# manuelbb-upb/Morbit.jl

Hardware: AMD Instinct MI355X
Metric: RBF build+solve+eval cycles/sec (higher is better)
Workload: dtype f64

## Files before the change

include/mrbf.h:

```cpp
#ifndef MRBF_H
#define MRBF_H

#include <stdint.h>

#ifdef __cplusplus
extern "C" {
#endif

typedef struct mrbf_ctx mrbf_ctx;
typedef struct mrbf_model mrbf_model;

enum {
    MRBF_CUBIC = 0,
    MRBF_INV_MULTIQUADRIC = 1,
    MRBF_MULTIQUADRIC = 2,
    MRBF_THIN_PLATE_SPLINE = 3,
    MRBF_GAUSSIAN = 4
};

enum {
    MRBF_OK = 0,
    MRBF_ENOTPD = 1,
    MRBF_ESINGULAR = 2,
    MRBF_EHIP = 3,
// ... 20 lines not shown
    MRBF_OPT_TIMING = 6,
    MRBF_OPT_DIAG_IMPL = 7,
    MRBF_OPT_CHOL_WINDOW = 8,
    MRBF_OPT_SPIN_MS = 9,
    MRBF_OPT_LAST_DEVICE_MS = 11,
    MRBF_OPT_SLOW_LAUNCHES = 12,
    MRBF_OPT_ARENA_BYTES = 13,
    MRBF_OPT_LIVE_HANDLES = 14,
    MRBF_OPT_DEBUG_FAULT = 10
};

enum {
    MRBF_FB_CHOL_HOST_DRIVEN = 1,
    MRBF_FB_BACKSOLVE_BLOCKED = 2,
    MRBF_FB_LU = 4
};

typedef struct {
    int32_t path;
    int32_t factor_info;
    int32_t n, q;
    double rel_residual;
    double max_pitw;
    double mu;
    float ms_gram, ms_project, ms_factor, ms_solve, ms_check, ms_total;
    int32_t fallbacks;
    int32_t giveup_code;
    float ms_factor_device;
    int32_t slow_launches;
} mrbf_fit_info;

typedef struct {
    float ms_total;
    float ms_dist, ms_kernel, ms_contract;
} mrbf_eval_info;

int32_t mrbf_init(int32_t device_id, mrbf_ctx **ctx);
int32_t mrbf_shutdown(mrbf_ctx *ctx);
const char *mrbf_last_error(const mrbf_ctx *ctx);
const char *mrbf_version(void);
int32_t mrbf_set_option(mrbf_ctx *ctx, int32_t key, double value);
int32_t mrbf_get_option(const mrbf_ctx *ctx, int32_t key, double *value);
int32_t mrbf_set_stream(mrbf_ctx *ctx, void *hip_stream);
int32_t mrbf_sync(mrbf_ctx *ctx);

int32_t mrbf_gram(mrbf_ctx *ctx, int64_t n, int32_t d, const double *centres, int32_t kernel_id, double a, double b,
                  int32_t poly_deg, double *Phi_out, double *Pi_out, float *ms);

int32_t mrbf_cross_gram(mrbf_ctx *ctx, int64_t m, int64_t n, int32_t d, const double *X, const double *centres, int32_t kernel_id,
                        double a, double b, double *K_out);

int32_t mrbf_fit(mrbf_ctx *ctx, int64_t n, int32_t d, int32_t k, const double *centres, const double *values,
                 int32_t kernel_id, double a, double b, int32_t poly_deg, mrbf_model **model, double *weights_out,
                 double *poly_out, mrbf_fit_info *info);

int32_t mrbf_model_from_coeffs(mrbf_ctx *ctx, int64_t n, int32_t d, int32_t k, const double *centres,
                               const double *weights, const double *poly, int32_t kernel_id, double a, double b,
                               int32_t poly_deg, mrbf_model **model);

int32_t mrbf_eval(mrbf_ctx *ctx, const mrbf_model *model, int64_t m, const double *X, double *vals_out,
                  double *jac_out, mrbf_eval_info *info);

int32_t mrbf_backtrack(mrbf_ctx *ctx, const mrbf_model *model, const double *x, const double *dir, double step0,
                       double omega, int32_t strict, double const_rhs, double shrink, double min_stepsize,
                       int32_t max_loops, double *x_plus, double *mx_plus, double *step, int32_t *n_loops);

int32_t mrbf_affine_scores(mrbf_ctx *ctx, int64_t mc, int32_t d, int32_t dz, const double *shifted, const double *Z, int32_t p_is_inf,
                           double *vals_out, int64_t *argmax, double *maxval);
int32_t mrbf_affine_select(mrbf_ctx *ctx, int64_t mc, int32_t d, const double *shifted, int32_t j0, const double *Q0, int32_t max_picks,
                           double pivot_val, int32_t p_is_inf, int64_t *picked_out, int32_t *n_picked, double *Z_out);

typedef struct {
    int64_t mc;
    int32_t j0;
    int32_t max_picks;
    double pivot_val;
    const double *shifted;
    const double *Q0;
    int64_t *picked_out;
    double *Z_out;
    int32_t n_picked;
    int32_t reserved;
} mrbf_affine_job;
int32_t mrbf_affine_select_batch(mrbf_ctx *ctx, int64_t n_starts, int32_t d, int32_t p_is_inf, mrbf_affine_job *jobs,
                                 float *ms_total);

typedef struct mrbf_round4_state mrbf_round4_state;
int32_t mrbf_round4(mrbf_ctx *ctx, int64_t n0, int32_t d, const double *start_sites, int64_t mc, const double *cand_sites,
                    int32_t kernel_id, double a, double b, int32_t poly_deg, int32_t max_points, double theta_pivot_cholesky,
                    int32_t *accepted_out, int32_t *n_accepted, mrbf_round4_state **state);
int32_t mrbf_fit_from_round4(mrbf_ctx *ctx, const mrbf_round4_state *state, int32_t k, const double *values, mrbf_model **model,
                             double *weights_out, double *poly_out, mrbf_fit_info *info);
int32_t mrbf_round4_sites(const mrbf_round4_state *state, int64_t *n0, int64_t *n_candidates, int32_t *n_accepted);
int32_t mrbf_free_round4(mrbf_ctx *ctx, mrbf_round4_state *state);

typedef struct {
    int64_t n0, mc;
    const double *start_sites;
    const double *cand_sites;
    int32_t kernel_id, poly_deg;
    double a, b;
    int32_t max_points;
    double theta_pivot_cholesky;
    int32_t *accepted_out;
    int32_t n_accepted;
    int32_t rc;
} mrbf_round4_job;
int32_t mrbf_round4_batch(mrbf_ctx *ctx, int64_t n_starts, int32_t d, mrbf_round4_job *jobs, float *ms_total);

int32_t mrbf_model_dims(const mrbf_model *model, int64_t *n, int32_t *d, int32_t *k, int32_t *q);
int32_t mrbf_free_model(mrbf_ctx *ctx, mrbf_model *model);

typedef struct {
    int64_t n, m;
    int32_t d, k, kernel_id, poly_deg;
    double a, b;
    const double *centres;
    const double *values;
    const double *X;
    double *weights_out;
    double *poly_out;
    double *vals_out;
    double *jac_out;
} mrbf_problem;

typedef struct {
    int32_t status;
    int32_t device;
    mrbf_fit_info fit;
    float ms_eval;
    double checksum_w;
    double checksum_vals;
} mrbf_result;

int32_t mrbf_batch_run(int32_t n_dev, const int32_t *device_ids, int64_t n_problems, const mrbf_problem *problems,
                       mrbf_result *results);

typedef struct {
    int64_t n;
    int32_t d, k, kernel_id, poly_deg;
    double a, b;
    const double *centres, *values;
    double *weights_out, *poly_out;
    mrbf_model *model;
    int32_t status;
    int32_t reserved;
    mrbf_fit_info info;
} mrbf_fit_job;
int32_t mrbf_fit_batch(mrbf_ctx *ctx, int64_t n_starts, mrbf_fit_job *jobs, float *ms_total);

int32_t mrbf_debug_env(const char *name);
int32_t mrbf_debug_mfma_layout(mrbf_ctx *ctx, double *out16x16_a_times_b, const double *A16x4, const double *B4x16);
int32_t mrbf_debug_potrf(mrbf_ctx *ctx, int64_t n, double *A_colmajor_inout, int32_t impl, int32_t *info, float *ms);
int32_t mrbf_debug_diag(mrbf_ctx *ctx, const double *A128, int32_t reps, float *ms_per_call, double *shader_cycles,
                        double *realtime_us);
int32_t mrbf_debug_mfma_peak(mrbf_ctx *ctx, int32_t blocks_per_cu, int32_t threads, int32_t iters, float *ms, double *tflops);
int32_t mrbf_debug_mfma_asm(mrbf_ctx *ctx, int32_t variant, int32_t blocks_per_cu, int32_t iters, float *ms, double *tflops,
                            double *cycles_per_mfma);
int32_t mrbf_debug_dgemm(mrbf_ctx *ctx, int32_t m, int32_t n, int32_t k, float *ms, double *tflops);
int32_t mrbf_debug_mega_tables(int32_t nt, int32_t mt, int32_t slack, int32_t slack_chain, int32_t first, int32_t win, int32_t srows,
                               int32_t half_cols, int64_t *out6);
int32_t mrbf_debug_mega_tables2(int32_t nt, int32_t mt, int32_t slack, int32_t slack_chain, int32_t first, int32_t win, int32_t srows,
                                int32_t half_cols, const int32_t *opt5, int64_t *out6);
int32_t mrbf_debug_mega_plan(int32_t nt, int32_t mt, int32_t xreal, int64_t *out39);

enum { MRBF_PS_OK = 0, MRBF_PS_CRITICAL = 1, MRBF_PS_FAILURE = 2 };
typedef struct {
    int32_t max_ideal_evals;
    int32_t max_ps_evals;
    int32_t max_polish_evals;
    int32_t reserved;
    uint64_t seed;
    double t0;
    double xtol_rel;
} mrbf_ps_options;
typedef struct {
    int32_t status;
    int32_t generations;
    int32_t evals_ideal, evals_ps, evals_polish;
    float ms_total;
    double tau;
} mrbf_ps_info;
int32_t mrbf_ps_step(mrbf_ctx *ctx, const mrbf_model *model, const double *x_n, const double *lb_eff, const double *ub_eff,
                     const double *fx_n, const double *r_or_null, const mrbf_ps_options *opts, double *x_trial, double *mx_trial,
                     double *r_out, mrbf_ps_info *info);

enum { MRBF_ROLE_NONE = -1, MRBF_ROLE_EQ = -2, MRBF_ROLE_INEQ = -3 };
typedef struct {
    int32_t n_models, n_objectives;
    const mrbf_model *const *models;
    const int32_t *roles;
    int32_t n_lin_eq, n_lin_ineq;
    const double *A_eq, *b_eq, *A_ineq, *b_ineq;
    double eq_tol;
} mrbf_ps_problem;
int32_t mrbf_ps_step_problem(mrbf_ctx *ctx, const mrbf_ps_problem *problem, const double *x_n, const double *lb_eff,
                             const double *ub_eff, const double *fx_n, const double *r_or_null, const mrbf_ps_options *opts,
                             double *x_trial, double *mx_trial, double *r_out, mrbf_ps_info *info);
int32_t mrbf_debug_ps_rank(mrbf_ctx *ctx, int32_t lam, const double *f, const double *phi, uint64_t seed, int32_t gen, int32_t impl,
                           int32_t *order_out, int32_t *gave_up);

enum { MRBF_SD_OK = 0, MRBF_SD_NO_OBJECTIVE = 1, MRBF_SD_INFEASIBLE = 2, MRBF_SD_GAVE_UP = 3 };
int32_t mrbf_sd_direction(mrbf_ctx *ctx, int64_t n_lp, int32_t d, int32_t k, int32_t m_eq, int32_t m_ineq, const double *G,
                          const double *x, const double *lb, const double *ub, const double *A_eq, const double *b_eq,
                          const double *A_ineq, const double *b_ineq, int32_t normalize, double *d_out, double *omega_out,
                          double *dual_out, int32_t *status_out, int32_t *iters_out);
typedef struct {
    int32_t status;
    int32_t iterations;
    int32_t bound_flips;
    float ms_total;
    double omega;
} mrbf_sd_info;
int32_t mrbf_sd_criticality(mrbf_ctx *ctx, const mrbf_ps_problem *problem, const double *x, const double *x_n, const double *lb,
                            const double *ub, int32_t normalize, double *d_out, double *dual_out, mrbf_sd_info *info);

enum { MRBF_NS_OK = 0, MRBF_NS_INFEASIBLE = 1, MRBF_NS_GAVE_UP = 2 };
int32_t mrbf_normal_direction(mrbf_ctx *ctx, int64_t n_lp, int32_t d, int32_t m_eq, int32_t m_ineq, const double *x, const double *lb,
                              const double *ub, const double *A_eq, const double *b_eq, const double *A_ineq, const double *b_ineq,
                              double *n_out, double *alpha_out, double *dual_out, int32_t *status_out, int32_t *iters_out);
typedef struct {
    int32_t status;
    int32_t iterations;
    int32_t bound_flips;
    float ms_total;
    double alpha;
    double delta;
} mrbf_normal_info;
int32_t mrbf_normal_step(mrbf_ctx *ctx, const mrbf_ps_problem *problem, int32_t d, const double *x, const double *lb, const double *ub,
                         double delta, double kappa_delta, double delta_max, int32_t variable_radius, double *n_out, double *dual_out,
                         mrbf_normal_info *info);

typedef struct {
    int32_t strict;
    int32_t max_loops;
    double const_rhs;
    double shrink;
    double min_stepsize;
} mrbf_sd_step_options;
typedef struct {
    int32_t branch;
    int32_t loops;
    float ms_total;
    double sigma;
    double omega;
    double step_norm;
} mrbf_sd_step_info;
int32_t mrbf_sd_step(mrbf_ctx *ctx, const mrbf_ps_problem *problem, const double *x, const double *x_n, double delta, const double *lb,
                     const double *ub, double omega, const double *d, const mrbf_sd_step_options *opts, double *x_plus, double *mx_plus,
                     mrbf_sd_step_info *info);

typedef struct {
    int32_t sd_status;
    int32_t iterations, bound_flips;
    int32_t branch, loops;
    int32_t reserved;
    double omega;
    double omega_step;
    double sigma, step_norm;
} mrbf_sd_batch_record;
int32_t mrbf_sd_iterate_batch(mrbf_ctx *ctx, int64_t n_starts, const mrbf_ps_problem *shape, const mrbf_model *const *models,
                              const double *x, const double *x_n, const double *delta, const double *lb, const double *ub,
                              int32_t normalize, const mrbf_sd_step_options *opts, double *d_out, double *x_plus, double *mx_plus,
                              mrbf_sd_batch_record *records, float *ms_total);

typedef struct {
    int32_t status;
    int32_t iterations, bound_flips;
    int32_t reserved;
    double alpha;
    double delta;
} mrbf_normal_batch_record;
int32_t mrbf_normal_step_batch(mrbf_ctx *ctx, int64_t n_starts, const mrbf_ps_problem *shape, const mrbf_model *const *models, int32_t d,
                               const double *x, const double *lb, const double *ub, const double *delta, double kappa_delta,
                               double delta_max, int32_t variable_radius, double *n_out, double *x_n_out, double *dual_out,
                               mrbf_normal_batch_record *records, float *ms_total);

enum { MRBF_DISPATCH_REFERENCE = 0, MRBF_DISPATCH_DEVICE = 1 };
enum { MRBF_FIT_FULL = 0, MRBF_FIT_FROM_ROUND4 = 1 };
enum { MRBF_ENTRY_ROUND4 = 1, MRBF_ENTRY_FIT_FROM_ROUND4 = 2, MRBF_ENTRY_PS_STEP = 3, MRBF_ENTRY_BACKTRACK = 4, MRBF_ENTRY_AFFINE = 5,
       MRBF_ENTRY_SD = 6, MRBF_ENTRY_NORMAL = 7, MRBF_ENTRY_SD_STEP = 8, MRBF_ENTRY_SD_BATCH = 9, MRBF_ENTRY_AFFINE_BATCH = 10,
       MRBF_ENTRY_FIT_BATCH = 11, MRBF_ENTRY_NORMAL_BATCH = 12, MRBF_ENTRY_ROUND4_BATCH = 13 };
int32_t mrbf_dispatch_ps(int32_t d, int32_t k, int32_t n_models, int32_t n_nl_constraints, int32_t n_lin_constraints, int32_t n_foreign);
int32_t mrbf_dispatch_sd(int32_t d, int32_t k, int32_t n_models, int32_t n_nl_constraints, int32_t n_lin_constraints, int32_t n_foreign);
int32_t mrbf_dispatch_normal(int32_t d, int32_t n_models, int32_t n_nl_constraints, int32_t n_lin_constraints, int32_t n_foreign);
int32_t mrbf_dispatch_sd_step(int32_t d, int32_t k, int32_t n_models, int32_t n_nl_constraints, int32_t n_lin_constraints, int32_t n_foreign,
                              int32_t max_loops);
int32_t mrbf_dispatch_sd_batch(int64_t n_starts, int32_t d, int32_t k, int32_t n_models, int32_t n_nl_constraints,
                               int32_t n_lin_constraints, int32_t n_foreign, int32_t max_loops);
int32_t mrbf_dispatch_normal_batch(int64_t n_starts, int32_t d, int32_t n_models, int32_t n_nl_constraints, int32_t n_lin_constraints,
                                   int32_t n_foreign);
int32_t mrbf_dispatch_backtrack(int32_t n_objective_models, int32_t n_foreign, int32_t outputs_in_order);
int32_t mrbf_dispatch_affine(int64_t n_candidates, int32_t d);
int32_t mrbf_dispatch_affine_batch(int64_t n_starts, int32_t d, int32_t p_is_inf);
int32_t mrbf_dispatch_round4(int64_t n0, int32_t d, int32_t poly_deg, int64_t n_candidates);
int32_t mrbf_dispatch_fit_batch(int64_t n_starts);
int32_t mrbf_dispatch_round4_batch(int64_t n_starts, int32_t d);
int32_t mrbf_dispatch_fit(int64_t n_training, int64_t state_n0, int32_t state_q, int32_t state_n_accepted, int32_t same_sites);
int32_t mrbf_dispatch_after(int32_t entry, int32_t rc);

int32_t mrbf_stochastic_rank(int32_t lam, const double *f, const double *phi, const double *u, double pf, int32_t *idx_out);

#ifdef __cplusplus
}
#endif
#endif
// ... 1 lines not shown
```

morbit.jl_amd/_lib.py:

```python
import ctypes
import os

import numpy as np

_HERE = os.path.dirname(os.path.abspath(__file__))
LIB_PATH = os.environ.get("MRBF_LIB") or os.path.join(_HERE, "libmrbf.so")

c_dp = ctypes.POINTER(ctypes.c_double)
c_fp = ctypes.POINTER(ctypes.c_float)
c_ip = ctypes.POINTER(ctypes.c_int32)
c_vp = ctypes.c_void_p

MRBF_OK, MRBF_ENOTPD, MRBF_ESINGULAR, MRBF_EHIP, MRBF_EBLAS, MRBF_ENOMEM, MRBF_ENODEVICE, MRBF_ENCCL = range(8)
PATH_CHOL, PATH_PROJ_CHOL, PATH_LU, PATH_MINNORM, PATH_ROUND4 = 1, 2, 3, 4, 5
OPT_GRAM_MODE, OPT_RESIDUAL, OPT_FORCE_PATH, OPT_CHOL_IMPL, OPT_EVAL_IMPL, OPT_TIMING, OPT_DIAG_IMPL, OPT_CHOL_WINDOW = 1, 2, 3, 4, 5, 6, 7, 8
OPT_SPIN_MS, OPT_DEBUG_FAULT, OPT_LAST_DEVICE_MS, OPT_SLOW_LAUNCHES = 9, 10, 11, 12
OPT_ARENA_BYTES, OPT_LIVE_HANDLES = 13, 14
FB_CHOL_HOST_DRIVEN, FB_BACKSOLVE_BLOCKED, FB_LU = 1, 2, 4


class FitInfo(ctypes.Structure):
    _fields_ = [("path", ctypes.c_int32), ("factor_info", ctypes.c_int32), ("n", ctypes.c_int32), ("q", ctypes.c_int32),
                ("rel_residual", ctypes.c_double), ("max_pitw", ctypes.c_double), ("mu", ctypes.c_double),
                ("ms_gram", ctypes.c_float), ("ms_project", ctypes.c_float), ("ms_factor", ctypes.c_float),
# ... 24 lines not shown

    def asdict(self):
        return {f: getattr(self, f) for f, _ in self._fields_}


PS_OK, PS_CRITICAL, PS_FAILURE = 0, 1, 2
ROLE_NONE, ROLE_EQ, ROLE_INEQ = -1, -2, -3
DISPATCH_REFERENCE, DISPATCH_DEVICE = 0, 1
FIT_FULL, FIT_FROM_ROUND4 = 0, 1
ENTRY_ROUND4, ENTRY_FIT_FROM_ROUND4, ENTRY_PS_STEP, ENTRY_BACKTRACK, ENTRY_AFFINE, ENTRY_SD, ENTRY_NORMAL, ENTRY_SD_STEP = 1, 2, 3, 4, 5, 6, 7, 8
ENTRY_SD_BATCH = 9
ENTRY_AFFINE_BATCH = 10
ENTRY_FIT_BATCH = 11
ENTRY_NORMAL_BATCH = 12
ENTRY_ROUND4_BATCH = 13
SD_OK, SD_NO_OBJECTIVE, SD_INFEASIBLE, SD_GAVE_UP = 0, 1, 2, 3
NS_OK, NS_INFEASIBLE, NS_GAVE_UP = 0, 1, 2
SD_BRANCH_DELTA, SD_BRANCH_ONE, SD_BRANCH_INTERSECT = 0, 1, 2


class PsProblem(ctypes.Structure):
    _fields_ = [("n_models", ctypes.c_int32), ("n_objectives", ctypes.c_int32), ("models", ctypes.POINTER(ctypes.c_void_p)),
                ("roles", ctypes.POINTER(ctypes.c_int32)), ("n_lin_eq", ctypes.c_int32), ("n_lin_ineq", ctypes.c_int32),
                ("A_eq", ctypes.c_void_p), ("b_eq", ctypes.c_void_p), ("A_ineq", ctypes.c_void_p), ("b_ineq", ctypes.c_void_p),
                ("eq_tol", ctypes.c_double)]


class SdInfo(ctypes.Structure):
    _fields_ = [("status", ctypes.c_int32), ("iterations", ctypes.c_int32), ("bound_flips", ctypes.c_int32), ("ms_total", ctypes.c_float),
                ("omega", ctypes.c_double)]

    def asdict(self):
        return {f: getattr(self, f) for f, _ in self._fields_}


class NormalInfo(ctypes.Structure):
    _fields_ = [("status", ctypes.c_int32), ("iterations", ctypes.c_int32), ("bound_flips", ctypes.c_int32), ("ms_total", ctypes.c_float),
                ("alpha", ctypes.c_double), ("delta", ctypes.c_double)]

    def asdict(self):
        return {f: getattr(self, f) for f, _ in self._fields_}


class SdStepOptions(ctypes.Structure):
    _fields_ = [("strict", ctypes.c_int32), ("max_loops", ctypes.c_int32), ("const_rhs", ctypes.c_double), ("shrink", ctypes.c_double),
                ("min_stepsize", ctypes.c_double)]


class SdStepInfo(ctypes.Structure):
    _fields_ = [("branch", ctypes.c_int32), ("loops", ctypes.c_int32), ("ms_total", ctypes.c_float), ("sigma", ctypes.c_double),
                ("omega", ctypes.c_double), ("step_norm", ctypes.c_double)]

    def asdict(self):
        return {f: getattr(self, f) for f, _ in self._fields_}


class SdBatchRecord(ctypes.Structure):
    _fields_ = [("sd_status", ctypes.c_int32), ("iterations", ctypes.c_int32), ("bound_flips", ctypes.c_int32), ("branch", ctypes.c_int32),
                ("loops", ctypes.c_int32), ("reserved", ctypes.c_int32), ("omega", ctypes.c_double), ("omega_step", ctypes.c_double),
                ("sigma", ctypes.c_double), ("step_norm", ctypes.c_double)]

    def asdict(self):
        return {f: getattr(self, f) for f, _ in self._fields_}


class NormalBatchRecord(ctypes.Structure):
    _fields_ = [("status", ctypes.c_int32), ("iterations", ctypes.c_int32), ("bound_flips", ctypes.c_int32), ("reserved", ctypes.c_int32),
                ("alpha", ctypes.c_double), ("delta", ctypes.c_double)]

    def asdict(self):
        return {f: getattr(self, f) for f, _ in self._fields_}


class AffineJob(ctypes.Structure):
    _fields_ = [("mc", ctypes.c_int64), ("j0", ctypes.c_int32), ("max_picks", ctypes.c_int32), ("pivot_val", ctypes.c_double),
                ("shifted", ctypes.c_void_p), ("Q0", ctypes.c_void_p), ("picked_out", ctypes.c_void_p), ("Z_out", ctypes.c_void_p),
                ("n_picked", ctypes.c_int32), ("reserved", ctypes.c_int32)]


class Round4Job(ctypes.Structure):
    _fields_ = [("n0", ctypes.c_int64), ("mc", ctypes.c_int64), ("start_sites", ctypes.c_void_p), ("cand_sites", ctypes.c_void_p),
                ("kernel_id", ctypes.c_int32), ("poly_deg", ctypes.c_int32), ("a", ctypes.c_double), ("b", ctypes.c_double),
                ("max_points", ctypes.c_int32), ("theta_pivot_cholesky", ctypes.c_double), ("accepted_out", ctypes.c_void_p),
                ("n_accepted", ctypes.c_int32), ("rc", ctypes.c_int32)]


class FitJob(ctypes.Structure):
    _fields_ = [("n", ctypes.c_int64), ("d", ctypes.c_int32), ("k", ctypes.c_int32), ("kernel_id", ctypes.c_int32),
                ("poly_deg", ctypes.c_int32), ("a", ctypes.c_double), ("b", ctypes.c_double), ("centres", ctypes.c_void_p),
                ("values", ctypes.c_void_p), ("weights_out", ctypes.c_void_p), ("poly_out", ctypes.c_void_p), ("model", ctypes.c_void_p),
                ("status", ctypes.c_int32), ("reserved", ctypes.c_int32), ("info", FitInfo)]


class Problem(ctypes.Structure):
    _fields_ = [("n", ctypes.c_int64), ("m", ctypes.c_int64), ("d", ctypes.c_int32), ("k", ctypes.c_int32),
                ("kernel_id", ctypes.c_int32), ("poly_deg", ctypes.c_int32), ("a", ctypes.c_double), ("b", ctypes.c_double),
                ("centres", c_dp), ("values", c_dp), ("X", c_dp), ("weights_out", c_dp), ("poly_out", c_dp),
                ("vals_out", c_dp), ("jac_out", c_dp)]


class Result(ctypes.Structure):
    _fields_ = [("status", ctypes.c_int32), ("device", ctypes.c_int32), ("fit", FitInfo), ("ms_eval", ctypes.c_float),
                ("checksum_w", ctypes.c_double), ("checksum_vals", ctypes.c_double)]


SIGNATURES = {
    "mrbf_init": (ctypes.c_int32, [ctypes.c_int32, ctypes.POINTER(c_vp)]),
    "mrbf_shutdown": (ctypes.c_int32, [c_vp]),
    "mrbf_last_error": (ctypes.c_char_p, [c_vp]),
    "mrbf_version": (ctypes.c_char_p, []),
    "mrbf_set_option": (ctypes.c_int32, [c_vp, ctypes.c_int32, ctypes.c_double]),
    "mrbf_get_option": (ctypes.c_int32, [c_vp, ctypes.c_int32, c_dp]),
    "mrbf_set_stream": (ctypes.c_int32, [c_vp, c_vp]),
    "mrbf_sync": (ctypes.c_int32, [c_vp]),
    "mrbf_gram": (ctypes.c_int32, [c_vp, ctypes.c_int64, ctypes.c_int32, c_vp, ctypes.c_int32, ctypes.c_double,
                                   ctypes.c_double, ctypes.c_int32, c_vp, c_vp, c_fp]),
    "mrbf_cross_gram": (ctypes.c_int32, [c_vp, ctypes.c_int64, ctypes.c_int64, ctypes.c_int32, c_vp, c_vp, ctypes.c_int32, ctypes.c_double,
                                         ctypes.c_double, c_vp]),
    "mrbf_fit": (ctypes.c_int32, [c_vp, ctypes.c_int64, ctypes.c_int32, ctypes.c_int32, c_vp, c_vp, ctypes.c_int32,
                                  ctypes.c_double, ctypes.c_double, ctypes.c_int32, ctypes.POINTER(c_vp), c_vp, c_vp,
                                  ctypes.POINTER(FitInfo)]),
    "mrbf_model_from_coeffs": (ctypes.c_int32, [c_vp, ctypes.c_int64, ctypes.c_int32, ctypes.c_int32, c_vp, c_vp, c_vp,
                                                ctypes.c_int32, ctypes.c_double, ctypes.c_double, ctypes.c_int32,
                                                ctypes.POINTER(c_vp)]),
    "mrbf_eval": (ctypes.c_int32, [c_vp, c_vp, ctypes.c_int64, c_vp, c_vp, c_vp, ctypes.POINTER(EvalInfo)]),
    "mrbf_backtrack": (ctypes.c_int32, [c_vp, c_vp, c_vp, c_vp, ctypes.c_double, ctypes.c_double, ctypes.c_int32,
                                        ctypes.c_double, ctypes.c_double, ctypes.c_double, ctypes.c_int32, c_vp, c_vp,
                                        c_vp, c_ip]),
    "mrbf_affine_scores": (ctypes.c_int32, [c_vp, ctypes.c_int64, ctypes.c_int32, ctypes.c_int32, c_vp, c_vp, ctypes.c_int32, c_vp,
                                            ctypes.POINTER(ctypes.c_int64), c_dp]),
    "mrbf_affine_select": (ctypes.c_int32, [c_vp, ctypes.c_int64, ctypes.c_int32, c_vp, ctypes.c_int32, c_vp, ctypes.c_int32, ctypes.c_double,
                                            ctypes.c_int32, ctypes.POINTER(ctypes.c_int64), c_ip, c_vp]),
    "mrbf_affine_select_batch": (ctypes.c_int32, [c_vp, ctypes.c_int64, ctypes.c_int32, ctypes.c_int32, ctypes.POINTER(AffineJob), c_fp]),
    "mrbf_round4": (ctypes.c_int32, [c_vp, ctypes.c_int64, ctypes.c_int32, c_vp, ctypes.c_int64, c_vp, ctypes.c_int32, ctypes.c_double,
                                     ctypes.c_double, ctypes.c_int32, ctypes.c_int32, ctypes.c_double, c_vp, c_ip, ctypes.POINTER(c_vp)]),
    "mrbf_fit_from_round4": (ctypes.c_int32, [c_vp, c_vp, ctypes.c_int32, c_vp, ctypes.POINTER(c_vp), c_vp, c_vp, ctypes.POINTER(FitInfo)]),
    "mrbf_round4_sites": (ctypes.c_int32, [c_vp, ctypes.POINTER(ctypes.c_int64), ctypes.POINTER(ctypes.c_int64), c_ip]),
    "mrbf_free_round4": (ctypes.c_int32, [c_vp, c_vp]),
    "mrbf_round4_batch": (ctypes.c_int32, [c_vp, ctypes.c_int64, ctypes.c_int32, ctypes.POINTER(Round4Job), c_fp]),
    "mrbf_dispatch_round4_batch": (ctypes.c_int32, [ctypes.c_int64, ctypes.c_int32]),
    "mrbf_model_dims": (ctypes.c_int32, [c_vp, ctypes.POINTER(ctypes.c_int64), c_ip, c_ip, c_ip]),
    "mrbf_free_model": (ctypes.c_int32, [c_vp, c_vp]),
    "mrbf_batch_run": (ctypes.c_int32, [ctypes.c_int32, c_ip, ctypes.c_int64, ctypes.POINTER(Problem),
                                        ctypes.POINTER(Result)]),
    "mrbf_fit_batch": (ctypes.c_int32, [c_vp, ctypes.c_int64, ctypes.POINTER(FitJob), c_fp]),
    "mrbf_dispatch_fit_batch": (ctypes.c_int32, [ctypes.c_int64]),
    "mrbf_debug_mfma_layout": (ctypes.c_int32, [c_vp, c_vp, c_vp, c_vp]),
    "mrbf_debug_potrf": (ctypes.c_int32, [c_vp, ctypes.c_int64, c_vp, ctypes.c_int32, c_ip, c_fp]),
    "mrbf_debug_env": (ctypes.c_int32, [ctypes.c_char_p]),
    "mrbf_debug_diag": (ctypes.c_int32, [c_vp, c_vp, ctypes.c_int32, c_fp, c_dp, c_dp]),
    "mrbf_debug_ps_rank": (ctypes.c_int32, [c_vp, ctypes.c_int32, c_vp, c_vp, ctypes.c_uint64, ctypes.c_int32, ctypes.c_int32, c_ip, c_ip]),
    "mrbf_debug_mfma_peak": (ctypes.c_int32, [c_vp, ctypes.c_int32, ctypes.c_int32, ctypes.c_int32, c_fp, c_dp]),
    "mrbf_debug_mfma_asm": (ctypes.c_int32, [c_vp, ctypes.c_int32, ctypes.c_int32, ctypes.c_int32, c_fp, c_dp, c_dp]),
    "mrbf_debug_dgemm": (ctypes.c_int32, [c_vp, ctypes.c_int32, ctypes.c_int32, ctypes.c_int32, c_fp, c_dp]),
    "mrbf_debug_mega_tables": (ctypes.c_int32, [ctypes.c_int32] * 8 + [c_vp]),
    "mrbf_debug_mega_tables2": (ctypes.c_int32, [ctypes.c_int32] * 8 + [c_vp, c_vp]),
    "mrbf_debug_mega_plan": (ctypes.c_int32, [ctypes.c_int32] * 3 + [c_vp]),
    "mrbf_stochastic_rank": (ctypes.c_int32, [ctypes.c_int32, c_vp, c_vp, c_vp, ctypes.c_double, c_vp]),
    "mrbf_ps_step": (ctypes.c_int32, [c_vp, c_vp, c_vp, c_vp, c_vp, c_vp, c_vp, ctypes.POINTER(PsOptions), c_vp, c_vp, c_vp,
                                      ctypes.POINTER(PsInfo)]),
    "mrbf_ps_step_problem": (ctypes.c_int32, [c_vp, ctypes.POINTER(PsProblem), c_vp, c_vp, c_vp, c_vp, c_vp, ctypes.POINTER(PsOptions),
                                              c_vp, c_vp, c_vp, ctypes.POINTER(PsInfo)]),
    "mrbf_sd_direction": (ctypes.c_int32, [c_vp, ctypes.c_int64, ctypes.c_int32, ctypes.c_int32, ctypes.c_int32, ctypes.c_int32] + [c_vp] * 8
                          + [ctypes.c_int32, c_vp, c_vp, c_vp, c_vp, c_vp]),
    "mrbf_sd_criticality": (ctypes.c_int32, [c_vp, ctypes.POINTER(PsProblem), c_vp, c_vp, c_vp, c_vp, ctypes.c_int32, c_vp, c_vp,
                                             ctypes.POINTER(SdInfo)]),
    "mrbf_normal_direction": (ctypes.c_int32, [c_vp, ctypes.c_int64, ctypes.c_int32, ctypes.c_int32, ctypes.c_int32] + [c_vp] * 12),
    "mrbf_normal_step": (ctypes.c_int32, [c_vp, ctypes.POINTER(PsProblem), ctypes.c_int32, c_vp, c_vp, c_vp, ctypes.c_double, ctypes.c_double,
                                          ctypes.c_double, ctypes.c_int32, c_vp, c_vp, ctypes.POINTER(NormalInfo)]),
    "mrbf_sd_step": (ctypes.c_int32, [c_vp, ctypes.POINTER(PsProblem), c_vp, c_vp, ctypes.c_double, c_vp, c_vp, ctypes.c_double, c_vp,
                                      ctypes.POINTER(SdStepOptions), c_vp, c_vp, ctypes.POINTER(SdStepInfo)]),
    "mrbf_sd_iterate_batch": (ctypes.c_int32, [c_vp, ctypes.c_int64, ctypes.POINTER(PsProblem), ctypes.POINTER(ctypes.c_void_p), c_vp, c_vp, c_vp,
                                               c_vp, c_vp, ctypes.c_int32, ctypes.POINTER(SdStepOptions), c_vp, c_vp, c_vp,
                                               ctypes.POINTER(SdBatchRecord), c_fp]),
    "mrbf_dispatch_sd_batch": (ctypes.c_int32, [ctypes.c_int64] + [ctypes.c_int32] * 7),
    "mrbf_normal_step_batch": (ctypes.c_int32, [c_vp, ctypes.c_int64, ctypes.POINTER(PsProblem), ctypes.POINTER(ctypes.c_void_p), ctypes.c_int32,
                                                c_vp, c_vp, c_vp, c_vp, ctypes.c_double, ctypes.c_double, ctypes.c_int32, c_vp, c_vp, c_vp,
                                                ctypes.POINTER(NormalBatchRecord), c_fp]),
    "mrbf_dispatch_normal_batch": (ctypes.c_int32, [ctypes.c_int64] + [ctypes.c_int32] * 5),
    "mrbf_dispatch_ps": (ctypes.c_int32, [ctypes.c_int32] * 6),
    "mrbf_dispatch_sd_step": (ctypes.c_int32, [ctypes.c_int32] * 7),
    "mrbf_dispatch_sd": (ctypes.c_int32, [ctypes.c_int32] * 6),
    "mrbf_dispatch_normal": (ctypes.c_int32, [ctypes.c_int32] * 5),
    "mrbf_dispatch_backtrack": (ctypes.c_int32, [ctypes.c_int32] * 3),
    "mrbf_dispatch_affine": (ctypes.c_int32, [ctypes.c_int64, ctypes.c_int32]),
    "mrbf_dispatch_affine_batch": (ctypes.c_int32, [ctypes.c_int64, ctypes.c_int32, ctypes.c_int32]),
    "mrbf_dispatch_round4": (ctypes.c_int32, [ctypes.c_int64, ctypes.c_int32, ctypes.c_int32, ctypes.c_int64]),
    "mrbf_dispatch_fit": (ctypes.c_int32, [ctypes.c_int64, ctypes.c_int64, ctypes.c_int32, ctypes.c_int32, ctypes.c_int32]),
    "mrbf_dispatch_after": (ctypes.c_int32, [ctypes.c_int32, ctypes.c_int32]),
}

_LIB = None


class MrbfError(RuntimeError):
    def __init__(self, code, msg):
        super().__init__("libmrbf error %d: %s" % (code, msg))
        self.code = code


def load():
    global _LIB
    if _LIB is None:
        if not os.path.exists(LIB_PATH):
            raise ImportError("libmrbf.so is not built (%s); run `python -c 'import __graft_entry__ as g; g.build()'` "
                              "or `make -C morbit.jl_amd/csrc`. There is no CPU fallback." % LIB_PATH)
        lib = ctypes.CDLL(LIB_PATH)
        for name, (res, args) in SIGNATURES.items():
            fn = getattr(lib, name)
            fn.restype = res
            fn.argtypes = args
        _LIB = lib
    return _LIB


def as_ptr(a):
    if a is None:
        return None
    if isinstance(a, np.ndarray):
        return ctypes.c_void_p(a.ctypes.data)
    if hasattr(a, "data_ptr"):
        return ctypes.c_void_p(a.data_ptr())
    raise TypeError("expected numpy array or tensor, got %r" % type(a))


def host_f64(a, shape=None):
    a = np.ascontiguousarray(a, dtype=np.float64)
    if shape is not None:
        a = a.reshape(shape)
    return a


class Context:

    def __init__(self, device_id=-1):
        self.lib = load()
        h = c_vp()
        rc = self.lib.mrbf_init(device_id, ctypes.byref(h))
        if rc != 0:
            raise MrbfError(rc, (self.lib.mrbf_last_error(None) or b"").decode())
        self.h = h

    def check(self, rc):
        if rc != 0:
            raise MrbfError(rc, (self.lib.mrbf_last_error(self.h) or b"").decode())

    def set_option(self, key, value):
        self.check(self.lib.mrbf_set_option(self.h, key, float(value)))

    def get_option(self, key):
        v = ctypes.c_double()
        self.check(self.lib.mrbf_get_option(self.h, key, ctypes.byref(v)))
        return v.value

    def sync(self):
        self.check(self.lib.mrbf_sync(self.h))

    def close(self):
        if getattr(self, "h", None):
            self.lib.mrbf_shutdown(self.h)
            self.h = None

    def __del__(self):
        try:
            self.close()
        except Exception:
            pass


_DEFAULT_CTX = {}


def default_context(device_id=-1):
    import threading

    key = (threading.get_ident(), device_id)
    if key not in _DEFAULT_CTX:
        _DEFAULT_CTX[key] = Context(device_id)
    return _DEFAULT_CTX[key]
```

morbit.jl_amd/csrc/backsolve.hip:

```cpp
#include "common.hpp"

namespace mrbf {

namespace bsolve {

constexpr int NB = 128, NTHR = 512;
typedef double v2d __attribute__((ext_vector_type(2)));
typedef double v4d __attribute__((ext_vector_type(4)));
typedef __attribute__((address_space(1))) unsigned gu32;
typedef __attribute__((address_space(1))) double gf64;
typedef __attribute__((address_space(1))) v2d gv2d;

template <int KB>
struct Shared {
    double xs[2][KB][NB];
    int ok;
};

__global__ __launch_bounds__(256) void premul_kernel(const double *__restrict__ L, int64_t lda, const double *__restrict__ linv_all,
                                                     double *__restrict__ Mbuf, int nb, unsigned *__restrict__ flags, int nflags,
                                                     unsigned long long *__restrict__ xb, int nxb) {
    for (int e = blockIdx.x * 256 + threadIdx.x; e < nflags; e += gridDim.x * 256) flags[e] = 0u;
    for (int e = blockIdx.x * 256 + threadIdx.x; e < nxb; e += gridDim.x * 256) xb[e] = ~0ull;
    const int slab = blockIdx.x & 3, t = (blockIdx.x >> 2) & 1, j = blockIdx.x >> 3;
    const int i = j + 1 + t;
    if (i >= nb) return;
    const double *A = L + (int64_t)i * NB + (int64_t)j * NB * lda;
    const double *B = linv_all + (size_t)j * NB * NB;
    double *M = Mbuf + ((size_t)j * 2 + t) * NB * NB;
    const int lane = threadIdx.x & 63, wave = threadIdx.x >> 6, l15 = lane & 15, l4 = lane >> 4;
    const int i0 = 32 * wave, j0 = 32 * slab;
    v4d acc[2][2];
#pragma unroll
    for (int a = 0; a < 2; ++a)
#pragma unroll
        for (int b = 0; b < 2; ++b) acc[a][b] = (v4d){0.0, 0.0, 0.0, 0.0};
    const double *pa = A + (i0 + l15) + (int64_t)(j0 + l4) * lda;
    const double *pb = B + (j0 + l4) + (int64_t)(j0 + l15) * NB;
    constexpr int UK = 8;
    double fa0[2][UK], fa1[2][UK], fb0[2][UK], fb1[2][UK];
    auto burst = [&](int buf) {
#pragma unroll
        for (int u = 0; u < UK; ++u) {
            fa0[buf][u] = pa[(int64_t)4 * u * lda];
            fa1[buf][u] = pa[(int64_t)4 * u * lda + 16];
            fb0[buf][u] = pb[4 * u];
            fb1[buf][u] = pb[4 * u + 16 * NB];
        }
        pa += (int64_t)4 * UK * lda;
        pb += 4 * UK;
    };
    auto mma = [&](int buf) {
#pragma unroll
        for (int u = 0; u < UK; ++u) {
            acc[0][0] = __builtin_amdgcn_mfma_f64_16x16x4f64(fa0[buf][u], fb0[buf][u], acc[0][0], 0, 0, 0);
            acc[0][1] = __builtin_amdgcn_mfma_f64_16x16x4f64(fa0[buf][u], fb1[buf][u], acc[0][1], 0, 0, 0);
            acc[1][0] = __builtin_amdgcn_mfma_f64_16x16x4f64(fa1[buf][u], fb0[buf][u], acc[1][0], 0, 0, 0);
            acc[1][1] = __builtin_amdgcn_mfma_f64_16x16x4f64(fa1[buf][u], fb1[buf][u], acc[1][1], 0, 0, 0);
        }
    };
    const int nburst = (NB - j0) / (4 * UK);
    burst(0);
    for (int b = 0; b < nburst; b += 2) {
        if (b + 1 < nburst) burst(1);
        mma(0);
        if (b + 1 >= nburst) break;
        if (b + 2 < nburst) burst(0);
        mma(1);
    }
#pragma unroll
    for (int a = 0; a < 2; ++a)
#pragma unroll
        for (int b = 0; b < 2; ++b)
#pragma unroll
            for (int r = 0; r < 4; ++r) M[(i0 + 16 * a + l4 + 4 * r) + (size_t)(j0 + 16 * b + l15) * NB] = acc[a][b][r];
}

__device__ __forceinline__ void load_tile(const double *__restrict__ T, int64_t ldt, v2d (&r)[2][8]) {
    const int lane = threadIdx.x & 63, w = threadIdx.x >> 6;
    const double *p = T + (int64_t)(16 * w + 2 * (lane >> 3)) * ldt + 2 * (lane & 7);
#pragma unroll
    for (int cc = 0; cc < 2; ++cc)
#pragma unroll
        for (int u = 0; u < 8; ++u) r[cc][u] = *(const gv2d *)(p + cc * ldt + 16 * u);
}

template <int N>
__device__ __forceinline__ double shl_lanes(double v) {
    const long long b = __double_as_longlong(v);
    const int lo = __builtin_amdgcn_update_dpp((int)b, (int)b, 0x100 + N, 0xf, 0xf, false);
    const int hi = __builtin_amdgcn_update_dpp((int)(b >> 32), (int)(b >> 32), 0x100 + N, 0xf, 0xf, false);
    return __longlong_as_double(((long long)hi << 32) | (unsigned)lo);
}

template <int KB>
__device__ __forceinline__ void tile_dot(const double (*xs)[NB], const v2d (&r)[2][8], double (&out)[2][KB]) {
    const int q = threadIdx.x & 7;
    double acc[2][KB];
#pragma unroll
    for (int cc = 0; cc < 2; ++cc)
#pragma unroll
        for (int l = 0; l < KB; ++l) acc[cc][l] = 0.0;
#pragma unroll
    for (int u = 0; u < 8; ++u) {
#pragma unroll
        for (int l = 0; l < KB; ++l) {
            const v2d x = *(const v2d *)&xs[l][16 * u + 2 * q];
#pragma unroll
            for (int cc = 0; cc < 2; ++cc) acc[cc][l] = fma(r[cc][u][1], x[1], fma(r[cc][u][0], x[0], acc[cc][l]));
        }
    }
#pragma unroll
    for (int cc = 0; cc < 2; ++cc)
#pragma unroll
        for (int l = 0; l < KB; ++l) {
            double v = acc[cc][l];
            v += shl_lanes<4>(v);
            v += shl_lanes<2>(v);
            v += shl_lanes<1>(v);
            out[cc][l] = v;
        }
}

template <int KB>
__device__ __forceinline__ void await_block(Shared<KB> &sh, double (*xs)[NB], const double *glob, int i, double spec, int backoff,
                                            unsigned *abortw, unsigned epoch, unsigned long long spin_ticks, int *status, int code) {
    const int tid = threadIdx.x;
    if (tid >= KB * NB) return;
    const gf64 *src = (const gf64 *)&glob[((size_t)i * KB + tid / NB) * NB + (tid % NB)];
    double v = spec;
    if (__double_as_longlong(v) == -1ll) v = __hip_atomic_load(src, __ATOMIC_RELAXED, __HIP_MEMORY_SCOPE_AGENT);
    unsigned spins = 0;
    unsigned long long t0 = 0;
    while (__double_as_longlong(v) == -1ll) {
        if ((++spins & 63u) == 0u) {
            if (__hip_atomic_load((const gu32 *)abortw, __ATOMIC_RELAXED, __HIP_MEMORY_SCOPE_AGENT) != 0u) {
                sh.ok = 0;
                break;
            }
            const unsigned long long now = wall_clock64();
            if (t0 == 0) t0 = now;
            if (now - t0 > spin_ticks) {
                __hip_atomic_store((gu32 *)abortw, epoch, __ATOMIC_RELAXED, __HIP_MEMORY_SCOPE_AGENT);
                *(__attribute__((address_space(1))) int *)status = code + (i & 0xff);
                sh.ok = 0;
                break;
            }
        }
        for (int b = 0; b < backoff; ++b) __builtin_amdgcn_s_sleep(8);
        v = __hip_atomic_load(src, __ATOMIC_RELAXED, __HIP_MEMORY_SCOPE_AGENT);
    }
    xs[tid / NB][tid % NB] = v;
}

__device__ __forceinline__ void lds_barrier() { asm volatile("s_waitcnt lgkmcnt(0)\n\ts_barrier" ::: "memory"); }

__device__ __forceinline__ void publish(double *dst, v2d v) {
    if (__double_as_longlong(v[0]) == -1ll) v[0] = __longlong_as_double(0x7ff8000000000000ll);
    if (__double_as_longlong(v[1]) == -1ll) v[1] = __longlong_as_double(0x7ff8000000000000ll);
    asm volatile("global_store_dwordx4 %0, %1, off sc1" ::"v"(dst), "v"(v) : "memory");
}

template <int KB>
__global__ __launch_bounds__(NTHR, 1) void backsolve_persistent_kernel(const double *__restrict__ L, int64_t lda, const double *__restrict__ linv_all,
                                                                        const double *__restrict__ Mbuf, double *__restrict__ Y, int64_t ldy, int k0,
                                                                        int nb, unsigned *flags, unsigned epoch, unsigned long long spin_ticks,
                                                                        int *status, int fault, double *__restrict__ xb, double *__restrict__ zb,
                                                                        long long *stamps) {
    __shared__ __attribute__((aligned(16))) Shared<KB> sh;
    const int p = (int)blockIdx.x >> 1;
    const bool finisher = blockIdx.x & 1;
    const int j = nb - 1 - p, tid = threadIdx.x;
    const int lane = tid & 63, col = 16 * (tid >> 6) + 2 * (lane >> 3), q = lane & 7;
    unsigned *abortw = flags + (size_t)nb * 32;
    const int na = nb - 1 - j, npm = na < 2 ? na : 2, npl = na - npm;
    if (tid == 0) sh.ok = 1;
// ... 13 lines not shown
        auto look = [&](int s) {
            const int i = nb - 1 - (s < npl ? s : (npl > 0 ? npl - 1 : 0));
            const int e = tid < KB * NB ? tid : 0;
            return __hip_atomic_load((const gf64 *)&xb[((size_t)i * KB + e / NB) * NB + (e % NB)], __ATOMIC_RELAXED, __HIP_MEMORY_SCOPE_AGENT);
        };
        double spec = fillv, spec2 = fillv;
        auto step = [&](int s, const v2d(&r)[2][8]) -> bool {
            double(*xs)[NB] = sh.xs[s & 1];
            if (s < npl) {
                const int i = nb - 1 - s;
                const int backoff = (i - j - 3) < 24 ? (i - j - 3) : 24;
                await_block<KB>(sh, xs, xb, i, spec, backoff, abortw, epoch, spin_ticks, status, 0x700);
                if (stamps && tid == 0 && s == npl - 1) stamps[256 * 5 + j * 4 + 0] = (long long)wall_clock64();
            } else if (q == 0) {
#pragma unroll
                for (int l = 0; l < KB; ++l) *(v2d *)&xs[l][col] = (v2d){w[0][l], w[1][l]};
            }
            spec = spec2;
            spec2 = look(s + 2);
            if (s + 2 >= npl) spec2 = fillv;
            lds_barrier();
            if (!sh.ok) return false;
            double dsum[2][KB];
            tile_dot<KB>(xs, r, dsum);
#pragma unroll
            for (int cc = 0; cc < 2; ++cc)
#pragma unroll
                for (int l = 0; l < KB; ++l) w[cc][l] = s == npl ? dsum[cc][l] : w[cc][l] - dsum[cc][l];
            return true;
        };
        v2d t0[2][8], t1[2][8], t2[2][8];
        const int o = (3 - nst % 3) % 3, G = (nst + o) / 3;
        if (0 - o >= 0) fetch(0 - o, t0);
        if (1 - o >= 0) fetch(1 - o, t1);
        fetch(2 - o, t2);
        spec = look(0);
        if (npl == 0) spec = fillv;
        spec2 = look(1);
        if (npl <= 1) spec2 = fillv;
        int g = 0;
        if (G >= 2) {
            const int s = -o;
            if (s >= 0 && !step(s, t0)) return;
            fetch(s + 3, t0);
            if (s + 1 >= 0 && !step(s + 1, t1)) return;
            fetch(s + 4, t1);
            if (!step(s + 2, t2)) return;
            fetch(s + 5, t2);
            g = 1;
        }
        for (; g < G - 1; ++g) {
            const int s = 3 * g - o;
            if (!step(s, t0)) return;
            fetch(s + 3, t0);
            if (!step(s + 1, t1)) return;
            fetch(s + 4, t1);
            if (!step(s + 2, t2)) return;
            fetch(s + 5, t2);
        }
        {
            const int s = 3 * (G - 1) - o;
            if (s >= 0 && !step(s, t0)) return;
            if (s + 1 >= 0 && !step(s + 1, t1)) return;
            if (!step(s + 2, t2)) return;
        }
        if (stamps && tid == 0) stamps[256 * 5 + j * 4 + 1] = (long long)wall_clock64();
        if (q == 0) {
#pragma unroll
            for (int l = 0; l < KB; ++l) publish(&zb[((size_t)j * KB + l) * NB + col], (v2d){w[0][l], w[1][l]});
        }
        return;
    }
    v2d tm2[2][8], tm1[2][8];
    if (npm == 2) load_tile(Mbuf + ((size_t)j * 2 + 1) * NB * NB, NB, tm2);
    if (npm >= 1) load_tile(Mbuf + (size_t)j * 2 * NB * NB, NB, tm1);
    double acc[2][KB];
#pragma unroll
    for (int cc = 0; cc < 2; ++cc)
#pragma unroll
        for (int l = 0; l < KB; ++l) acc[cc][l] = 0.0;
    if (npm == 2) {
        await_block<KB>(sh, sh.xs[0], xb, j + 2, fillv, 1, abortw, epoch, spin_ticks, status, 0x700);
        lds_barrier();
        if (!sh.ok) return;
        if (stamps && tid == 0) stamps[256 * 5 + j * 4 + 3] = (long long)wall_clock64();
        tile_dot<KB>(sh.xs[0], tm2, acc);
    }
    v2d zj[KB];
    if (q == 0) {
        unsigned spins = 0;
        unsigned long long t0 = 0;
#pragma unroll
        for (int l = 0; l < KB; ++l) {
            const double *src = &zb[((size_t)j * KB + l) * NB + col];
            while (true) {
                v2d v;
                asm volatile("global_load_dwordx4 %0, %1, off sc1\n\ts_waitcnt vmcnt(0)" : "=v"(v) : "v"(src) : "memory");
                if (__double_as_longlong(v[0]) != -1ll && __double_as_longlong(v[1]) != -1ll) {
                    zj[l] = v;
                    break;
                }
                if ((++spins & 63u) == 0u) {
                    if (__hip_atomic_load((const gu32 *)abortw, __ATOMIC_RELAXED, __HIP_MEMORY_SCOPE_AGENT) != 0u) {
                        sh.ok = 0;
                        break;
                    }
                    const unsigned long long now = wall_clock64();
                    if (t0 == 0) t0 = now;
                    if (now - t0 > spin_ticks) {
                        __hip_atomic_store((gu32 *)abortw, epoch, __ATOMIC_RELAXED, __HIP_MEMORY_SCOPE_AGENT);
                        *(__attribute__((address_space(1))) int *)status = 0x600 + (j & 0xff);
                        sh.ok = 0;
                        break;
                    }
                }
                __builtin_amdgcn_s_sleep(2);
            }
            if (!sh.ok) break;
        }
    }
    if (stamps && tid == 0) stamps[256 * 5 + j * 4 + 2] = (long long)wall_clock64();
    double last[2][KB];
#pragma unroll
    for (int cc = 0; cc < 2; ++cc)
#pragma unroll
        for (int l = 0; l < KB; ++l) last[cc][l] = 0.0;
    if (npm >= 1) {
        if (stamps && tid == 0) stamps[256 * 4 + j] = (long long)wall_clock64();
        await_block<KB>(sh, sh.xs[1], xb, j + 1, fillv, 0, abortw, epoch, spin_ticks, status, 0x700);
        if (stamps && tid == 0) stamps[j * 4 + 0] = (long long)wall_clock64();
        lds_barrier();
        if (!sh.ok) return;
        if (stamps && tid == 0) stamps[j * 4 + 1] = (long long)wall_clock64();
        tile_dot<KB>(sh.xs[1], tm1, last);
    } else {
        lds_barrier();
        if (!sh.ok) return;
    }
    if ((fault & 1) && j == nb / 2) return;
    if (stamps && tid == 0) stamps[j * 4 + 2] = (long long)wall_clock64();
    if (q == 0) {
#pragma unroll
        for (int l = 0; l < KB; ++l) {
            const v2d v = (v2d){(zj[l][0] - acc[0][l]) - last[0][l], (zj[l][1] - acc[1][l]) - last[1][l]};
            publish(&xb[((size_t)j * KB + l) * NB + col], v);
            *(v2d *)&Y[(int64_t)(k0 + l) * ldy + (int64_t)j * NB + col] = v;
        }
    }
}

}

int backsolve_blocked(mrbf_ctx *ctx, int64_t npad, const double *L, int64_t lda, const double *linv_all, double *Y, int64_t ldy, int k);

int backsolve_persistent(mrbf_ctx *ctx, int64_t npad, const double *L, int64_t lda, const double *linv_all, double *Y, int64_t ldy, int k,
                         int *status) {
    using namespace bsolve;
    const int nb = (int)(npad / NB);
    static const int force_old = mrbf_env("MRBF_BACKSOLVE_LAUNCHES") ? atoi(mrbf_env("MRBF_BACKSOLVE_LAUNCHES")) : 0;
    const int ncu = ctx->ncu;
    if (force_old || nb < 3 || nb > ncu || (lda & 1) || (reinterpret_cast<uintptr_t>(L) & 15))
        return backsolve_blocked(ctx, npad, L, lda, linv_all, Y, ldy, k);
    unsigned *flags;
    MRBF_TRY(get_buf(ctx, S_BSOLVE_FLAGS, (size_t)(nb + 1) * 32, &flags));
    const unsigned long long spin_ticks = (unsigned long long)std::max(1, ctx->spin_ms) * 100000ull;
    const int fault = (ctx->debug_fault & 2) ? 1 : 0;
    double *xb, *Mbuf;
    MRBF_TRY(get_buf(ctx, S_BSOLVE_X, (size_t)2 * nb * 4 * NB, &xb));
    MRBF_TRY(get_buf(ctx, S_BSOLVE_M, (size_t)nb * 2 * NB * NB, &Mbuf));
    hipLaunchKernelGGL(premul_kernel, dim3((unsigned)(8 * (nb - 1))), dim3(256), 0, ctx->stream, L, lda, linv_all, Mbuf, nb, flags, (nb + 1) * 32,
                       reinterpret_cast<unsigned long long *>(xb), 2 * nb * 4 * NB);
    static const bool want_stamps = mrbf_env("MRBF_BSOLVE_STAMPS") && atoi(mrbf_env("MRBF_BSOLVE_STAMPS")) != 0;
    long long *stamps = nullptr;
    if (want_stamps) {
        static long long *dbg = nullptr;
        if (!dbg) MRBF_HIP(ctx, hipMalloc(&dbg, (size_t)256 * 9 * sizeof(long long)));
        stamps = dbg;
    }
    unsigned epoch = 0;
    for (int k0 = 0; k0 < k; k0 += 4) {
        const int kb = std::min(4, k - k0);
        ++epoch;
        if (k0 > 0) MRBF_HIP(ctx, hipMemsetAsync(xb, 0xff, (size_t)2 * nb * 4 * NB * sizeof(double), ctx->stream));
#define MRBF_BSP(KBV)                                                                                                          \
    hipLaunchKernelGGL((backsolve_persistent_kernel<KBV>), dim3((unsigned)(2 * nb)), dim3(NTHR), 0, ctx->stream, L, lda, linv_all, Mbuf, Y, ldy, k0, nb, \
                       flags, epoch, spin_ticks, status, fault, xb, xb + (size_t)nb * 4 * NB, stamps)
        if (kb == 1) MRBF_BSP(1); else if (kb == 2) MRBF_BSP(2); else if (kb == 3) MRBF_BSP(3); else MRBF_BSP(4);
#undef MRBF_BSP
    }
    MRBF_HIP(ctx, hipGetLastError());
    if (want_stamps) {
        std::vector<long long> h((size_t)256 * 9);
        MRBF_HIP(ctx, hipMemcpyAsync(h.data(), stamps, h.size() * sizeof(long long), hipMemcpyDeviceToHost, ctx->stream));
        MRBF_HIP(ctx, hipStreamSynchronize(ctx->stream));
        double seen = 0, bar = 0, dot = 0, hop = 0, late = 0;
        int cnt = 0;
        for (int j = 1; j + 2 < nb; ++j) {
            seen += (double)(h[j * 4 + 0] - h[(j + 1) * 4 + 2]);
            bar += (double)(h[j * 4 + 1] - h[j * 4 + 0]);
            dot += (double)(h[j * 4 + 2] - h[j * 4 + 1]);
            hop += (double)(h[j * 4 + 2] - h[(j + 1) * 4 + 2]);
            late += (double)(h[256 * 4 + j] - h[(j + 1) * 4 + 2]);
            ++cnt;
        }
        double a3 = 0, zt = 0, zs = 0, x2 = 0;
        int c2 = 0;
        for (int j = 2; j + 4 < nb; ++j) {
            const long long *S = &h[256 * 5 + j * 4];
            a3 += (double)(S[0] - h[(j + 3) * 4 + 2]);
            zt += (double)(S[1] - S[0]);
            zs += (double)(S[2] - S[1]);
            x2 += (double)(S[3] - h[(j + 2) * 4 + 2]);
            ++c2;
        }
        fprintf(stderr, "[backsolve stamps] streamer: x_{j+3} seen %.2f us after its publication, z_j published %.2f us later, finisher has z_j %.2f us "
                "later; finisher past x_{j+2} %.2f us after that block's publication\n", a3 / c2 / 100.0, zt / c2 / 100.0, zs / c2 / 100.0, x2 / c2 / 100.0);
        fprintf(stderr, "[backsolve stamps] nb %d: publish -> seen %.2f us, seen -> barrier %.2f us, barrier -> publish %.2f us, step %.2f us; "
                "the finisher starts polling %.2f us after the publication\n", nb, seen / cnt / 100.0, bar / cnt / 100.0, dot / cnt / 100.0,
                hop / cnt / 100.0, late / cnt / 100.0);
    }
    return 0;
}

}
```

morbit.jl_amd/csrc/chol.hip:

```cpp
#include <chrono>

#include "common.hpp"

namespace mrbf {

int debug_diag(mrbf_ctx *ctx, const double *A128_dev, int reps, float *ms_per_call, unsigned long long *stamps_host);
int launch_pad_identity(mrbf_ctx *ctx, double *A, int64_t n, int64_t npad, int64_t ld);

int potrf_lower(mrbf_ctx *ctx, int impl, int64_t n, double *A, int64_t lda, int *info_host) {
    int *dinfo;
    MRBF_TRY(get_buf(ctx, S_INFO, (size_t)4, &dinfo));
    const int64_t npad = round_up(n, 128);
    if (impl == 0) impl = (lda >= npad) ? ((npad >= ctx->mega.min && npad <= ctx->mega.max) ? 3 : 2) : 1;
    if (impl == 2 || impl == 3) {
        if (lda < npad) return fail(ctx, MRBF_EHIP, "built-in Cholesky needs lda >= round_up(n,128)");
        MRBF_TRY(launch_pad_identity(ctx, A, n, npad, lda));
        PotrfOpts opt;
        opt.impl = impl;
        opt.any_size = true;
        MRBF_TRY(potrf_blocked_tall(ctx, npad, npad, A, lda, dinfo, nullptr, opt));
    } else {
        MRBF_BLAS(ctx, rocsolver_dpotrf(ctx->blas, rocblas_fill_lower, (int)n, A, (int)lda, dinfo));
    }
    MRBF_HIP(ctx, hipMemcpyAsync(info_host, dinfo, sizeof(int), hipMemcpyDeviceToHost, ctx->stream));
    MRBF_HIP(ctx, hipStreamSynchronize(ctx->stream));
    MRBF_TRY(mega_collect_stat(ctx));
    return 0;
}

}

using namespace mrbf;

extern "C" int32_t mrbf_debug_potrf(mrbf_ctx *ctx, int64_t n, double *A, int32_t impl, int32_t *info, float *ms) {
    if (!ctx) return -1;
    if (n <= 0) return -2;
    if (!A) return -3;
    (void)hipSetDevice(ctx->device);
    const int64_t npad = round_up(n, 128);
    double *dA;
    MRBF_TRY(get_buf(ctx, S_PHI, (size_t)npad * npad, &dA));
    const hipMemcpyKind in = is_device_ptr(A) ? hipMemcpyDeviceToDevice : hipMemcpyHostToDevice;
    const hipMemcpyKind out = is_device_ptr(A) ? hipMemcpyDeviceToDevice : hipMemcpyDeviceToHost;
    MRBF_HIP(ctx, hipMemcpy2DAsync(dA, (size_t)npad * sizeof(double), A, (size_t)n * sizeof(double), (size_t)n * sizeof(double),
                                   (size_t)n, in, ctx->stream));
    int hinfo = 0;
    static const double host_trace_ms = mrbf_env("MRBF_MEGA_HOSTTRACE") ? atof(mrbf_env("MRBF_MEGA_HOSTTRACE")) : 0.0;
    auto now_ms = []() { return std::chrono::duration<double, std::milli>(std::chrono::steady_clock::now().time_since_epoch()).count(); };
    const double h0 = now_ms();
    MRBF_HIP(ctx, hipEventRecord(ctx->ev[0], ctx->stream));
    const double h1 = now_ms();
    MRBF_TRY(potrf_lower(ctx, impl, n, dA, npad, &hinfo));
    const double h2 = now_ms();
    MRBF_HIP(ctx, hipEventRecord(ctx->ev[1], ctx->stream));
    MRBF_HIP(ctx, hipEventSynchronize(ctx->ev[1]));
    const double h3 = now_ms();
    if (host_trace_ms > 0.0 && h3 - h0 > host_trace_ms)
        fprintf(stderr, "mrbf_debug_potrf host trace (n %lld): record ev0 %.3f ms | potrf_lower incl. sync %.3f | record ev1 + sync %.3f\n", (long long)n,
                h1 - h0, h2 - h1, h3 - h2);
    if (ms) MRBF_HIP(ctx, hipEventElapsedTime(ms, ctx->ev[0], ctx->ev[1]));
    if (info) *info = hinfo;
    MRBF_HIP(ctx, hipMemcpy2DAsync(A, (size_t)n * sizeof(double), dA, (size_t)npad * sizeof(double), (size_t)n * sizeof(double),
                                   (size_t)n, out, ctx->stream));
    MRBF_HIP(ctx, hipStreamSynchronize(ctx->stream));
    return MRBF_OK;
}

extern "C" int32_t mrbf_debug_diag(mrbf_ctx *ctx, const double *A128, int32_t reps, float *ms_per_call, double *shader_cycles,
                                   double *realtime_us) {
    if (!ctx) return -1;
    if (!A128) return -2;
    (void)hipSetDevice(ctx->device);
    const double *dA;
    MRBF_TRY(stage_in(ctx, S_STAGE_A, A128, 128 * 128, &dA));
    unsigned long long st[6] = {0, 0, 0, 0, 0, 0};
    float ms = 0;
    MRBF_TRY(debug_diag(ctx, dA, reps, &ms, st));
    if (ms_per_call) *ms_per_call = ms;
    if (shader_cycles) *shader_cycles = (double)st[0];
    if (realtime_us) *realtime_us = (double)st[1] / 100.0;
    if (mrbf_env("MRBF_DIAG_VERBOSE"))
        fprintf(stderr, "diag segments (cycles over 128 columns, wave 0): barrier %llu read %llu critical %llu rest %llu\n", st[2], st[3],
                st[4], st[5]);
    return MRBF_OK;
}
```

morbit.jl_amd/csrc/chol_blocked.hip:

```cpp
#include "common.hpp"
#include "mega_gemm.hpp"

namespace mrbf {

typedef double v4d __attribute__((ext_vector_type(4)));
typedef double v2d __attribute__((ext_vector_type(2)));

constexpr int CNB = 128;

enum { UPD_LOWER_SUB = 0, UPD_OVERWRITE = 1, UPD_FULL_SUB = 2, UPD_COLUMN_SUB = 3 };
int launch_diag_v4(mrbf_ctx *ctx, hipStream_t st, double *Ajj, int64_t lda, double *Linv, int *dinfo, int col0);

template <int TM, int MODE>
__global__ __launch_bounds__(256, 2) void chol_update_kernel(const double *__restrict__ A, int64_t lda,
                                                             const double *__restrict__ B, int64_t ldb,
                                                             double *__restrict__ C, int64_t ldc, int K,
                                                             const int *__restrict__ info, int mt_sq = 0, int ntiles_total = 0,
                                                             const double *__restrict__ cvec = nullptr, double cs = 0.0, int64_t cn = 0) {
    constexpr int NJ = (TM == 128) ? 4 : 2;
    __shared__ __attribute__((aligned(16))) double smem[mega::NSTG * mega::STG];
    if (info && *info != 0) return;
    if (MODE == UPD_OVERWRITE || MODE == UPD_COLUMN_SUB) __builtin_amdgcn_s_setprio(2);
    const int tid = threadIdx.x, lane = tid & 63, wave = tid >> 6;
    const int l15 = lane & 15, l4 = lane >> 4;
    const int tile_end = (MODE == UPD_LOWER_SUB && ntiles_total > 0) ? ntiles_total : (int)blockIdx.x + 1;
    for (int bid = blockIdx.x; bid < tile_end; bid += gridDim.x) {
    int ti, tj;
    if (MODE == UPD_LOWER_SUB) {
        const int ntri = mt_sq * (mt_sq + 1) / 2;
        if (bid < ntri || mt_sq == 0) {
            int t = (int)((sqrt(8.0 * (double)bid + 1.0) - 1.0) * 0.5);
            while ((t + 1) * (t + 2) / 2 <= bid) ++t;
            while (t * (t + 1) / 2 > bid) --t;
            ti = t;
            tj = bid - t * (t + 1) / 2;
        } else {
            ti = mt_sq + (bid - ntri) / mt_sq;
            tj = (bid - ntri) % mt_sq;
        }
    } else {
        ti = blockIdx.x;
        tj = blockIdx.y;
    }
    const int64_t I0 = (int64_t)ti * TM, J0 = (int64_t)tj * 128;
    const int ioff = (TM == 128) ? (wave >> 1) * 64 : 0;
    const int joff = (TM == 128) ? (wave & 1) * 64 : wave * 32;

    v4d acc[NJ][4];
#pragma unroll
    for (int j = 0; j < NJ; ++j)
#pragma unroll
        for (int i = 0; i < 4; ++i) acc[j][i] = (v4d){0.0, 0.0, 0.0, 0.0};

    asm volatile("s_waitcnt vmcnt(0)" ::: "memory");
    constexpr bool NEG_START = (MODE == UPD_LOWER_SUB);
    if (NEG_START) {
#pragma unroll
        for (int j = 0; j < NJ; ++j)
#pragma unroll
            for (int r = 0; r < 4; ++r) {
                const int64_t gj = J0 + joff + j * 16 + l4 + 4 * r;
#pragma unroll
                for (int i = 0; i < 4; ++i) acc[j][i][r] = -C[(I0 + ioff + i * 16 + l15) + gj * ldc];
            }
    }
    mega::gemm_acc<TM>(A + I0, lda, B + J0, ldb, K, acc, smem);
    double cvi[4] = {0.0, 0.0, 0.0, 0.0}, cei[4] = {0.0, 0.0, 0.0, 0.0};
    if (MODE == UPD_LOWER_SUB && cvec) {
#pragma unroll
        for (int i = 0; i < 4; ++i) {
            const int64_t gi = I0 + ioff + i * 16 + l15;
            cvi[i] = cs * cvec[gi];
            cei[i] = gi < cn ? cs : 0.0;
        }
    }
#pragma unroll
    for (int j = 0; j < NJ; ++j) {
        double cv[4][4];
        double cvj[4] = {0.0, 0.0, 0.0, 0.0}, cej[4] = {0.0, 0.0, 0.0, 0.0};
        if (MODE == UPD_LOWER_SUB && cvec) {
#pragma unroll
            for (int r = 0; r < 4; ++r) {
                const int64_t gj = J0 + joff + j * 16 + l4 + 4 * r;
                cvj[r] = cvec[gj];
                cej[r] = gj < cn ? 1.0 : 0.0;
            }
        }
        if (MODE != UPD_OVERWRITE && !NEG_START) {
#pragma unroll
            for (int r = 0; r < 4; ++r) {
                const int64_t gj = J0 + joff + j * 16 + l4 + 4 * r;
#pragma unroll
                for (int i = 0; i < 4; ++i) cv[r][i] = C[(I0 + ioff + i * 16 + l15) + gj * ldc];
            }
        }
#pragma unroll
        for (int r = 0; r < 4; ++r) {
            const int64_t gj = J0 + joff + j * 16 + l4 + 4 * r;
#pragma unroll
            for (int i = 0; i < 4; ++i) {
                const int64_t gi = I0 + ioff + i * 16 + l15;
                double *dst = C + gi + gj * ldc;
                if (MODE == UPD_OVERWRITE) {
                    *dst = acc[j][i][r];
                } else if (MODE == UPD_FULL_SUB) {
                    *dst = cv[r][i] - acc[j][i][r];
                } else if (MODE == UPD_COLUMN_SUB) {
                    if (gi >= gj) *dst = cv[r][i] - acc[j][i][r];
                } else {
                    double x = -acc[j][i][r];
                    if (cvec) x -= fma(cei[i], cvj[r], cvi[i] * cej[r]);
                    if (ti != tj || gi >= gj) *dst = x;
                }
            }
        }
    }
    if (bid + (int)gridDim.x < tile_end) __syncthreads();
    }
}

struct __attribute__((aligned(16))) DiagShared {
    double col[2][2 * CNB];
    double rinv[2];
    int sbad;
    unsigned long long seg[4];
    int stamp;
};

__device__ __forceinline__ double fast_rsqrt(double x) {
    double y = __builtin_amdgcn_rsq(x);
    const double h = 0.5 * x;
#pragma unroll
    for (int it = 0; it < 3; ++it) y = y * fma(-h, y * y, 1.5);
    return y;
}

template <int KV, bool STAMP>
__device__ __forceinline__ void diag_phase(double (&a)[8][8], DiagShared &sh, int ti, int tj, int half, int &buf, int &bad) {
    constexpr int KN = (KV < 7) ? KV + 1 : 7;
    double piv = 0.0;
    if (half == 0) piv = __shfl(a[KV][KV], tj, 16);
#pragma unroll 1
    for (int kk = 0; kk < 16; ++kk) {
        const int k = KV * 16 + kk;
        const bool st = STAMP && threadIdx.x < 64;
        unsigned long long s0 = 0, s1 = 0, s2 = 0, s3 = 0;
        if (st) s0 = __builtin_amdgcn_s_memtime();
        __syncthreads();
        if (st) s1 = __builtin_amdgcn_s_memtime();
        double lj[8];
#pragma unroll
        for (int v = KV; v < 8; ++v) lj[v] = sh.col[buf][tj + 16 * v];
        if (half == 0) {
            double li[8];
#pragma unroll
            for (int u = KV; u < 8; ++u) li[u] = sh.col[buf][ti + 16 * u];
            if (st) {
                asm volatile("s_waitcnt lgkmcnt(0)" ::: "memory");
                s2 = __builtin_amdgcn_s_memtime();
            }
            if (kk < 15) {
                if (tj > kk) piv = fma(-lj[KV], lj[KV], piv);
                if (tj == kk + 1) {
                    const int kn = k + 1;
                    double rinv = 0.0;
                    if (piv > 0.0) {
                        rinv = fast_rsqrt(piv);
                    } else if (bad == 0) {
                        bad = kn + 1;
                    }
                    if (ti == 0) sh.rinv[buf ^ 1] = rinv;
                    double w[8];
#pragma unroll
                    for (int u = 0; u < 8; ++u) {
                        const int i = ti + 16 * u;
                        double val = 0.0;
                        if (u >= KV && i >= kn) {
                            val = fma(-li[u], lj[KV], a[u][KV]) * rinv;
                            a[u][KV] = val;
                        }
                        w[u] = val;
                    }
#pragma unroll
                    for (int u = 0; u < 8; ++u) sh.col[buf ^ 1][ti + 16 * u] = w[u];
                }
            } else if (KV < 7) {
                if (tj == 0) {
                    const int kn = k + 1;
                    const double pv = __shfl(fma(-li[KN], lj[KN], a[KN][KN]), 0, 16);
                    double rinv = 0.0;
                    if (pv > 0.0) {
                        rinv = fast_rsqrt(pv);
                    } else if (bad == 0) {
                        bad = kn + 1;
                    }
                    if (ti == 0) sh.rinv[buf ^ 1] = rinv;
                    double w[8];
#pragma unroll
                    for (int u = 0; u < 8; ++u) {
                        double val = 0.0;
                        if (u >= KN) {
                            val = fma(-li[u], lj[KN], a[u][KN]) * rinv;
                            a[u][KN] = val;
                        }
                        w[u] = val;
                    }
#pragma unroll
                    for (int u = 0; u < 8; ++u) sh.col[buf ^ 1][ti + 16 * u] = w[u];
                }
            }
            if (st) {
                asm volatile("s_waitcnt lgkmcnt(0)" ::: "memory");
                s3 = __builtin_amdgcn_s_memtime();
            }
            const bool own_next = (kk < 15) ? (tj == kk + 1) : (KV < 7 && tj == 0);
            const bool lowtri = ti >= tj;
#pragma unroll
            for (int v = KV; v < 8; ++v) {
                double ljv = lj[v];
                if (v == KV) ljv = (tj > kk && !(own_next && kk < 15)) ? ljv : 0.0;
                if (v == KN && KV < 7) ljv = (own_next && kk == 15) ? 0.0 : ljv;
                a[v][v] = fma(lowtri ? -li[v] : 0.0, ljv, a[v][v]);
#pragma unroll
                for (int u = v + 1; u < 8; ++u) a[u][v] = fma(-li[u], ljv, a[u][v]);
            }
            if (st && threadIdx.x == 0) {
                asm volatile("" ::"v"(a[7][7]));
                const unsigned long long s4 = __builtin_amdgcn_s_memtime();
                sh.seg[0] += s1 - s0;
                sh.seg[1] += s2 - s1;
                sh.seg[2] += s3 - s2;
                sh.seg[3] += s4 - s3;
            }
        } else {
            const double rinv = sh.rinv[buf];
            const double ljk = (tj > kk) ? lj[KV] : 0.0;
#pragma unroll
            for (int u = 0; u <= KV; ++u) {
                const double erk = sh.col[buf][CNB + ti + 16 * u] * rinv;
                if (tj == kk) a[u][KV] = erk;
                a[u][KV] = fma(-erk, ljk, a[u][KV]);
#pragma unroll
                for (int v = KV + 1; v < 8; ++v) a[u][v] = fma(-erk, lj[v], a[u][v]);
            }
            if (kk < 15) {
                if (tj == kk + 1) {
#pragma unroll
                    for (int u = 0; u < 8; ++u) sh.col[buf ^ 1][CNB + ti + 16 * u] = (u <= KV) ? a[u][KV] : 0.0;
                }
            } else if (KV < 7) {
                if (tj == 0) {
#pragma unroll
                    for (int u = 0; u < 8; ++u) sh.col[buf ^ 1][CNB + ti + 16 * u] = (u <= KN) ? a[u][KN] : 0.0;
                }
            }
        }
        buf ^= 1;
    }
}

template <bool STAMP>
__global__ __launch_bounds__(512) void chol_diag_kernel(double *__restrict__ A, int64_t lda, double *__restrict__ Linv,
                                                        int *__restrict__ info, int col0,
                                                        unsigned long long *__restrict__ stamps) {
    __shared__ DiagShared sh;
    if (*info != 0) return;
    unsigned long long t0 = 0, r0 = 0;
    if (STAMP) {
        if (threadIdx.x == 0) sh.seg[0] = sh.seg[1] = sh.seg[2] = sh.seg[3] = 0;
        __syncthreads();
        t0 = __builtin_amdgcn_s_memtime();
        r0 = __builtin_amdgcn_s_memrealtime();
    }
    const int tid = threadIdx.x, ti = tid & 15, tj = (tid >> 4) & 15, half = tid >> 8;
    double a[8][8];
#pragma unroll
    for (int v = 0; v < 8; ++v)
#pragma unroll
        for (int u = 0; u < 8; ++u) {
            const int i = ti + 16 * u, j = tj + 16 * v;
            if (half == 0)
                a[u][v] = (i >= j) ? A[i + (int64_t)j * lda] : 0.0;
            else
                a[u][v] = (i == j) ? 1.0 : 0.0;
        }
    int buf = 0, bad = 0;
    if (tj == 0) {
        if (half == 0) {
            const double pv = __shfl(a[0][0], 0, 16);
            double rinv = 0.0;
            if (pv > 0.0) {
                rinv = fast_rsqrt(pv);
            } else {
                bad = 1;
            }
            if (ti == 0) sh.rinv[0] = rinv;
#pragma unroll
            for (int u = 0; u < 8; ++u) {
                a[u][0] *= rinv;
                sh.col[0][ti + 16 * u] = a[u][0];
            }
        } else {
#pragma unroll
            for (int u = 0; u < 8; ++u) sh.col[0][CNB + ti + 16 * u] = (u == 0) ? a[0][0] : 0.0;
        }
    }
    diag_phase<0, STAMP>(a, sh, ti, tj, half, buf, bad);
    diag_phase<1, STAMP>(a, sh, ti, tj, half, buf, bad);
    diag_phase<2, STAMP>(a, sh, ti, tj, half, buf, bad);
    diag_phase<3, STAMP>(a, sh, ti, tj, half, buf, bad);
    diag_phase<4, STAMP>(a, sh, ti, tj, half, buf, bad);
    diag_phase<5, STAMP>(a, sh, ti, tj, half, buf, bad);
    diag_phase<6, STAMP>(a, sh, ti, tj, half, buf, bad);
    diag_phase<7, STAMP>(a, sh, ti, tj, half, buf, bad);
    if (tid == 0) sh.sbad = 0x7fffffff;
    __syncthreads();
    if (bad) atomicMin(&sh.sbad, bad);
    __syncthreads();
    if (sh.sbad != 0x7fffffff) {
        if (tid == 0) *info = col0 + sh.sbad;
        return;
    }
#pragma unroll
    for (int v = 0; v < 8; ++v)
#pragma unroll
        for (int u = 0; u < 8; ++u) {
            const int i = ti + 16 * u, j = tj + 16 * v;
            if (half == 0) {
                if (i >= j) A[i + (int64_t)j * lda] = a[u][v];
            } else {
                Linv[j + i * CNB] = (j >= i) ? a[u][v] : 0.0;
            }
        }
    if (STAMP && threadIdx.x == 0) {
        stamps[0] = __builtin_amdgcn_s_memtime() - t0;
        stamps[1] = __builtin_amdgcn_s_memrealtime() - r0;
        for (int q = 0; q < 4; ++q) stamps[2 + q] = sh.seg[q];
    }
}

__global__ void pad_identity_kernel(double *__restrict__ A, int64_t n, int64_t npad, int64_t ld) {
    const int64_t idx = (int64_t)blockIdx.x * blockDim.x + threadIdx.x;
    const int64_t pw = npad - n;
    if (idx >= npad * pw) return;
    const int64_t j = n + idx / npad, i = idx % npad;
    A[i + j * ld] = (i == j) ? 1.0 : 0.0;
    if (i < n) A[j + i * ld] = 0.0;
}

int launch_pad_identity(mrbf_ctx *ctx, double *A, int64_t n, int64_t npad, int64_t ld) {
    if (npad == n) return 0;
    const int64_t cnt = npad * (npad - n);
    hipLaunchKernelGGL(pad_identity_kernel, dim3((unsigned)((cnt + 255) / 256)), dim3(256), 0, ctx->stream, A, n, npad, ld);
    MRBF_HIP(ctx, hipGetLastError());
    return 0;
}

int debug_diag(mrbf_ctx *ctx, const double *A128_dev, int reps, float *ms_per_call, unsigned long long *stamps_host) {
    const bool with_stamps = reps > 0;
    if (reps < 0) reps = -reps;
    double *W, *Linv;
    int *dinfo;
    unsigned long long *st;
    MRBF_TRY(get_buf(ctx, S_PHI, (size_t)CNB * CNB * reps, &W));
    MRBF_TRY(get_buf(ctx, S_CHOL_WS, (size_t)CNB * CNB, &Linv));
    MRBF_TRY(get_buf(ctx, S_INFO, (size_t)4, &dinfo));
    MRBF_TRY(get_buf(ctx, S_MISC, (size_t)8, (double **)&st));
    for (int r = 0; r < reps; ++r)
        MRBF_HIP(ctx, hipMemcpyAsync(W + (size_t)r * CNB * CNB, A128_dev, sizeof(double) * CNB * CNB, hipMemcpyDeviceToDevice, ctx->stream));
    MRBF_HIP(ctx, hipMemsetAsync(dinfo, 0, sizeof(int), ctx->stream));
    MRBF_HIP(ctx, hipEventRecord(ctx->ev[0], ctx->stream));
    for (int r = 0; r < reps; ++r)
        if (ctx->diag_impl != 1)
            launch_diag_v4(ctx, ctx->stream, W + (size_t)r * CNB * CNB, (int64_t)CNB, Linv, dinfo, 0);
        else if (with_stamps)
            hipLaunchKernelGGL(chol_diag_kernel<true>, dim3(1), dim3(512), 0, ctx->stream, W + (size_t)r * CNB * CNB, (int64_t)CNB, Linv,
                               dinfo, 0, st);
        else
            hipLaunchKernelGGL(chol_diag_kernel<false>, dim3(1), dim3(512), 0, ctx->stream, W + (size_t)r * CNB * CNB, (int64_t)CNB, Linv,
                               dinfo, 0, (unsigned long long *)nullptr);
    MRBF_HIP(ctx, hipEventRecord(ctx->ev[1], ctx->stream));
    MRBF_HIP(ctx, hipEventSynchronize(ctx->ev[1]));
    float t;
    MRBF_HIP(ctx, hipEventElapsedTime(&t, ctx->ev[0], ctx->ev[1]));
    *ms_per_call = t / reps;
    if (const char *e = mrbf_env("MRBF_DIAG_DBG")) {
        if (atoi(e) & 4) {
            double seg[6];
            MRBF_HIP(ctx, hipMemcpy(seg, Linv, sizeof(seg), hipMemcpyDeviceToHost));
            fprintf(stderr, "diag segments (wave 0, cycles over 8 panels): pre-leaf %.0f leaf %.0f post-leaf %.0f wait-X %.0f deferred %.0f wait-Y %.0f\n",
                    seg[0], seg[1], seg[2], seg[3], seg[4], seg[5]);
        }
    }
    MRBF_HIP(ctx, hipMemcpy(stamps_host, st, 6 * sizeof(unsigned long long), hipMemcpyDeviceToHost));
    return 0;
}

int launch_update_lower(mrbf_ctx *ctx, const double *A, int64_t lda, const double *B, int64_t ldb, double *C, int64_t ldc, int64_t nt,
                        int K, const double *cvec, double cs, int64_t cn) {
    if (nt <= 0 || K <= 0) return 0;
    hipLaunchKernelGGL((chol_update_kernel<128, UPD_LOWER_SUB>), dim3((unsigned)(nt * (nt + 1) / 2)), dim3(256), 0, ctx->stream, A,
                       lda, B, ldb, C, ldc, K, (const int *)nullptr, (int)nt, 0, cvec, cs, cn);
    MRBF_HIP(ctx, hipGetLastError());
    return 0;
}

int potrf_blocked_tall(mrbf_ctx *ctx, int64_t ncols, int64_t mrows, double *A, int64_t lda, int *dinfo, double *linv_all, PotrfOpts opt) {
    if (ncols % CNB != 0 || mrows % CNB != 0 || mrows < ncols || (lda & 1) || (reinterpret_cast<uintptr_t>(A) & 15))
        return fail(ctx, MRBF_EHIP, "potrf_blocked needs 128-padded, 16-byte aligned storage (ncols=%lld mrows=%lld lda=%lld)",
                    (long long)ncols, (long long)mrows, (long long)lda);
    const int impl = opt.impl != 0 ? opt.impl : ctx->chol_impl;
    if ((impl == 3 || (impl == 0 && ncols <= ctx->mega.max)) && (opt.any_size || ncols >= ctx->mega.min))
        return potrf_mega_tall(ctx, ncols, mrows, A, lda, dinfo, linv_all, opt);
    double *Lone = nullptr;
    if (!linv_all) MRBF_TRY(get_buf(ctx, S_CHOL_WS, (size_t)CNB * CNB, &Lone));
    hipStream_t S = ctx->stream, M = ctx->bulk_stream, P = ctx->panel_stream;
    hipEvent_t evStart = ctx->evx[0], evT = ctx->evx[1], evU2 = ctx->evx[2], evEnd = ctx->evx[3];
    const bool single = ncols <= 4 * CNB;
    if (single) M = P = S;
    MRBF_HIP(ctx, hipMemsetAsync(dinfo, 0, sizeof(int), S));
    if (!single) {
        MRBF_HIP(ctx, hipEventRecord(evStart, S));
        MRBF_HIP(ctx, hipStreamWaitEvent(P, evStart, 0));
        MRBF_HIP(ctx, hipStreamWaitEvent(M, evStart, 0));
    }
    const int nb = (int)(ncols / CNB);
    bool have_u2 = false;
    int w0 = 0, W = 1;
    for (int j = 0; j < nb; ++j) {
        const int64_t c = (int64_t)j * CNB;
        if (j == w0) {
            const int64_t rem = ncols - c;
            W = (rem > 4800) ? 4 : (rem > 2400 ? 2 : 1);
            if (ctx->chol_window > 0) W = ctx->chol_window;
        }
        const bool last_in_window = (j == w0 + W - 1) || (j == nb - 1);
        const int kpan = (int)((j - w0 + 1) * CNB);
        const int64_t cw = (int64_t)w0 * CNB;
        double *Ajj = A + c + c * lda;
        double *Linv = linv_all ? linv_all + (size_t)j * CNB * CNB : Lone;
        if (ctx->diag_impl == 1)
            hipLaunchKernelGGL(chol_diag_kernel<false>, dim3(1), dim3(512), 0, P, Ajj, lda, Linv, dinfo, (int)c,
                               (unsigned long long *)nullptr);
        else
            launch_diag_v4(ctx, P, Ajj, lda, Linv, dinfo, (int)c);
        const int64_t m = mrows - c - CNB;
        if (m <= 0) break;
        double *A21 = A + (c + CNB) + c * lda;
        hipLaunchKernelGGL((chol_update_kernel<64, UPD_OVERWRITE>), dim3((unsigned)(m / 64), 1), dim3(256), 0, P, A21, lda, Linv,
                           (int64_t)CNB, A21, lda, CNB, dinfo);
        if (c + CNB >= ncols) break;
        if (!single) MRBF_HIP(ctx, hipEventRecord(evT, P));
        if (have_u2 && !single) {
            MRBF_HIP(ctx, hipStreamWaitEvent(P, evU2, 0));
            have_u2 = false;
        }
        const double *Pw = A + (c + CNB) + cw * lda;
        double *A22 = A + (c + CNB) + (c + CNB) * lda;
        hipLaunchKernelGGL((chol_update_kernel<64, UPD_COLUMN_SUB>), dim3((unsigned)(m / 64), 1), dim3(256), 0, P, Pw, lda, Pw, lda,
                           A22, lda, kpan, dinfo);
        if (last_in_window) {
            const int64_t mt2 = (ncols - c - 2 * CNB) / CNB;
            if (mt2 > 0) {
                if (!single) MRBF_HIP(ctx, hipStreamWaitEvent(M, evT, 0));
                const int64_t mx = (mrows - ncols) / CNB;
                const int64_t rem_next = ncols - c - CNB;
                int Wn = (rem_next > 4800) ? 4 : (rem_next > 2400 ? 2 : 1);
                if (ctx->chol_window > 0) Wn = ctx->chol_window;
                const int64_t na = std::min<int64_t>(Wn, mt2);
                const double *P2 = A + (c + 2 * CNB) + cw * lda;
                double *C2 = A + (c + 2 * CNB) + (c + 2 * CNB) * lda;
                hipLaunchKernelGGL((chol_update_kernel<128, UPD_LOWER_SUB>),
                                   dim3((unsigned)(na * (na + 1) / 2 + (mt2 - na + mx) * na)), dim3(256), 0, M, P2, lda, P2, lda, C2, lda,
                                   kpan, dinfo, (int)na);
                if (!single) MRBF_HIP(ctx, hipEventRecord(evU2, M));
                have_u2 = true;
                const int64_t mb2 = mt2 - na;
                if (mb2 > 0) {
                    const double *P3 = P2 + na * CNB;
                    double *C3 = C2 + na * CNB + na * CNB * lda;
                    const int64_t nt3 = mb2 * (mb2 + 1) / 2 + mx * mb2;
                    const int64_t g3 = (ctx->bulk_grid > 0 && nt3 > ctx->bulk_grid) ? ctx->bulk_grid : nt3;
                    hipLaunchKernelGGL((chol_update_kernel<128, UPD_LOWER_SUB>), dim3((unsigned)g3), dim3(256), 0, M, P3, lda, P3, lda,
                                       C3, lda, kpan, dinfo, (int)mb2, (int)nt3);
                }
            }
            w0 = j + 1;
        }
    }
    MRBF_HIP(ctx, hipGetLastError());
    if (!single) {
        MRBF_HIP(ctx, hipEventRecord(evEnd, P));
        MRBF_HIP(ctx, hipStreamWaitEvent(S, evEnd, 0));
        MRBF_HIP(ctx, hipEventRecord(evStart, M));
        MRBF_HIP(ctx, hipStreamWaitEvent(S, evStart, 0));
    }
    return 0;
}

constexpr int BS_LD = 65;
template <int KB>
__device__ __forceinline__ void tile_tdot(const double *__restrict__ Tl, int64_t ldt, const double *xs ,
                                          double *res , double *stage ,
                                          double *part ) {
    const int tid = threadIdx.x, c = tid & 127, g = tid >> 7;
    double acc[KB];
#pragma unroll
    for (int l = 0; l < KB; ++l) acc[l] = 0.0;
    for (int h = 0; h < 2; ++h) {
        double v[32];
#pragma unroll
        for (int p = 0; p < 32; ++p) v[p] = Tl[(int64_t)(p * 4 + (tid >> 6)) * ldt + 64 * h + (tid & 63)];
        __syncthreads();
#pragma unroll
        for (int p = 0; p < 32; ++p) stage[(p * 4 + (tid >> 6)) * BS_LD + (tid & 63)] = v[p];
        __syncthreads();
#pragma unroll 8
        for (int r = 0; r < 32; ++r) {
            const double t = stage[c * BS_LD + 32 * g + r];
#pragma unroll
            for (int l = 0; l < KB; ++l) acc[l] = fma(t, xs[l * CNB + 64 * h + 32 * g + r], acc[l]);
        }
    }
#pragma unroll
    for (int l = 0; l < KB; ++l) part[l * 256 + tid] = acc[l];
    __syncthreads();
    if (g == 0) {
#pragma unroll
        for (int l = 0; l < KB; ++l) res[l * CNB + c] = part[l * 256 + c] + part[l * 256 + 128 + c];
    }
}

template <int KB>
__global__ __launch_bounds__(256) void chol_backsolve_kernel(const double *__restrict__ L, int64_t lda, const double *__restrict__ linv_all,
                                                             double *__restrict__ Y, int64_t ldy, int k0, int i ,
                                                             int prologue) {
    __shared__ double xs[KB * CNB];
    __shared__ double res[KB * CNB];
    __shared__ double part[KB * 256];
    __shared__ double stage[CNB * BS_LD];
    const int tid = threadIdx.x;
    const int j = blockIdx.x;
    if (!prologue) {
        for (int t = tid; t < KB * CNB; t += 256) xs[t] = Y[(int64_t)(k0 + t / CNB) * ldy + (int64_t)i * CNB + (t % CNB)];
        __syncthreads();
        tile_tdot<KB>(L + (int64_t)i * CNB + (int64_t)j * CNB * lda, lda, xs, res, stage, part);
        __syncthreads();
        for (int t = tid; t < KB * CNB; t += 256) {
            double *yp = Y + (int64_t)(k0 + t / CNB) * ldy + (int64_t)j * CNB + (t % CNB);
            const double v = *yp - res[t];
            *yp = v;
            xs[t] = v;
        }
        if (j != i - 1) return;
        __syncthreads();
// ... 34 lines not shown
```

morbit.jl_amd/csrc/chol_mega.hip:

```cpp
#include <chrono>

#include "chol_diag_core.hpp"
#include "common.hpp"
#include "mega_gemm.hpp"

namespace mrbf {

typedef double v4d __attribute__((ext_vector_type(4)));
typedef double v2d __attribute__((ext_vector_type(2)));

namespace mega {

constexpr int WIN_DEFAULT = 4;

enum { JOB_U = 0, JOB_T = 1, JOB_P = 2, JOB_S = 3, JOB_UH = 4 };
struct Job {
    short kind, i, c, w;
};
enum { CTL_QP = 0, CTL_ABORT = 32, CTL_TIMEOUT = 64, CTL_PCOLS = 96, CTL_QC = 128, CTL_TS = 144 , CTL_WORDS = 160 };
constexpr int QSTRIDE = 32;
__host__ __device__ inline int wstart(int w, int first, int win) { return w <= 0 ? 0 : first + win * (w - 1); }
__host__ __device__ inline int nbulk_updates(int i, int c, int slack, int slack_chain, int first, int win, int srows = 2) {
    const int t = c - ((i - c <= srows) ? slack_chain : slack);
    return t < first ? 0 : (t - first) / win + 1;
// ... 1099 lines not shown
        if (ctx->mega_tables.size() >= 8) {
            MRBF_HIP(ctx, hipStreamSynchronize(ctx->stream));
            size_t lru = 0;
            for (size_t t = 1; t < ctx->mega_tables.size(); ++t)
                if (ctx->mega_tables[t].stamp < ctx->mega_tables[lru].stamp) lru = t;
            (void)hipFree(ctx->mega_tables[lru].block);
            ctx->mega_tables.erase(ctx->mega_tables.begin() + lru);
        }
        MegaTables t{};
        t.nt = NT;
        t.mt = MT;
        t.params = tp;
        t.npanel = (int)pj.size();
        t.nbulk = (int)bj.size();
        t.nchainjobs = (int)cj.size();
        t.nwin = ((int)wqs.size() - 1) / 2;
        const size_t job_bytes = (pj.size() + bj.size() + cj.size() + 1) * sizeof(Job), wq_bytes = wqs.size() * sizeof(int);
        const size_t wq_off = (job_bytes + 255) & ~size_t(255);
        MRBF_HIP(ctx, hipMalloc(&t.block, wq_off + wq_bytes));
        std::vector<char> img(wq_off + wq_bytes, 0);
        Job *hj = (Job *)img.data();
        std::copy(pj.begin(), pj.end(), hj);
        std::copy(bj.begin(), bj.end(), hj + pj.size());
        std::copy(cj.begin(), cj.end(), hj + pj.size() + bj.size());
        std::memcpy(img.data() + wq_off, wqs.data(), wq_bytes);
        MRBF_HIP(ctx, hipMemcpy(t.block, img.data(), img.size(), hipMemcpyHostToDevice));
        t.jobs = t.block;
        t.wq = (char *)t.block + wq_off;
        ctx->mega_tables.push_back(t);
        tab = &ctx->mega_tables.back();
    }
    tab->stamp = ++ctx->mega_table_clock;
    Job *dj = (Job *)tab->jobs;
    a.pjobs = dj;
    a.npanel = tab->npanel;
    a.bjobs = dj + tab->npanel;
    a.nbulk = tab->nbulk;
    a.cjobs = dj + tab->npanel + tab->nbulk;
    a.nchainjobs = tab->nchainjobs;
    a.nwin = tab->nwin;
    a.wq_start = (int *)tab->wq;
    const size_t nfl = ((size_t)CTL_WORDS + (size_t)QSTRIDE * (2 * a.nwin + 1) + (size_t)QSTRIDE * 512 + (size_t)QSTRIDE * (1 + 2 * plan.srows_max) * NT + 2 * (size_t)MT * NT + 3) / 4 * 4;
    unsigned *fl;
    MRBF_TRY(get_buf(ctx, S_MEGA_FLAGS, nfl, &fl));
    hnow();
    MRBF_HIP(ctx, hipMemsetAsync(fl, 0, nfl * sizeof(unsigned), ctx->stream));
    hnow();
    if (!opt.info_clean) MRBF_HIP(ctx, hipMemsetAsync(dinfo, 0, sizeof(int), ctx->stream));
    hnow();
    a.ctl = fl;
    a.wq_head = fl + CTL_WORDS;
    a.quiet = a.wq_head + (size_t)QSTRIDE * (2 * a.nwin + 1);
    a.dprog = a.quiet + (size_t)QSTRIDE * 512;
    a.sprog = a.dprog + (size_t)QSTRIDE * NT;
    a.tdone = a.sprog + (size_t)QSTRIDE * 2 * plan.srows_max * NT;
    a.ucnt = a.tdone + (size_t)MT * NT;
    a.info = dinfo;
    a.nchain = plan.nchain;
    a.ndedicated = plan.ndedicated;
    a.look = plan.look;
    a.use_quiet = plan.use_quiet;
    a.slack = tp.slack;
    a.slack_chain = tp.slack_chain;
    a.first = tp.first;
    a.win = tp.win;
    a.wbias = plan.wbias;
    a.srows = tp.srows;
    a.edge = tp.edge;
    a.cboost = plan.cboost;
    a.head_job1 = plan.head_job1;
    a.reserve_job0 = plan.reserve_job0;
    a.nreserve = plan.nreserve;
    a.panel_dma = plan.panel_dma;
    a.pstream = plan.pstream;
    a.xchain = plan.xchain;
    a.quiet_tail = plan.quiet_tail;
    a.spin_ticks = (unsigned long long)std::max(1, ctx->spin_ms) * 100000ull;
    a.fault = (ctx->debug_fault & 1) && MT > 1;
    const int grid = plan.grid;
    const char *trace_path = mrbf_env("MRBF_MEGA_TRACE");
    if (trace_path) {
        a.trace_dbg = mrbf_env("MRBF_MEGA_TRACE_WAVE") ? 12 + 16 * (atoi(mrbf_env("MRBF_MEGA_TRACE_WAVE")) & 3) : 4;
        MRBF_TRY(get_buf(ctx, S_MEGA_TRACE, (size_t)NT * 80 + 4 * 1024, &a.trace));
        MRBF_HIP(ctx, hipMemsetAsync(a.trace, 0, ((size_t)NT * 80 + 4 * 1024) * sizeof(unsigned long long), ctx->stream));
    }
    const char *jlog_path = mrbf_env("MRBF_MEGA_JLOG");
    if (jlog_path) {
        a.jlog_cap = a.npanel + a.nbulk + a.nchainjobs + 16;
        MRBF_TRY(get_buf(ctx, S_MEGA_JLOG, (size_t)8 * a.jlog_cap + 16, &a.jlog));
        MRBF_HIP(ctx, hipMemsetAsync(a.jlog, 0, ((size_t)8 * a.jlog_cap + 16) * sizeof(unsigned long long), ctx->stream));
    }
    hipLaunchKernelGGL(potrf_mega_kernel, dim3((unsigned)grid), dim3(256), 0, ctx->stream, a);
    hnow();
    if (jlog_path) {
        std::vector<unsigned long long> h((size_t)8 * a.jlog_cap + 16);
        MRBF_HIP(ctx, hipStreamSynchronize(ctx->stream));
        MRBF_HIP(ctx, hipMemcpy(h.data(), a.jlog, h.size() * sizeof(unsigned long long), hipMemcpyDeviceToHost));
        if (FILE *f = fopen(jlog_path, "w")) {
            const unsigned long long n = std::min<unsigned long long>(h[0], (unsigned long long)a.jlog_cap);
            unsigned long long t0 = ~0ull;
            for (unsigned long long j = 0; j < n; ++j) t0 = std::min(t0, h[8 + 8 * j + 1]);
            for (unsigned long long j = 0; j < n; ++j) {
                const unsigned long long *r = &h[8 + 8 * j];
                fprintf(f, "%llu %llu %llu %llu %llu", r[0] & 0xff, (r[0] >> 8) & 0xffff, (r[0] >> 24) & 0xffff, (r[0] >> 40) & 0xfff, r[0] >> 52);
                for (int k = 1; k < 8; ++k) fprintf(f, " %.2f", r[k] ? (double)(r[k] - t0) * 0.01 : -1.0);
                fprintf(f, "\n");
            }
            fclose(f);
        }
    }
    MRBF_HIP(ctx, hipGetLastError());
    if (trace_path) {
        std::vector<unsigned long long> h((size_t)NT * 2 * 8);
        MRBF_HIP(ctx, hipStreamSynchronize(ctx->stream));
        MRBF_HIP(ctx, hipMemcpy(h.data(), a.trace, h.size() * sizeof(unsigned long long), hipMemcpyDeviceToHost));
        if (FILE *f = fopen(trace_path, "w")) {
            const unsigned long long t0 = h[0];
            for (int c = 0; c < NT; ++c) {
                fprintf(f, "%d", c);
                for (int k = 0; k < 8; ++k) fprintf(f, " %.2f", h[(size_t)c * 16 + k] ? (double)(h[(size_t)c * 16 + k] - t0) * 0.01 : -1.0);
                for (int k = 8; k < 15; ++k) fprintf(f, " %.0f", (double)h[(size_t)c * 16 + k]);
                fprintf(f, " %.2f", h[(size_t)c * 16 + 15] ? (double)(h[(size_t)c * 16 + 15] - t0) * 0.01 : -1.0);
                fprintf(f, "\n");
            }
            std::vector<unsigned long long> u(4 * 1024);
            (void)hipMemcpy(u.data(), a.trace + (size_t)NT * 16, u.size() * sizeof(unsigned long long), hipMemcpyDeviceToHost);
            double tb = 0, tp = 0;
            unsigned long long nb = 0, np = 0;
            for (int g = 0; g < grid && g < 1024; ++g) {
                tb += (double)u[4 * g] * 0.01;
                tp += (double)u[4 * g + 1] * 0.01;
                nb += u[4 * g + 2];
                np += u[4 * g + 3];
            }
            {
                std::vector<unsigned long long> ss((size_t)NT * 64);
                (void)hipMemcpy(ss.data(), a.trace + (size_t)NT * 16 + 4 * 1024, ss.size() * sizeof(unsigned long long), hipMemcpyDeviceToHost);
                for (int c2 = 0; c2 < NT; ++c2) {
                    fprintf(f, "#S %d", c2);
                    for (int k2 = 0; k2 < 64; ++k2) {
                        if ((k2 & 7) > 5) continue;
                        fprintf(f, " %.2f", ss[(size_t)c2 * 64 + k2] ? (double)(ss[(size_t)c2 * 64 + k2] - t0) * 0.01 : -1.0);
                    }
                    fprintf(f, "\n");
                }
            }
            fprintf(f, "# util: bulk %.1f us over %llu jobs (%.1f us/job), panel %.1f us over %llu jobs (%.1f us/job), grid %d\n", tb, nb,
                    nb ? tb / nb : 0.0, tp, np, np ? tp / np : 0.0, grid);
            fclose(f);
        }
    }
    unsigned long long *dstat;
    MRBF_TRY(get_buf(ctx, S_MEGA_STAT, (size_t)2, &dstat));
    hipLaunchKernelGGL(mega_status_kernel, dim3(1), dim3(1), 0, ctx->stream, (const unsigned *)fl, dinfo, dstat);
    ctx->mega_stat_dev = dstat;
    ctx->mega_stat_shape = (long)NT * 100000 + MT;
    ctx->mega_stat_pending = 1;
    hnow();
    if (host_trace_ms > 0.0 && nh == 6 && hstamp[5] - hstamp[0] > host_trace_ms)
        fprintf(stderr, "potrf_mega_tall host trace (NT %d): buffers/tables %.3f ms | memset flags %.3f | memset info %.3f | kernel launch %.3f | status launch %.3f\n", NT,
                hstamp[1] - hstamp[0], hstamp[2] - hstamp[1], hstamp[3] - hstamp[2], hstamp[4] - hstamp[3], hstamp[5] - hstamp[4]);
    if (mrbf_env("MRBF_MEGA_DEBUG")) {
        unsigned h[CTL_WORDS];
        MRBF_HIP(ctx, hipStreamSynchronize(ctx->stream));
        MRBF_HIP(ctx, hipMemcpy(h, fl, sizeof(h), hipMemcpyDeviceToHost));
        if (h[CTL_TIMEOUT]) {
            const long off = (long)h[CTL_TIMEOUT + 1];
            const long t0 = a.tdone - a.ctl, u0 = a.ucnt - a.ctl, d0 = a.dprog - a.ctl, s0 = a.sprog - a.ctl;
            fprintf(stderr, "mega timeout code 0x%x word %ld want %u: ", h[CTL_TIMEOUT], off, h[CTL_TIMEOUT + 2]);
            if (off >= u0) fprintf(stderr, "ucnt[%ld][%ld]", (off - u0) / NT, (off - u0) % NT);
            else if (off >= t0) fprintf(stderr, "tdone[%ld][%ld]", (off - t0) / NT, (off - t0) % NT);
            else if (off >= s0) fprintf(stderr, "sprog[%ld][%ld]", (off - s0) / QSTRIDE / NT, (off - s0) / QSTRIDE % NT);
            else if (off >= d0) fprintf(stderr, "dprog[%ld]", (off - d0) / QSTRIDE);
            fprintf(stderr, "  (NT %d MT %d pcols %u qpanel %u/%d qchain %u/%d)\n", NT, MT, h[CTL_PCOLS], h[CTL_QP], a.npanel, h[CTL_QC], a.nchainjobs);
        }
    }
    MRBF_HIP(ctx, hipGetLastError());
    return 0;
}

}

static int32_t check_mega_tables(int nt, int mt, const mrbf::mega::TableParams &p, int64_t *out) {
    using namespace mrbf;
    using namespace mrbf::mega;
    std::vector<Job> pj, bj, cj;
    std::vector<int> wqs;
    build_job_tables(nt, mt, p, pj, bj, cj, wqs);
    const int slack = p.slack, slack_chain = p.slack_chain, first = p.first, win = p.win, srows = p.srows;
    const bool chainq = p.chainq != 0;
    const Edge &edge = p.edge;
    int64_t bad = 0;
    auto sr = [&](int c) { return srows_at(c, srows, edge); };
    std::vector<int> fin((size_t)mt * nt, 0);
    for (const Job &j : cj) {
        if (j.i < j.c || j.i >= mt || j.c >= nt) {
            ++bad;
            continue;
        }
        fin[(size_t)j.i * nt + j.c] += (j.kind == JOB_S && j.w != 0) ? 1 : 2;
        if (j.kind == JOB_P ? j.i != j.c : (j.kind != JOB_S || j.i <= j.c || j.i > j.c + sr(j.c) || j.w < 0 || j.w > 2 ||
                                            (j.w != 0) != shalf_at(j.c, srows, edge)))
            ++bad;
    }
    for (const Job &j : pj) {
        const bool xh = xhalf_at(j.i, nt, edge);
        if (j.kind != JOB_T || j.c >= nt || j.i <= j.c + sr(j.c) || j.i >= mt || j.w < 0 || j.w > 3 || (j.w == 3) != xh ||
            (!xh && (j.w == 2) != tfull_at(j.i, j.c, srows, edge))) {
            ++bad;
            continue;
        }
        fin[(size_t)j.i * nt + j.c] += j.w >= 2 ? 2 : 1;
    }
    for (int c = 0; c < nt; ++c)
        for (int i = 0; i < mt; ++i) bad += fin[(size_t)i * nt + c] != (i >= c ? 2 : 0);
    const int nwin = ((int)wqs.size() - 1) / 2;
    std::vector<int> upd((size_t)mt * nt, 0);
    for (int w = 0; w < nwin; ++w) {
        std::fill(upd.begin(), upd.end(), 0);
        for (int cls = 0; cls < 2; ++cls) {
            int last_c = -1;
            for (int q = wqs[cls * nwin + w]; q < wqs[cls * nwin + w + 1]; ++q) {
                const Job &j = bj[q];
                if (j.i < j.c || j.i >= mt || j.c >= nt || (j.w & 255) != w || (j.kind != JOB_U && j.kind != JOB_UH)) {
                    ++bad;
                    continue;
                }
                if (j.c < last_c) ++bad;
                last_c = j.c;
                if (j.c < wstart(w + 1, first, win)) ++bad;
                if (((j.i - j.c <= sr(j.c)) && chainq) != (cls == 1)) ++bad;
                const int hcode = j.w >> 8;
                if (j.kind == JOB_U ? hcode != 0 : (hcode > 2 || (hcode == 2) != xhalf_at(j.i, nt, edge))) ++bad;
                if (j.kind == JOB_U && xhalf_at(j.i, nt, edge)) ++bad;
                upd[(size_t)j.i * nt + j.c] += (j.kind == JOB_U || hcode == 2) ? 2 : 1;
            }
        }
        for (int c = 0; c < nt; ++c)
            for (int i = c; i < mt; ++i) bad += upd[(size_t)i * nt + c] != (w < nbulk_updates(i, c, slack, slack_chain, first, win, sr(c)) ? 2 : 0);
    }
    for (size_t w = 0; w + 1 < wqs.size(); ++w) bad += wqs[w] > wqs[w + 1];
    int64_t sum = 0;
    int64_t pos = 1;
    for (const std::vector<Job> *v : {&pj, &bj, &cj})
        for (const Job &j : *v) sum += (pos++) * (int64_t)(1 + j.kind + 7 * j.i + 131 * j.c + 1009 * j.w);
    out[0] = (int64_t)pj.size();
    out[1] = (int64_t)bj.size();
    out[2] = (int64_t)cj.size();
    out[3] = nwin;
    out[4] = sum;
    out[5] = bad;
    return 0;
}

extern "C" int32_t mrbf_debug_mega_tables(int32_t nt, int32_t mt, int32_t slack, int32_t slack_chain, int32_t first, int32_t win, int32_t srows,
                                          int32_t half_cols, int64_t *out) {
    if (nt < 1 || mt < nt || mt > 32000) return -1;
    if (slack < 1 || slack_chain < slack || win < 1 || first < 1 || first > win || srows < 0 || half_cols < 0) return -3;
    if (!out) return -9;
    const mrbf::mega::Edge no_edge{0, nt, srows, 1, 0};
    return check_mega_tables(nt, mt, mrbf::mega::TableParams{slack, slack_chain, first, win, srows, half_cols, 0, 0, 0, no_edge}, out);
}

extern "C" int32_t mrbf_debug_mega_tables2(int32_t nt, int32_t mt, int32_t slack, int32_t slack_chain, int32_t first, int32_t win, int32_t srows,
                                           int32_t half_cols, const int32_t *opt5, int64_t *out) {
    if (nt < 1 || mt < nt || mt > 32000) return -1;
    if (slack < 1 || slack_chain < slack || win < 1 || first < 1 || first > win || srows < 0 || half_cols < 0) return -3;
    if (!opt5) return -9;
    if (!out) return -10;
    if (opt5[0] < 0 || opt5[1] < 0 || opt5[2] < 0 || opt5[3] < 0) return -9;
    mrbf::mega::Edge edge{};
    edge.srows_edge = std::max(srows, 5);
    edge.pstream_edge = 2;
    edge.head = srows < edge.srows_edge ? std::min(opt5[0], nt) : 0;
    edge.tail_c0 = srows < edge.srows_edge ? std::max(edge.head, nt - opt5[1]) : nt;
    edge.shalf = (opt5[4] & 2) ? 1 : 0;
    edge.sh_head = (opt5[4] >> 2) & 0xff;
    edge.sh_tail_c0 = ((opt5[4] >> 10) & 0xff) ? std::max(edge.sh_head, nt - ((opt5[4] >> 10) & 0xff)) : (edge.sh_head ? nt : 0);
    edge.xhalf = (opt5[4] >> 26) & 1;
    edge.tfull1 = (opt5[4] >> 18) & 0xff;
    return check_mega_tables(nt, mt, mrbf::mega::TableParams{slack, slack_chain, first, win, srows, half_cols, opt5[2], opt5[3] > 0 ? opt5[3] : 1000, opt5[4] & 1, edge}, out);
}

extern "C" int32_t mrbf_debug_mega_plan(int32_t nt, int32_t mt, int32_t xreal, int64_t *out) {
    if (nt < 1 || mt < nt || mt > 32000) return -1;
    if (xreal < 0) return -3;
    if (!out) return -4;
    const mrbf::mega::Plan p = mrbf::mega::plan_for(nt, mt, mrbf::mega::Knobs{}, xreal);
    const mrbf::mega::TableParams &t = p.tp;
    const mrbf::mega::Edge &e = t.edge;
    const int v[33] = {t.slack, t.slack_chain, t.first, t.win, t.srows, t.half_cols, t.tail_half, t.tail_half_w, t.chainq,
                       e.head, e.tail_c0, e.srows_edge, e.pstream_edge, e.shalf, e.sh_head, e.sh_tail_c0, e.tfull1, e.xhalf,
                       p.nchain, p.ndedicated, p.nreserve, p.head_job1, p.reserve_job0, p.xchain, p.quiet_tail, p.pstream, p.look, p.use_quiet,
                       p.wbias, p.cboost, p.panel_dma, p.grid, p.srows_max};
    for (int i = 0; i < 33; ++i) out[i] = v[i];
    return check_mega_tables(nt, mt, t, out + 33);
}
```

morbit.jl_amd/csrc/common.hpp:

```cpp
#pragma once
#include <hip/hip_runtime.h>
#include <rocblas/rocblas.h>
#include <rocsolver/rocsolver.h>

#include <cmath>
#include <cstdlib>
#include <cstdint>
#include <cstdio>
#include <cstring>
#include <map>
#include <string>
#include <vector>

#include "../../include/mrbf.h"
#include "model_pool.hpp"

namespace mrbf {

struct KP {
    int kid;
    double a, b;
    double a2;
    double sgn;
    int fast;
    int ik;
    double phi0;
};
KP make_kp(int kid, double a, double b);
int cpd_order(int kid, double a, double b);
inline int poly_dim(int d, int deg) { return deg < 0 ? 0 : (deg == 0 ? 1 : d + 1); }

enum Slot {
    S_XC = 0, S_SQ, S_MEAN, S_PHI, S_PI, S_Q1, S_W1, S_G, S_R, S_TAU, S_RHS, S_T1, S_T2, S_IPIV, S_INFO,
    S_STAGE_A, S_STAGE_B, S_STAGE_C, S_STAGE_D, S_EVAL_E, S_EVAL_A, S_EVAL_J, S_EVAL_SA, S_EVAL_XC, S_EVAL_XSQ,
    S_OUT_A, S_OUT_B, S_CHOL_WS, S_MISC, S_MEGA_JOBS, S_MEGA_FLAGS, S_MEGA_WQ, S_MEGA_IT, S_BSOLVE_FLAGS, S_MEGA_TRACE, S_MEGA_JLOG,
    S_T1W, S_PS_STATE, S_PS_STAT, S_PS_POLISH, S_BSOLVE_X, S_V0, S_QR_INV, S_DIAG_SCR, S_SMALL_WS, S_SMALL_DESC, S_SMALL_FLAGS, S_MEGA_STAT, S_BSOLVE_M, S_SMALL_CL, S_GW_PART, S_GW_RS, S_GW_GP, S_GW_M, S_CHECK_SCAL, S_TAIL_PART, S_PS_RANK, S_SD_IN, S_SD_OUT, S_SD_WS, S_NS_IN, S_NS_OUT, S_NS_WS, S_SD_STEP, S_SD_BATCH, S_AFF_BATCH, S_NS_BATCH, S_R4_BATCH, S_NSLOTS
};
}

namespace mrbf {
namespace mega {
struct Edge {
    int head, tail_c0, srows_edge, pstream_edge;
    int shalf, sh_head, sh_tail_c0;
    int tfull1;
    int xhalf;
};
struct TableParams {
    int slack, slack_chain, first, win, srows, half_cols, tail_half, tail_half_w, chainq;
    Edge edge;
};
constexpr bool operator==(const TableParams &a, const TableParams &b) {
    return a.slack == b.slack && a.slack_chain == b.slack_chain && a.first == b.first && a.win == b.win && a.srows == b.srows &&
           a.half_cols == b.half_cols && a.tail_half == b.tail_half && a.tail_half_w == b.tail_half_w && a.chainq == b.chainq &&
           a.edge.head == b.edge.head && a.edge.tail_c0 == b.edge.tail_c0 && a.edge.srows_edge == b.edge.srows_edge &&
           a.edge.pstream_edge == b.edge.pstream_edge && a.edge.shalf == b.edge.shalf && a.edge.sh_head == b.edge.sh_head &&
           a.edge.sh_tail_c0 == b.edge.sh_tail_c0 && a.edge.tfull1 == b.edge.tfull1 && a.edge.xhalf == b.edge.xhalf;
}
struct Knobs {
    int grid = 512, dedicated = 64, look = 2, quiet = 1, slack = 3, half_cols = 0, first_window = 1, wbias = 4, xhalf = 1, chainq = 0, cboost = 12, panel_dma = 1;
    int min = 256, max = 32768;
    int chain = 0, slack_chain = 0, win = 0, pstream = 0, srows = 0;
    int shalf = -1, shalf_head = -1, head = -1, tail = -1, reserve = -1, tail_half = -1, tail_half_w = -1, xchain = -1, quiet_tail = -1;
    int tfull = -1;
};
}
struct MegaTables {
    int nt, mt;
    mega::TableParams params;
    void *block, *jobs, *wq;
    int npanel, nbulk, nchainjobs, nwin;
    unsigned long long stamp;
};
struct PotrfOpts {
    int impl = 0;
    bool any_size = false;
    int xreal = 0;
    bool info_clean = false;
};
struct EvalHints {
    bool population = false;
    bool check_call = false;
    const double *pre_xq = nullptr;
};
}

struct mrbf_ctx {
    int device = 0;
    int ncu = 256;
    hipStream_t own_stream = nullptr;
    hipStream_t stream = nullptr;
    rocblas_handle blas = nullptr;
    mrbf::Buf slots[mrbf::S_NSLOTS];
    hipEvent_t ev[8] = {};
    hipStream_t panel_stream = nullptr;
    hipEvent_t evx[4] = {};
    hipStream_t bulk_stream = nullptr;
    int bulk_masked = 0;
    int bulk_grid = 384;
    mrbf::mega::Knobs mega;
    std::string err;
    std::vector<mrbf::Buf> model_pool;
    int gram_mode = 0, residual = 1, force_path = 0, chol_impl = 0, eval_impl = 0, timing = 1, diag_impl = 0, chol_window = 0;
    int spin_ms = 1000, debug_fault = 0;
    unsigned long long *mega_stat_dev = nullptr;
    long mega_stat_shape = 0;
    int mega_stat_pending = 0;
    char *pin_base = nullptr;
    size_t pin_off = 0;
    bool pin_armed = false;
    struct PinOut {
        void *user;
        const void *pin;
        size_t bytes;
    };
    std::vector<PinOut> pin_out;
    unsigned long long *hpin = nullptr;
    float last_device_ms = 0.f;
    int slow_launches = 0;
    int small_nc = 4;
    int small_cluster_ok = 0;
    int small_timeouts = 0;
    int live_models = 0, live_round4 = 0;
    unsigned ps_rank_epoch = 0;
    int ps_multi_off = 0;
    std::map<long, float> mega_best_ms;
    std::vector<mrbf::MegaTables> mega_tables;
    unsigned long long mega_table_clock = 0;
};

struct mrbf_model {
    int64_t n = 0, npad = 0;
    int d = 0, dpad = 0, k = 0, q = 0, deg = -1;
    mrbf::KP kp{};
    double *C = nullptr;
    double *Xc = nullptr;
    double *sq = nullptr;
    double *mean = nullptr;
    double *W = nullptr;
    double *Wc = nullptr;
    double *lam = nullptr;
    void *block = nullptr;
    size_t block_bytes = 0;
    mrbf::ModelSlab *slab = nullptr;
};

namespace mrbf {

int fail(mrbf_ctx *ctx, int code, const char *fmt, ...);
#define MRBF_HIP(ctx, call)                                                                                  \
    do {                                                                                                      \
        hipError_t e__ = (call);                                                                              \
        if (e__ != hipSuccess)                                                                                \
            return mrbf::fail(ctx, e__ == hipErrorOutOfMemory ? MRBF_ENOMEM : MRBF_EHIP, "%s: %s (%s:%d)", #call, \
                              hipGetErrorString(e__), __FILE__, __LINE__);                                    \
    } while (0)
#define MRBF_BLAS(ctx, call)                                                                                 \
    do {                                                                                                      \
        rocblas_status s__ = (call);                                                                          \
        if (s__ != rocblas_status_success)                                                                    \
            return mrbf::fail(ctx, MRBF_EBLAS, "%s: rocblas status %d (%s:%d)", #call, (int)s__, __FILE__, __LINE__); \
    } while (0)
#define MRBF_TRY(call)             \
    do {                           \
        int rc__ = (call);         \
        if (rc__ != 0) return rc__; \
    } while (0)

int get_buf(mrbf_ctx *ctx, Slot s, size_t bytes, void **out);
template <class T>
inline int get_buf(mrbf_ctx *ctx, Slot s, size_t count, T **out) {
    return get_buf(ctx, s, count * sizeof(T), (void **)out);
}
bool is_device_ptr(const void *p);
int stage_in(mrbf_ctx *ctx, Slot s, const double *user, size_t count, const double **dev);
int stage_out(mrbf_ctx *ctx, Slot s, double *user, size_t count, double **dev);
int finish_out(mrbf_ctx *ctx, double *user, const double *dev, size_t count);
void pin_reset(mrbf_ctx *ctx);
void pin_flush(mrbf_ctx *ctx);
void pin_discard(mrbf_ctx *ctx);
char *pin_take(mrbf_ctx *ctx, size_t bytes);
struct PinGuard {
    mrbf_ctx *ctx;
    bool flushed = false;
    explicit PinGuard(mrbf_ctx *c) : ctx(c) { pin_reset(c); }
    void flush() {
        pin_flush(ctx);
        flushed = true;
    }
    ~PinGuard() {
        if (!flushed) pin_discard(ctx);
    }
    PinGuard(const PinGuard &) = delete;
    PinGuard &operator=(const PinGuard &) = delete;
};
enum HpinSlot : int {
    HPIN_FIT_FLAGS = 0,
    HPIN_FIT_SCAL = 4,
    HPIN_SMALL_FLAGS = 8,
    HPIN_SMALL_SCAL = 12,
    HPIN_SMALL_CHK = 16,
    HPIN_RESIDUAL = 20,
    HPIN_R4_COUNT = 24,
    HPIN_MEGA_STAT = 63,
};

inline int64_t round_up(int64_t x, int64_t m) { return (x + m - 1) / m * m; }

inline const char *mrbf_env(const char *name) {
    const char *gate = std::getenv("MRBF_EXPERIMENTS");
    if (!gate || std::atoi(gate) == 0) return nullptr;
    return std::getenv(name);
}

int launch_center_pad(mrbf_ctx *ctx, const double *X, int64_t n, int d, const double *mean_or_null, double *mean_out,
                      double *Xc, int64_t npad, int dpad, double *sq);
int launch_poly_matrix(mrbf_ctx *ctx, const double *C, int64_t n, int d, int q, double *Pi, int64_t ldpi);
int launch_transpose(mrbf_ctx *ctx, const double *in, int64_t rows, int64_t cols, double *out);
int launch_gram(mrbf_ctx *ctx, int mode, const double *C, const double *Xc, const double *sq, int64_t n, int64_t npad,
                int d, int dpad, const KP &kp, double *Phi, int64_t ld);
int launch_cross_gram(mrbf_ctx *ctx, const double *X, int64_t m, const double *C, int64_t n, int d, const KP &kp, double *K);
bool gram_w_applies(const mrbf_ctx *ctx, const mrbf_model *M);
int launch_gram_w(mrbf_ctx *ctx, const mrbf_model *M, double *Phi, int64_t ld, double **Wpart_out, double **rspart_out, int *nseg_out);
int launch_projection_small(mrbf_ctx *ctx, const mrbf_model *M, const double *Wpart, const double *rspart, int nseg, const double *linv,
                            const double *Q1, double *W1, double *G, double *scal, int *flags, int K2, int skip, double *PA, double *PB,
                            double *v0);
int eval_model(mrbf_ctx *ctx, const mrbf_model *M, int64_t m, const double *Xdev, double *vals_dev, double *jac_dev,
               mrbf_eval_info *info, EvalHints hints = {});
int potrf_blocked_tall(mrbf_ctx *ctx, int64_t ncols, int64_t mrows, double *A, int64_t lda, int *dinfo, double *linv_all, PotrfOpts opt = {});
int potrf_mega_tall(mrbf_ctx *ctx, int64_t ncols, int64_t mrows, double *A, int64_t lda, int *dinfo, double *linv_all, PotrfOpts opt = {});
mega::Knobs mega_knobs_from_env();
int potrf_lower(mrbf_ctx *ctx, int impl, int64_t n, double *A, int64_t lda, int *info_host);
int fit_model(mrbf_ctx *ctx, mrbf_model *M, const double *Ydev, mrbf_fit_info *info);
int build_model_shell(mrbf_ctx *ctx, int64_t n, int d, int k, const double *Cdev, int kid, double a, double b, int deg,
                      mrbf_model **out);
void destroy_model(mrbf_ctx *ctx, mrbf_model *M);
void model_set_dims(mrbf_model *M, int64_t n, int d, int k, int kid, double a, double b, int deg);
size_t model_block_layout(const mrbf_model *M, size_t off[7]);
void model_carve(mrbf_model *M, char *base, const size_t off[7]);
int model_block_acquire(mrbf_ctx *ctx, size_t total, void **p, size_t *bytes);
void model_block_release(mrbf_ctx *ctx, void *p, size_t bytes, bool slab = false);
int fit_check(mrbf_ctx *ctx, mrbf_model *M, const double *Y, mrbf_fit_info *info);
int mega_collect_stat(mrbf_ctx *ctx);
int mega_stat_enqueue(mrbf_ctx *ctx);
int mega_stat_finish(mrbf_ctx *ctx);

}
```

morbit.jl_amd/csrc/small.hip:

```cpp
#include "chol_diag_core.hpp"
#include "radial.hpp"
#include "small.hpp"

#include <utility>

namespace mrbf {
namespace smallfit {

typedef double v4d __attribute__((ext_vector_type(4)));

__device__ __forceinline__ double phi_rt(double s, const KP &p) {
    switch (p.kid) {
        case MRBF_CUBIC: return p.fast ? rbf_phi_t<MRBF_CUBIC, true>(s, p) : rbf_phi_t<MRBF_CUBIC, false>(s, p);
        case MRBF_INV_MULTIQUADRIC: return p.fast ? rbf_phi_t<MRBF_INV_MULTIQUADRIC, true>(s, p) : rbf_phi_t<MRBF_INV_MULTIQUADRIC, false>(s, p);
        case MRBF_MULTIQUADRIC: return p.fast ? rbf_phi_t<MRBF_MULTIQUADRIC, true>(s, p) : rbf_phi_t<MRBF_MULTIQUADRIC, false>(s, p);
        case MRBF_THIN_PLATE_SPLINE: return rbf_phi_t<MRBF_THIN_PLATE_SPLINE, false>(s, p);
        default: return rbf_phi_t<MRBF_GAUSSIAN, false>(s, p);
    }
}

typedef __attribute__((address_space(1))) double gdbl;
__device__ __forceinline__ void gst(double *p, double v) { *(gdbl *)p = v; }
__device__ __forceinline__ double gld(const double *p) { return *(const gdbl *)p; }

// ... 550 lines not shown
        }
        if (q > 1) {
            const int d16 = (d + 15) & ~15;
            for (int e = tid + 256 * member; e < 128 * 128; e += 256 * nc) Gx[e] = (e % 128 == e / 128 && e % 128 >= d) ? 1.0 : 0.0;
            MRBF_CLB();
            wg_gemm<false, true, true>(d16, d16, n16, P.Xc, dpad, P.Xc, dpad, NoPre(), [&](int a, int b, double v, double) {
                if (a < d && b < d) gst(&Gx[a + b * 128], v);
            }, member, nc);
            MRBF_CLB();
            if (member == 0) {
                const int bad = diag_block_auto(Gx, 128, d, LinvX, sh);
                __syncthreads();
                if (tid == 0 && bad) P.flags[1] = bad;
            }
            MRBF_CLB();
            double *Qx = Q1 + np;
            wg_gemm<true, true, false>(n16, d16, d16, P.Xc, dpad, LinvX, 128, NoPre(), [&](int i, int a, double v, double) {
                if (i < n && a < d) gst(&Qx[i + (int64_t)a * np], v);
            }, member, nc);
        }
        MRBF_CLB();
        MRBF_STAMP();
        wg_gemm<false, false, false>(n16, q16, n16, Phi, np, Q1, np, NoPre(), [&](int i, int t, double v, double) { gst(&Wm[i + (int64_t)t * np], v); },
                                     member, nc);
        for (int e = tid + 256 * member; e < (np - n16) * q16; e += 256 * nc) Wm[n16 + e % (np - n16) + (int64_t)(e / (np - n16)) * np] = 0.0;
        MRBF_CLB();
        wg_gemm<true, false, false>(q16, q16, n16, Q1, np, Wm, np, NoPre(), [&](int a, int b, double v, double) { gst(&G[a + b * q16], v); }, member, nc);
        MRBF_CLB();
        double tr = 0.0;
        for (int t = tid; t < q; t += 256) tr += gld(&G[t + t * q16]);
        tr = wg_sum(tr, red);
        const double mu_raw = ((double)n * P.kp.phi0 - tr) / (double)max(n - q, 1);
        const bool mu_ok = mu_raw > 0.0 && mu_raw < 1e300;
        const double mu = mu_ok ? mu_raw : 1.0;
        if (tid == 0 && member == 0) {
            P.scal[0] = tr;
            P.scal[1] = mu;
            if (!mu_ok) P.flags[2] = 1;
        }
        wg_gemm<false, false, false>(n16, q16, q16, Q1, np, G, q16, [&](int i, int t) { return gld(&Wm[i + (int64_t)t * np]); },
                                     [&](int i, int t, double v, double o) { gst(&Wm[i + (int64_t)t * np], o - 0.5 * v); }, member, nc);
        MRBF_CLB();
        {
            const double hmu = -0.5 * mu;
            batched_pass(np * q16, [&](int e) { return fma(hmu, gld(&Q1[e]), gld(&Wm[e])); }, [&](int e, double v) { gst(&V[e], v); }, member, nc);
        }
        MRBF_CLB();
        MRBF_STAMP();
        wg_gemm<false, true, true>(n16, n16, q16, Q1, np, V, np, [&](int i, int j) { return gld(&Phi[i + (int64_t)j * np]); },
                                   [&](int i, int j, double v, double o) { gst(&Phi[i + (int64_t)j * np], o - v); }, member, nc);
        __syncthreads();
        wg_gemm<false, true, true>(n16, n16, q16, V, np, Q1, np, [&](int i, int j) { return gld(&Phi[i + (int64_t)j * np]); },
                                   [&](int i, int j, double v, double o) { gst(&Phi[i + (int64_t)j * np], o - v); }, member, nc);
        MRBF_STAMP();
        wg_gemm<true, false, false>(q16, 16, n16, Q1, np, Yc, np, NoPre(), [&](int a, int l, double v, double) { gst(&T1[a + l * ldz], v); }, member, nc);
        batched_pass(np * 16, [&](int e) { return gld(&Yc[e]); }, [&](int e, double v) { gst(&Bm[e], v); }, member, nc);
        MRBF_CLB();
        wg_gemm<false, false, false>(n16, 16, q16, Q1, np, T1, ldz, [&](int i, int l) { return gld(&Bm[i + l * np]); },
                                     [&](int i, int l, double v, double o) { gst(&Bm[i + l * np], o - v); }, member, nc);
    } else {
        batched_pass(np * 16, [&](int e) { return gld(&Yc[e]); }, [&](int e, double v) { gst(&Bm[e], v); }, member, nc);
        if (tid == 0 && member == 0) {
            P.scal[0] = 0.0;
            P.scal[1] = 0.0;
        }
    }
    MRBF_CLB();

    MRBF_STAMP();
    {
        const int bad = wg_potrf(Phi, np, np, n16, Linv, Pt, sh, cl, P.diag6);
        if (bad) {
            if (tid == 0 && (member == 0 || bad < 0)) P.flags[bad > 0 ? 0 : 3] = bad > 0 ? bad : 1;
            return;
        }
        if (member != 0) return;
    }
    __syncthreads();
    MRBF_STAMP();
    const int nb = np / 128;
    for (int c = 0; c < nb; ++c) {
        if (c > 0) {
            wg_gemm<false, false, false>(128, 16, 128 * c, Phi + 128 * c, np, Fy, np, [&](int i, int l) { return gld(&Bm[128 * c + i + l * np]); },
                                         [&](int i, int l, double v, double o) { gst(&Bm[128 * c + i + l * np], o - v); });
            __syncthreads();
        }
        wg_gemm<false, false, false>(128, 16, 128, Linv + (int64_t)c * 128 * 128, 128, Bm + 128 * c, np, NoPre(),
                                     [&](int i, int l, double v, double) { gst(&Fy[128 * c + i + l * np], v); });
        __syncthreads();
    }
    for (int c = nb - 1; c >= 0; --c) {
        const int rest = np - 128 * (c + 1);
        if (rest > 0) {
            wg_gemm<true, false, false>(128, 16, rest, Phi + 128 * (c + 1) + (int64_t)128 * c * np, np, Xs + 128 * (c + 1), np,
                                        [&](int i, int l) { return gld(&Fy[128 * c + i + l * np]); },
                                        [&](int i, int l, double v, double o) { gst(&Fy[128 * c + i + l * np], o - v); });
            __syncthreads();
        }
        wg_gemm<true, false, false>(128, 16, 128, Linv + (int64_t)c * 128 * 128, 128, Fy + 128 * c, np, NoPre(),
                                    [&](int i, int l, double v, double) { gst(&Xs[128 * c + i + l * np], v); });
        __syncthreads();
    }
    MRBF_STAMP();
    if (q > 0) {
        wg_gemm<true, false, false>(q16, 16, n16, Q1, np, Xs, np, NoPre(), [&](int a, int l, double v, double) { gst(&T2[a + l * ldz], v); });
        __syncthreads();
        wg_gemm<false, false, false>(n16, 16, q16, Q1, np, T2, ldz, [&](int i, int l) { return gld(&Xs[i + l * np]); },
                                     [&](int i, int l, double v, double o) { gst(&Xs[i + l * np], o - v); });
        __syncthreads();
        wg_gemm<true, false, false>(q16, 16, n16, Wm, np, Xs, np, [&](int a, int l) { return gld(&T1[a + l * ldz]); },
                                    [&](int a, int l, double v, double o) { gst(&Z[a + l * ldz], o - v); });
        for (int e = tid; e < 16 * 16; e += 256) Z[q16 + e % 16 + (e / 16) * ldz] = 0.0;
        __syncthreads();
        if (q > 1) {
            const int d16 = (d + 15) & ~15;
            wg_gemm<true, false, false>(d16, 16, d16, LinvX, 128, Z + 1, ldz, NoPre(), [&](int a, int l, double v, double) { gst(&T2[1 + a + l * ldz], v); });
            __syncthreads();
        }
        for (int l = wave; l < k; l += 4) {
            double acc = 0.0;
            for (int t = 1 + lane; t < q; t += 64) acc = fma(s_mean[t - 1], T2[t + l * ldz], acc);
            for (int off = 32; off > 0; off >>= 1) acc += __shfl_xor(acc, off);
            if (lane == 0) P.lam[l] = Z[l * ldz] * rsn - acc;
        }
        for (int e = tid; e < (q - 1) * k; e += 256) {
            const int t = 1 + e / k, l = e % k;
            P.lam[(int64_t)t * k + l] = T2[t + l * ldz];
        }
    }
    MRBF_STAMP();
    for (int e = tid; e < np * k; e += 256) {
        const int i = e % np, l = e / np;
        const double v = i < n ? Xs[i + l * np] : 0.0;
        P.Wc[e] = v;
        if (i < n) P.W[(int64_t)i * k + l] = v;
    }
}

struct TailQ {
    const double *Xc, *Y;
    int n, npad, d, dpad, q, k;
    int np, rows;
    double *part;
    double *Gx, *LinvX;
    double *T1;
    double *Q1, *B;
    double *rows_out;
    int64_t ld;
    int xt;
    int *flags;
    double rsn;
};
constexpr int TQ_PS = 4096 + 1024 + 16;

__global__ __launch_bounds__(256) void tailq_gram_kernel(TailQ t) {
    __shared__ double red[4];
    __shared__ double part4[4][64];
    const int tid = threadIdx.x, p = blockIdx.x;
    const int n16 = (t.n + 15) & ~15, d16 = (t.d + 15) & ~15;
    const int r0 = p * t.rows, r1 = min(r0 + t.rows, n16), K = max(r1 - r0, 0);
    double *out = t.part + (size_t)p * TQ_PS;
    const double *X0 = t.Xc + (int64_t)r0 * t.dpad;
    if (K > 0) {
        wg_gemm<false, true, true>(d16, d16, K, X0, t.dpad, X0, t.dpad, NoPre(), [&](int a, int b, double v, double) { gst(&out[a + 64 * b], v); });
    } else {
        for (int e = tid; e < 4096; e += 256) gst(&out[e], 0.0);
    }
    const int c = tid & 63, g = tid >> 6;
    const int rend = min(r1, t.n);
    for (int l = 0; l < t.k; ++l) {
        double s = 0.0, sy = 0.0;
        for (int i0 = r0 + g; i0 < rend; i0 += 32) {
            double xv[8], yv[8];
#pragma unroll
            for (int u = 0; u < 8; ++u) {
                const int i = i0 + 4 * u < rend ? i0 + 4 * u : i0;
                xv[u] = gld(&X0[(int64_t)(i - r0) * t.dpad + c]);
                yv[u] = gld(&t.Y[(int64_t)i * t.k + l]);
            }
#pragma unroll
            for (int u = 0; u < 8; ++u)
                if (i0 + 4 * u < rend) {
                    s = fma(xv[u], yv[u], s);
                    sy += yv[u];
                }
        }
        __syncthreads();
        part4[g][c] = s;
        if (c == 0) red[g] = sy;
        __syncthreads();
        if (g == 0) gst(&out[4096 + c + 64 * l], (part4[0][c] + part4[1][c]) + (part4[2][c] + part4[3][c]));
        if (tid == 0) gst(&out[4096 + 1024 + l], (red[0] + red[1]) + (red[2] + red[3]));
    }
}

__global__ __launch_bounds__(256) void tailq_factor_kernel(TailQ t) {
    __shared__ double colbuf[2 * 128];
    __shared__ double Li[64 * 65];
    __shared__ double xty[64 * 16 + 16];
    const int tid = threadIdx.x, d = t.d, i = tid & 63, w = tid >> 6;
    __builtin_amdgcn_s_setprio(3);
    double g[16], e[16];
#pragma unroll
    for (int u = 0; u < 16; ++u) g[u] = 0.0;
    for (int p0 = 0; p0 < t.np; p0 += 4) {
        double x[4][16];
#pragma unroll
        for (int p = 0; p < 4; ++p)
#pragma unroll
            for (int u = 0; u < 16; ++u) {
                const int j = 4 * u + w;
                x[p][u] = (p0 + p < t.np && i < d && j <= i) ? gld(&t.part[(size_t)(p0 + p) * TQ_PS + i + 64 * j]) : 0.0;
            }
#pragma unroll
        for (int p = 0; p < 4; ++p)
#pragma unroll
            for (int u = 0; u < 16; ++u) g[u] += x[p][u];
    }
#pragma unroll
    for (int u = 0; u < 16; ++u) {
        const int j = 4 * u + w;
        if (!(i < d && j <= i)) g[u] = i == j ? 1.0 : 0.0;
        e[u] = i == j ? 1.0 : 0.0;
    }
    for (int idx = tid; idx < 64 * t.k + t.k; idx += 256) {
        const int src = idx < 64 * t.k ? 4096 + idx : 4096 + 1024 + (idx - 64 * t.k);
        double v = 0.0;
        for (int p0 = 0; p0 < t.np; p0 += 16) {
            double x[16];
#pragma unroll
            for (int p = 0; p < 16; ++p) x[p] = p0 + p < t.np ? gld(&t.part[(size_t)(p0 + p) * TQ_PS + src]) : 0.0;
#pragma unroll
            for (int p = 0; p < 16; ++p) v += x[p];
        }
        xty[idx < 64 * t.k ? idx : 64 * 16 + (idx - 64 * t.k)] = v;
    }
    const int bad = chol64_regs(g, e, d, colbuf);
    if (tid == 0) t.flags[1] = bad;
#pragma unroll
    for (int u = 0; u < 16; ++u) {
        const int j = 4 * u + w;
        Li[j * 65 + i] = (j < d && i <= j) ? e[u] : 0.0;
    }
    __syncthreads();
    for (int idx = tid; idx < 128 * 128; idx += 256) {
        const int a = idx & 127, b = idx >> 7;
        gst(&t.LinvX[idx], (a < d && b < d) ? Li[a * 65 + b] : (a == b ? 1.0 : 0.0));
    }
    for (int idx = tid; idx < t.q * t.k; idx += 256) {
        const int a = idx % t.q, l = idx / t.q;
        double v;
        if (a == 0) {
            v = xty[64 * 16 + l] * t.rsn;
        } else {
            v = 0.0;
            for (int b = 0; b < a; ++b) v = fma(Li[(a - 1) * 65 + b], xty[b + 64 * l], v);
        }
        gst(&t.T1[a + (int64_t)l * t.q], v);
    }
}

__global__ __launch_bounds__(256) void tailq_q1_kernel(TailQ t) {
    __shared__ double Qs[64 * 65];
    __shared__ double part4[4][64];
    const int tid = threadIdx.x, d = t.d, d16 = (t.d + 15) & ~15;
    const int R0 = 64 * blockIdx.x;
    for (int e = tid; e < 64 * 65; e += 256) Qs[e] = 0.0;
    __syncthreads();
    wg_gemm<true, true, false>(64, d16, d16, t.Xc + (int64_t)R0 * t.dpad, t.dpad, t.LinvX, 128, NoPre(), [&](int i, int a, double v, double) {
        if (a < d) {
            const double w = R0 + i < t.n ? v : 0.0;
            Qs[a * 65 + i] = w;
            gst(&t.Q1[(R0 + i) + (int64_t)(1 + a) * t.npad], w);
        }
    });
    if (tid < 64) gst(&t.Q1[R0 + tid], R0 + tid < t.n ? t.rsn : 0.0);
    __syncthreads();
    const int i = tid & 63, g = tid >> 6;
    for (int l = 0; l < t.k; ++l) {
        double s = 0.0;
        for (int a = g; a < d; a += 4) s = fma(Qs[a * 65 + i], gld(&t.T1[1 + a + (int64_t)l * t.q]), s);
        __syncthreads();
        part4[g][i] = s;
        __syncthreads();
        if (g == 0) {
            double b = 0.0;
            if (R0 + i < t.n)
                b = gld(&t.Y[(int64_t)(R0 + i) * t.k + l]) - fma(t.rsn, gld(&t.T1[(int64_t)l * t.q]), (part4[0][i] + part4[1][i]) + (part4[2][i] + part4[3][i]));
            gst(&t.B[(R0 + i) + (int64_t)l * t.npad], b);
            if (t.rows_out) gst(&t.rows_out[(t.npad + l) + (int64_t)(R0 + i) * t.ld], b);
        }
    }
    if (t.rows_out)
        for (int e = tid; e < 64 * t.xt; e += 256) {
            const int l = e % t.xt, r = e / t.xt;
            if (l >= t.k) gst(&t.rows_out[(t.npad + l) + (int64_t)(R0 + r) * t.ld], 0.0);
        }
}

}

bool small_fit_applies(const mrbf_ctx *ctx, int64_t n, int d, int k, int q, int path) {
    static const int off = mrbf_env("MRBF_SMALL_FIT") ? atoi(mrbf_env("MRBF_SMALL_FIT")) == 0 : 0;
    if (off || ctx->chol_impl == 1 || ctx->gram_mode == 1) return false;
    return n >= 1 && n <= 512 && d >= 1 && d <= 128 && k >= 1 && k <= 16 && n > q && (path == MRBF_PATH_CHOL || path == MRBF_PATH_PROJ_CHOL);
}

int small_fit_cluster(const mrbf_ctx *ctx, int count) {
    static const int env = mrbf_env("MRBF_SMALL_NC") ? atoi(mrbf_env("MRBF_SMALL_NC")) : 0;
    if (env == 1 || ctx->small_nc == 1 || !ctx->small_cluster_ok) return 1;
    const int groups = (std::max(count, 1) + 7) / 8;
    int nc = 1;
    while (2 * nc <= smallfit::MAX_CLUSTER && 8 * groups * 2 * nc <= ctx->ncu) nc *= 2;
    if (env > 1) nc = std::min(env, smallfit::MAX_CLUSTER);
    int p2 = 1;
    while (2 * p2 <= nc) p2 *= 2;
    return p2;
}

int launch_small_fit(mrbf_ctx *ctx, const smallfit::Prob *host_probs, int count, const smallfit::Prob *dev_probs, int nc) {
    if (count <= 0) return 0;
    const unsigned grid = nc == 1 ? (unsigned)count : 8u * (unsigned)nc * (unsigned)((count + 7) / 8);
    hipLaunchKernelGGL(smallfit::small_fit_kernel, dim3(grid), dim3(256), 0, ctx->stream, host_probs[0],
                       (count == 1 && !dev_probs) ? (const smallfit::Prob *)nullptr : dev_probs, count, nc);
    MRBF_HIP(ctx, hipGetLastError());
    return 0;
}

int launch_small_means(mrbf_ctx *ctx, const smallfit::Prob *dev_probs, int count) {
    if (count <= 0) return 0;
    hipLaunchKernelGGL(smallfit::small_mean_kernel, dim3((unsigned)count), dim3(256), 0, ctx->stream, dev_probs, count);
    MRBF_HIP(ctx, hipGetLastError());
    return 0;
}

bool tail_basis_applies(const mrbf_model *M) {
    static const int on = mrbf_env("MRBF_TAILQ") ? atoi(mrbf_env("MRBF_TAILQ")) : 1;
    return on && M->dpad == 64 && M->d >= 1 && M->d <= 64 && M->q == M->d + 1 && M->k >= 1 && M->k <= 16 && M->npad % 64 == 0;
}
int launch_tail_basis(mrbf_ctx *ctx, const mrbf_model *M, const double *Y, double *scratch, double *LinvX, double *T1, double *Q1, double *B,
                      double *rows_out, int64_t ld, int xt, int *flags) {
    smallfit::TailQ t;
    t.Xc = M->Xc;
    t.Y = Y;
    t.n = (int)M->n;
    t.npad = (int)M->npad;
    t.d = M->d;
    t.dpad = M->dpad;
    t.q = M->q;
    t.k = M->k;
    const int n16 = (t.n + 15) & ~15;
    t.np = std::min(32, std::max(4, t.n / 128));
    t.rows = ((n16 + t.np - 1) / t.np + 15) & ~15;
    t.Gx = scratch;
    t.part = scratch + 128 * 128;
    t.LinvX = LinvX;
    t.T1 = T1;
    t.Q1 = Q1;
    t.B = B;
    t.rows_out = rows_out;
    t.ld = ld;
    t.xt = xt;
    t.flags = flags;
    t.rsn = 1.0 / std::sqrt((double)M->n);
    hipLaunchKernelGGL(smallfit::tailq_gram_kernel, dim3((unsigned)t.np), dim3(256), 0, ctx->stream, t);
    hipLaunchKernelGGL(smallfit::tailq_factor_kernel, dim3(1), dim3(256), 0, ctx->stream, t);
    hipLaunchKernelGGL(smallfit::tailq_q1_kernel, dim3((unsigned)(M->npad / 64)), dim3(256), 0, ctx->stream, t);
    MRBF_HIP(ctx, hipGetLastError());
    return 0;
}
size_t tail_basis_scratch_doubles() { return (size_t)128 * 128 + (size_t)32 * smallfit::TQ_PS; }

}
```

morbit.jl_amd/csrc/solve.hip:

```cpp
#include "common.hpp"
#include "small.hpp"

namespace mrbf {

__global__ void fit_publish_kernel(const int *__restrict__ dinfo, const double *__restrict__ scal, const unsigned long long *__restrict__ dstat,
                                   int *__restrict__ hflags, double *__restrict__ hscal, unsigned long long *__restrict__ hstat) {
    const int t = threadIdx.x;
    if (t < 4) hflags[t] = dinfo[t];
    if (t >= 4 && t < 6 && scal) hscal[t - 4] = scal[t - 4];
    if (t == 6 && dstat && hstat) hstat[0] = dstat[0];
}

__global__ void fill_saddle_kernel(const double *__restrict__ Pi, int64_t n, int q, double *__restrict__ S, int64_t N) {
    const int64_t idx = (int64_t)blockIdx.x * blockDim.x + threadIdx.x;
    const int64_t tot = n * q;
    if (idx < tot) {
        const int64_t i = idx % n;
        const int t = (int)(idx / n);
        const double v = Pi[idx];
        S[i + (n + t) * N] = v;
        S[(n + t) + i * N] = v;
    } else if (idx < tot + (int64_t)q * q) {
        const int64_t r = idx - tot;
        S[(n + r % q) + (n + r / q) * N] = 0.0;
    }
}

__global__ void rhs_from_values_kernel(const double *__restrict__ Y, int64_t n, int k, double *__restrict__ B, int64_t N) {
    const int64_t idx = (int64_t)blockIdx.x * blockDim.x + threadIdx.x;
    if (idx >= N * k) return;
    const int64_t i = idx % N;
    const int l = (int)(idx / N);
    B[idx] = (i < n) ? Y[i * k + l] : 0.0;
}

__global__ void scatter_solution_kernel(const double *__restrict__ B, int64_t ldB, int64_t n, int64_t npad, int k, int q,
                                        int64_t lam_row0, double *__restrict__ W, double *__restrict__ Wc,
                                        double *__restrict__ lam, const double *__restrict__ lamsrc, int64_t ldlam) {
    const int64_t idx = (int64_t)blockIdx.x * blockDim.x + threadIdx.x;
    if (idx < npad * k) {
        const int64_t i = idx % npad;
        const int l = (int)(idx / npad);
        const double v = (i < n) ? B[i + l * ldB] : 0.0;
        Wc[idx] = v;
        if (i < n) W[i * k + l] = v;
    } else if (idx < npad * k + (int64_t)q * k) {
        const int64_t r = idx - npad * k;
        const int t = (int)(r % q), l = (int)(r / q);
        lam[(int64_t)t * k + l] = lamsrc[lam_row0 + t + l * ldlam];
    }
}

__global__ void copy_upper_kernel(const double *__restrict__ A, int64_t lda, int q, double *__restrict__ R) {
    const int idx = blockIdx.x * blockDim.x + threadIdx.x;
    if (idx >= q * q) return;
    const int i = idx % q, j = idx / q;
    R[idx] = (i <= j) ? A[i + (int64_t)j * lda] : 0.0;
}

__global__ void trace_kernel(const double *__restrict__ G, int q, double *__restrict__ out) {
    __shared__ double red[256];
    double s = 0.0;
    for (int i = threadIdx.x; i < q; i += 256) s += G[i + (int64_t)i * q];
    red[threadIdx.x] = s;
    __syncthreads();
    for (int w = 128; w > 0; w >>= 1) {
        if ((int)threadIdx.x < w) red[threadIdx.x] += red[threadIdx.x + w];
        __syncthreads();
    }
    if (threadIdx.x == 0) out[0] = red[0];
}

__global__ void max_abs_kernel(const double *__restrict__ v, int64_t cnt, double *__restrict__ out) {
    __shared__ double red[256];
    double s = 0.0;
    for (int64_t i = threadIdx.x; i < cnt; i += 256) s = fmax(s, fabs(v[i]));
    red[threadIdx.x] = s;
    __syncthreads();
    for (int w = 128; w > 0; w >>= 1) {
        if ((int)threadIdx.x < w) red[threadIdx.x] = fmax(red[threadIdx.x], red[threadIdx.x + w]);
        __syncthreads();
    }
    if (threadIdx.x == 0) out[0] = red[0];
}

__global__ void residual_kernel(const double *__restrict__ a, const double *__restrict__ b, int64_t cnt,
                                double *__restrict__ out) {
    __shared__ double r0[256], r1[256];
    double s0 = 0.0, s1 = 0.0;
    for (int64_t i = threadIdx.x; i < cnt; i += 256) {
        const double df = a[i] - b[i];
        s0 = fma(df, df, s0);
        s1 = fma(b[i], b[i], s1);
    }
    r0[threadIdx.x] = s0;
    r1[threadIdx.x] = s1;
    __syncthreads();
    for (int w = 128; w > 0; w >>= 1) {
        if ((int)threadIdx.x < w) {
            r0[threadIdx.x] += r0[threadIdx.x + w];
            r1[threadIdx.x] += r1[threadIdx.x + w];
        }
        __syncthreads();
    }
    if (threadIdx.x == 0) {
        out[0] = r0[0];
        out[1] = r1[0];
    }
}

static inline unsigned nblk(int64_t cnt) { return (unsigned)((cnt + 255) / 256); }

void model_block_release(mrbf_ctx *ctx, void *p, size_t bytes, bool slab) {
    if (!ctx) {
        (void)hipFree(p);
        return;
    }
    model_pool_release(ctx->model_pool, p, bytes, slab, [](void *q) { (void)hipFree(q); });
}

void destroy_model(mrbf_ctx *ctx, mrbf_model *M) {
    if (!M) return;
    if (ctx && (M->block || M->slab)) --ctx->live_models;
    if (M->block) model_block_release(ctx, M->block, M->block_bytes);
    if (M->slab && slab_drop(M->slab)) {
        model_block_release(ctx, M->slab->p, M->slab->bytes, true);
        delete M->slab;
    }
    delete M;
}

void model_set_dims(mrbf_model *M, int64_t n, int d, int k, int kid, double a, double b, int deg) {
    M->n = n;
    M->d = d;
    M->k = k;
    M->deg = deg;
    M->q = poly_dim(d, deg);
    M->npad = round_up(n, 128);
    M->dpad = (d <= 64) ? 64 : (d <= 128 ? 128 : (d <= 256 ? 256 : (int)round_up(d, 16)));
    M->kp = make_kp(kid, a, b);
}

size_t model_block_layout(const mrbf_model *M, size_t off[7]) {
    const size_t cnt[7] = {(size_t)M->n * M->d, (size_t)M->npad * M->dpad, (size_t)M->npad, (size_t)M->dpad, (size_t)M->n * M->k,
                           (size_t)M->npad * M->k, (size_t)std::max(M->q, 1) * M->k};
    size_t at = 0;
    for (int i = 0; i < 7; ++i) {
        off[i] = at;
        at += (std::max<size_t>(cnt[i], 2) * sizeof(double) + 255) & ~size_t(255);
    }
    return at;
}

void model_carve(mrbf_model *M, char *base, const size_t off[7]) {
    M->C = (double *)(base + off[0]);
    M->Xc = (double *)(base + off[1]);
    M->sq = (double *)(base + off[2]);
    M->mean = (double *)(base + off[3]);
    M->W = (double *)(base + off[4]);
    M->Wc = (double *)(base + off[5]);
    M->lam = (double *)(base + off[6]);
}

int model_block_acquire(mrbf_ctx *ctx, size_t total, void **p, size_t *bytes) {
    hipError_t e = hipSuccess;
    auto alloc = [&](size_t b) -> void * {
        void *q = nullptr;
        e = hipMalloc(&q, b);
        return e == hipSuccess ? q : nullptr;
    };
    if (!model_pool_acquire(ctx->model_pool, total, p, bytes, alloc, [](void *q) { (void)hipFree(q); }))
        return fail(ctx, MRBF_ENOMEM, "model allocation failed: %s", hipGetErrorString(e));
    return 0;
}

int build_model_shell(mrbf_ctx *ctx, int64_t n, int d, int k, const double *Cdev, int kid, double a, double b, int deg,
                      mrbf_model **out) {
    mrbf_model *M = new mrbf_model();
    model_set_dims(M, n, d, k, kid, a, b, deg);
    size_t off[7];
    const size_t total = model_block_layout(M, off);
    const int rc_block = model_block_acquire(ctx, total, &M->block, &M->block_bytes);
    if (rc_block != 0) {
        delete M;
        return rc_block;
    }
    ++ctx->live_models;
    model_carve(M, (char *)M->block, off);
    auto init = [&]() -> int {
        if (Cdev != M->C)
            MRBF_HIP(ctx, hipMemcpyAsync(M->C, Cdev, (size_t)n * d * sizeof(double), hipMemcpyDeviceToDevice, ctx->stream));
        MRBF_TRY(launch_center_pad(ctx, M->C, n, d, nullptr, M->mean, M->Xc, M->npad, M->dpad, M->sq));
        return 0;
    };
    const int rc = init();
    if (rc != 0) {
        destroy_model(ctx, M);
        return rc;
    }
    *out = M;
    return 0;
}

static int read_info(mrbf_ctx *ctx, const int *dinfo, int *hinfo) {
    MRBF_HIP(ctx, hipMemcpyAsync(hinfo, dinfo, sizeof(int), hipMemcpyDeviceToHost, ctx->stream));
    MRBF_HIP(ctx, hipStreamSynchronize(ctx->stream));
    return 0;
}

static int fit_lu(mrbf_ctx *ctx, mrbf_model *M, const double *Y, mrbf_fit_info *info) {
    const int64_t n = M->n, N = n + M->q;
    const int k = M->k, q = M->q;
    double *S, *B, *Pi = nullptr;
    int *ipiv, *dinfo;
    MRBF_TRY(get_buf(ctx, S_PHI, (size_t)N * N, &S));
    MRBF_TRY(get_buf(ctx, S_RHS, (size_t)N * k, &B));
    MRBF_TRY(get_buf(ctx, S_IPIV, (size_t)N, &ipiv));
    MRBF_TRY(get_buf(ctx, S_INFO, (size_t)4, &dinfo));
    hipLaunchKernelGGL(rhs_from_values_kernel, dim3(nblk(N * k)), dim3(256), 0, ctx->stream, Y, n, k, B, N);
    MRBF_HIP(ctx, hipEventRecord(ctx->ev[0], ctx->stream));
    MRBF_TRY(launch_gram(ctx, ctx->gram_mode, M->C, M->Xc, M->sq, n, M->npad, M->d, M->dpad, M->kp, S, N));
    MRBF_HIP(ctx, hipEventRecord(ctx->ev[1], ctx->stream));
    if (q > 0) {
        MRBF_TRY(get_buf(ctx, S_PI, (size_t)n * q, &Pi));
        MRBF_TRY(launch_poly_matrix(ctx, M->C, n, M->d, q, Pi, n));
        hipLaunchKernelGGL(fill_saddle_kernel, dim3(nblk(n * q + (int64_t)q * q)), dim3(256), 0, ctx->stream, Pi, n, q, S, N);
    }
    MRBF_HIP(ctx, hipGetLastError());
    MRBF_HIP(ctx, hipEventRecord(ctx->ev[5], ctx->stream));
    MRBF_BLAS(ctx, rocsolver_dgetrf(ctx->blas, (int)N, (int)N, S, (int)N, ipiv, dinfo));
    MRBF_HIP(ctx, hipEventRecord(ctx->ev[2], ctx->stream));
    int hinfo = 0;
    MRBF_TRY(read_info(ctx, dinfo, &hinfo));
    info->factor_info = hinfo;
    info->path = MRBF_PATH_LU;
    if (hinfo != 0) return fail(ctx, MRBF_ESINGULAR, "saddle matrix is singular (getrf info = %d, N = %lld)", hinfo, (long long)N);
    MRBF_BLAS(ctx, rocsolver_dgetrs(ctx->blas, rocblas_operation_none, (int)N, k, S, (int)N, ipiv, B, (int)N));
    hipLaunchKernelGGL(scatter_solution_kernel, dim3(nblk(M->npad * k + (int64_t)q * k)), dim3(256), 0, ctx->stream, B, N, n,
                       M->npad, k, q, n, M->W, M->Wc, M->lam, B, N);
    MRBF_HIP(ctx, hipGetLastError());
    MRBF_HIP(ctx, hipEventRecord(ctx->ev[3], ctx->stream));
    MRBF_HIP(ctx, hipEventSynchronize(ctx->ev[3]));
    MRBF_HIP(ctx, hipEventElapsedTime(&info->ms_gram, ctx->ev[0], ctx->ev[1]));
    MRBF_HIP(ctx, hipEventElapsedTime(&info->ms_project, ctx->ev[1], ctx->ev[5]));
    MRBF_HIP(ctx, hipEventElapsedTime(&info->ms_factor, ctx->ev[5], ctx->ev[2]));
    MRBF_HIP(ctx, hipEventElapsedTime(&info->ms_solve, ctx->ev[2], ctx->ev[3]));
    return 0;
}

__global__ void scale_rows_pinv_kernel(double *__restrict__ T, int N, int k, const double *__restrict__ sv) {
    const int idx = blockIdx.x * blockDim.x + threadIdx.x;
    if (idx >= N * k) return;
    const int i = idx % N;
    const double s = sv[i], cut = (double)N * 2.220446049250313e-16 * sv[0];
    T[idx] = (s > cut) ? T[idx] / s : 0.0;
}

static int fit_minnorm(mrbf_ctx *ctx, mrbf_model *M, const double *Y, mrbf_fit_info *info) {
    const int64_t n = M->n, N = n + M->q;
    const int k = M->k, q = M->q;
    const double one = 1.0, zero = 0.0;
    double *S, *B, *Pi, *U, *VT, *sv, *E, *T;
    int *dinfo;
    MRBF_TRY(get_buf(ctx, S_PHI, (size_t)N * N, &S));
    MRBF_TRY(get_buf(ctx, S_RHS, (size_t)N * k, &B));
    MRBF_TRY(get_buf(ctx, S_PI, (size_t)n * q, &Pi));
    MRBF_TRY(get_buf(ctx, S_Q1, (size_t)N * N, &U));
    MRBF_TRY(get_buf(ctx, S_W1, (size_t)N * N, &VT));
    MRBF_TRY(get_buf(ctx, S_TAU, (size_t)2 * N, &sv));
    MRBF_TRY(get_buf(ctx, S_T1, (size_t)N * k, &T));
    MRBF_TRY(get_buf(ctx, S_INFO, (size_t)4, &dinfo));
    E = sv + N;
    hipLaunchKernelGGL(rhs_from_values_kernel, dim3(nblk(N * k)), dim3(256), 0, ctx->stream, Y, n, k, B, N);
    MRBF_HIP(ctx, hipEventRecord(ctx->ev[0], ctx->stream));
    MRBF_TRY(launch_gram(ctx, ctx->gram_mode, M->C, M->Xc, M->sq, n, M->npad, M->d, M->dpad, M->kp, S, N));
    MRBF_HIP(ctx, hipEventRecord(ctx->ev[1], ctx->stream));
    MRBF_TRY(launch_poly_matrix(ctx, M->C, n, M->d, q, Pi, n));
    hipLaunchKernelGGL(fill_saddle_kernel, dim3(nblk(n * q + (int64_t)q * q)), dim3(256), 0, ctx->stream, Pi, n, q, S, N);
    MRBF_HIP(ctx, hipGetLastError());
    MRBF_BLAS(ctx, rocsolver_dgesvd(ctx->blas, rocblas_svect_all, rocblas_svect_all, (int)N, (int)N, S, (int)N, sv, U, (int)N, VT,
                                    (int)N, E, rocblas_outofplace, dinfo));
    MRBF_HIP(ctx, hipEventRecord(ctx->ev[2], ctx->stream));
    int hinfo = 0;
    MRBF_TRY(read_info(ctx, dinfo, &hinfo));
    info->factor_info = hinfo;
    info->path = MRBF_PATH_MINNORM;
    if (hinfo != 0) return fail(ctx, MRBF_ESINGULAR, "SVD of the saddle matrix did not converge (info = %d)", hinfo);
    MRBF_BLAS(ctx, rocblas_dgemm(ctx->blas, rocblas_operation_transpose, rocblas_operation_none, (int)N, k, (int)N, &one, U, (int)N,
                                 B, (int)N, &zero, T, (int)N));
    hipLaunchKernelGGL(scale_rows_pinv_kernel, dim3(nblk(N * k)), dim3(256), 0, ctx->stream, T, (int)N, k, sv);
    MRBF_BLAS(ctx, rocblas_dgemm(ctx->blas, rocblas_operation_transpose, rocblas_operation_none, (int)N, k, (int)N, &one, VT, (int)N,
                                 T, (int)N, &zero, B, (int)N));
    hipLaunchKernelGGL(scatter_solution_kernel, dim3(nblk(M->npad * k + (int64_t)q * k)), dim3(256), 0, ctx->stream, B, N, n,
                       M->npad, k, q, n, M->W, M->Wc, M->lam, B, N);
    MRBF_HIP(ctx, hipGetLastError());
    MRBF_HIP(ctx, hipEventRecord(ctx->ev[3], ctx->stream));
    MRBF_HIP(ctx, hipEventSynchronize(ctx->ev[3]));
    MRBF_HIP(ctx, hipEventElapsedTime(&info->ms_gram, ctx->ev[0], ctx->ev[1]));
    MRBF_HIP(ctx, hipEventElapsedTime(&info->ms_factor, ctx->ev[1], ctx->ev[2]));
    MRBF_HIP(ctx, hipEventElapsedTime(&info->ms_solve, ctx->ev[2], ctx->ev[3]));
    return 0;
}

int backsolve_blocked(mrbf_ctx *ctx, int64_t npad, const double *L, int64_t lda, const double *linv_all, double *Y, int64_t ldy, int k);
int backsolve_persistent(mrbf_ctx *ctx, int64_t npad, const double *L, int64_t lda, const double *linv_all, double *Y, int64_t ldy, int k,
                         int *status);
int launch_update_lower(mrbf_ctx *ctx, const double *A, int64_t lda, const double *B, int64_t ldb, double *C, int64_t ldc, int64_t nt, int K,
                        const double *cvec, double cs, int64_t cn);
int launch_pad_identity(mrbf_ctx *ctx, double *A, int64_t n, int64_t npad, int64_t ld);
int tsmm_tn(mrbf_ctx *ctx, int64_t n, int p, int r, double alpha, const double *A, int64_t lda, const double *B, int64_t ldb, double beta,
            double *C, int64_t ldc);
int symm_panel(mrbf_ctx *ctx, int64_t n, int64_t npad, int q, const double *Phi, int64_t ld, const double *Q, int64_t ldq, double *W,
               int64_t ldwo, bool const_first, double cval);

__global__ void set_rhs_rows_kernel(double *__restrict__ A, int64_t ld, int64_t npad, int xt, const double *__restrict__ B, int k) {
    const int64_t idx = (int64_t)blockIdx.x * blockDim.x + threadIdx.x;
    if (idx >= npad * xt) return;
    const int l = (int)(idx % xt);
    const int64_t i = idx / xt;
    A[(npad + l) + i * ld] = (l < k) ? B[i + (int64_t)l * npad] : 0.0;
}
__global__ void get_rhs_rows_kernel(const double *__restrict__ A, int64_t ld, int64_t npad, double *__restrict__ B, int k) {
    const int64_t idx = (int64_t)blockIdx.x * blockDim.x + threadIdx.x;
    if (idx >= npad * k) return;
    const int l = (int)(idx % k);
    const int64_t i = idx / k;
    B[i + (int64_t)l * npad] = A[(npad + l) + i * ld];
}
__global__ void xc_to_tall_kernel(const double *__restrict__ Xc, int64_t n, int d, int dpad, double *__restrict__ Tall, int64_t lt,
                                  int64_t dq) {
    const int64_t idx = (int64_t)blockIdx.x * blockDim.x + threadIdx.x;
    if (idx >= n * d) return;
    const int64_t i = idx / d;
    const int t = (int)(idx % d);
    Tall[(dq + i) + (int64_t)t * lt] = Xc[i * dpad + t];
}
__global__ void build_q1_kernel(const double *__restrict__ Tall, int64_t lt, int64_t dq, int64_t n, int64_t npad, int q,
                                double *__restrict__ Q1) {
    const int64_t idx = (int64_t)blockIdx.x * blockDim.x + threadIdx.x;
    if (idx >= npad * q) return;
    const int64_t i = idx % npad;
    const int t = (int)(idx / npad);
    double v = 0.0;
    if (i < n) v = (t == 0) ? 1.0 / sqrt((double)n) : Tall[(dq + i) + (int64_t)(t - 1) * lt];
    Q1[idx] = v;
}
__global__ void shift_from_trace_kernel(double *__restrict__ scal, double nphi0, double nmq, int *__restrict__ flags) {
    const double mu = (nphi0 - scal[0]) / nmq;
    const bool ok = mu > 0.0 && mu < 1e300;
    scal[1] = ok ? mu : 1.0;
    flags[2] = ok ? 0 : 1;
}

__global__ void build_panels_kernel(const double *__restrict__ Q1, const double *__restrict__ W, const double *__restrict__ scal,
                                    int64_t n, int64_t npad, int q, int K2, int skip, double *__restrict__ PA, double *__restrict__ PB,
                                    double *__restrict__ v0) {
    const int64_t idx = (int64_t)blockIdx.x * blockDim.x + threadIdx.x;
    if (idx >= npad * K2) return;
    const double mu = scal[1];
    const int64_t i = idx % npad;
    const int t = (int)(idx / npad);
    const int qq = q - skip;
    double a = 0.0, b = 0.0;
    if (i < n && t < 2 * qq) {
        const int tt = t % qq + skip;
        const double qv = Q1[i + (int64_t)tt * npad];
        const double vv = fma(-0.5 * mu, qv, W[i + (int64_t)tt * npad]);
        a = (t < qq) ? qv : vv;
        b = (t < qq) ? vv : qv;
    }
    PA[idx] = a;
    PB[idx] = b;
    if (skip && t == 0) v0[i] = (i < n) ? fma(-0.5 * mu, Q1[i], W[i]) : 0.0;
}
__global__ __launch_bounds__(64) void finish_lambda_kernel(double *__restrict__ T1, int q, int k, double sqrtn, const double *__restrict__ mean) {
    __shared__ double part[64];
    const int l = blockIdx.x, tid = threadIdx.x;
    if (l >= k) return;
    double acc = 0.0;
    for (int t = 1 + tid; t < q; t += 64) acc = fma(mean[t - 1], T1[t + (int64_t)l * q], acc);
    part[tid] = acc;
    __syncthreads();
    if (tid == 0) {
        double dsum = 0.0;
        for (int u = 0; u < 64; ++u) dsum += part[u];
        T1[(int64_t)l * q] = T1[(int64_t)l * q] / sqrtn - dsum;
    }
}

__global__ __launch_bounds__(256) void sub_qt_kernel(double *__restrict__ B, int64_t ldb, const double *__restrict__ Q, int64_t ldq,
                                                     const double *__restrict__ T, int64_t n, int q, int k) {
    __shared__ double part[4][64];
    const int r = threadIdx.x & 63, g = threadIdx.x >> 6;
    const int64_t row = (int64_t)blockIdx.x * 64 + r;
    for (int l = 0; l < k; ++l) {
        double s0 = 0.0, s1 = 0.0;
        if (row < n) {
            int t = g;
            for (; t + 4 < q; t += 8) {
                s0 = fma(Q[row + (int64_t)t * ldq], T[t + (int64_t)l * q], s0);
                s1 = fma(Q[row + (int64_t)(t + 4) * ldq], T[t + 4 + (int64_t)l * q], s1);
            }
            if (t < q) s0 = fma(Q[row + (int64_t)t * ldq], T[t + (int64_t)l * q], s0);
        }
        __syncthreads();
        part[g][r] = s0 + s1;
        __syncthreads();
        if (g == 0 && row < n) B[row + (int64_t)l * ldb] -= (part[0][r] + part[1][r]) + (part[2][r] + part[3][r]);
    }
}

__global__ __launch_bounds__(256) void apply_linv_t_kernel(const double *__restrict__ inv, int d, double *__restrict__ X, int64_t ldx, int k) {
    __shared__ double bs[128];
    const int j = threadIdx.x & 127, half = threadIdx.x >> 7;
    __shared__ double part[2][128];
    for (int l = 0; l < k; ++l) {
        __syncthreads();
        if (threadIdx.x < 128) bs[threadIdx.x] = threadIdx.x < d ? X[threadIdx.x + (int64_t)l * ldx] : 0.0;
        __syncthreads();
        double v = 0.0;
        if (j < d) {
            const double *col = inv + (int64_t)j * 128;
            for (int i = j + half; i < d; i += 2) v = fma(col[i], bs[i], v);
        }
        part[half][j] = v;
        __syncthreads();
        if (half == 0 && j < d) X[j + (int64_t)l * ldx] = part[0][j] + part[1][j];
    }
}

__global__ __launch_bounds__(256) void trsm_lt_small_kernel(const double *__restrict__ L, int64_t ldl, int d, double *__restrict__ X,
                                                            int64_t ldx, int k) {
    __shared__ double xs[256];
    const int j = threadIdx.x;
    for (int l = 0; l < k; ++l) {
        double v = j < d ? X[j + (int64_t)l * ldx] : 0.0;
        for (int c = d - 1; c >= 0; --c) {
            if (j == c) {
                v /= L[c + (int64_t)c * ldl];
                xs[c] = v;
            }
            __syncthreads();
            if (j < c) v -= L[c + (int64_t)j * ldl] * xs[c];
            __syncthreads();
        }
        if (j < d) X[j + (int64_t)l * ldx] = v;
    }
}

__global__ __launch_bounds__(256) void tail_dots_kernel(const double *__restrict__ Bw, int64_t ldb, const double *__restrict__ Q1,
                                                        const double *__restrict__ Wm, int64_t ldq, int64_t n, int q, int k,
                                                        double *__restrict__ part) {
    __shared__ double ws[64 * 16];
    __shared__ double red[4][2][64];
    const int tid = threadIdx.x, g = tid >> 6, lane = tid & 63;
    const int64_t R0 = (int64_t)blockIdx.x * 64;
    for (int e = tid; e < 64 * k; e += 256) {
        const int i = e & 63, l = e >> 6;
        ws[e] = R0 + i < n ? Bw[R0 + i + (int64_t)l * ldb] : 0.0;
    }
    __syncthreads();
    for (int a0 = 0; a0 < q; a0 += 64) {
        const int a = a0 + lane;
        double qv[16], wv[16];
#pragma unroll
        for (int u = 0; u < 16; ++u) {
            const int64_t r = R0 + 16 * g + u;
            const bool ok = a < q && r < n;
            qv[u] = ok ? Q1[r + (int64_t)a * ldq] : 0.0;
            wv[u] = ok ? Wm[r + (int64_t)a * ldq] : 0.0;
        }
        for (int l = 0; l < k; ++l) {
            double s0 = 0.0, s1 = 0.0;
#pragma unroll
            for (int u = 0; u < 16; ++u) {
                const double w = ws[l * 64 + 16 * g + u];
                s0 = fma(qv[u], w, s0);
                s1 = fma(wv[u], w, s1);
            }
            __syncthreads();
// ... 65 lines not shown
#pragma unroll
            for (int u = 0; u < 16; ++u) mv[u] = t0 + u < q ? mean[t0 + u - 1] : 0.0;
#pragma unroll
            for (int u = 0; u < 16; ++u) dsum = fma(mv[u], t0 + u < q ? xx[l * q + t0 + u] : 0.0, dsum);
        }
        xx[l * q] = zz[l * q] / sqrtn - dsum;
    }
    __syncthreads();
    for (int e = tid; e < k * q; e += nthr) lam_out[(e % q) + (int64_t)(e / q) * q] = xx[e];
}

__global__ __launch_bounds__(256) void tail_apply_kernel(const double *__restrict__ Bw, int64_t ldb, const double *__restrict__ Q1, int64_t ldq,
                                                         const double *__restrict__ T2, const double *__restrict__ lamsrc, int64_t n,
                                                         int64_t npad, int q, int k, double *__restrict__ W, double *__restrict__ Wc,
                                                         double *__restrict__ lam) {
    __shared__ double part4[4][64];
    const int tid = threadIdx.x, r = tid & 63, g = tid >> 6;
    const int64_t row = (int64_t)blockIdx.x * 64 + r;
    for (int l = 0; l < k; ++l) {
        double s0 = 0.0, s1 = 0.0;
        if (row < n) {
            int t = g;
            for (; t + 4 < q; t += 8) {
                s0 = fma(Q1[row + (int64_t)t * ldq], T2[t + (int64_t)l * q], s0);
                s1 = fma(Q1[row + (int64_t)(t + 4) * ldq], T2[t + 4 + (int64_t)l * q], s1);
            }
            if (t < q) s0 = fma(Q1[row + (int64_t)t * ldq], T2[t + (int64_t)l * q], s0);
        }
        __syncthreads();
        part4[g][r] = s0 + s1;
        __syncthreads();
        if (g == 0 && row < npad) {
            const double v = row < n ? Bw[row + (int64_t)l * ldb] - ((part4[0][r] + part4[1][r]) + (part4[2][r] + part4[3][r])) : 0.0;
            Wc[row + (int64_t)l * npad] = v;
            if (row < n) W[row * k + l] = v;
        }
    }
    if (blockIdx.x == 0)
        for (int e = tid; e < q * k; e += 256) lam[(int64_t)(e % q) * k + e / q] = lamsrc[(e % q) + (int64_t)(e / q) * q];
}

static int fit_chol(mrbf_ctx *ctx, mrbf_model *M, const double *Y, mrbf_fit_info *info, int *not_pd, int *gave_up, int impl = 0) {
    const int64_t n = M->n, npad = M->npad;
    const int k = M->k, q = M->q, d = M->d;
    const double one = 1.0, mhalf = -0.5;
    *not_pd = 0;
    *gave_up = 0;
    if (impl == 0) impl = ctx->chol_impl;
    const bool builtin = impl != 1;
    PotrfOpts popt;
    popt.impl = impl;
    const int xt = builtin ? (int)round_up(k, 128) : 0;
    const int64_t ld = npad + xt;
    double *Phi, *B;
    int *dinfo;
    MRBF_TRY(get_buf(ctx, S_PHI, (size_t)ld * npad, &Phi));
    MRBF_TRY(get_buf(ctx, S_RHS, (size_t)npad * k, &B));
    MRBF_TRY(get_buf(ctx, S_INFO, (size_t)4, &dinfo));
    MRBF_HIP(ctx, hipMemsetAsync(dinfo, 0, 4 * sizeof(int), ctx->stream));
    const bool tailq = q > 1 && tail_basis_applies(M) && M->k == k;
    if (!tailq) hipLaunchKernelGGL(rhs_from_values_kernel, dim3(nblk(npad * k)), dim3(256), 0, ctx->stream, Y, n, k, B, npad);
    double *Q1 = nullptr, *Wm = nullptr, *G = nullptr, *T1 = nullptr, *scal = nullptr, *Tall = nullptr, *LxInv = nullptr;
    int64_t lt = 0, dq = 0;
    info->mu = 0.0;
    hipStream_t main_stream = ctx->stream;
    const bool side = q > 0 && ctx->panel_stream && ctx->panel_stream != main_stream && n >= 2048;
    const bool fused = q > 0 && gram_w_applies(ctx, M) && (q == 1 || round_up(d, 128) == 128);
    if (q > 0) {
        MRBF_TRY(get_buf(ctx, S_Q1, (size_t)npad * q, &Q1));
        MRBF_TRY(get_buf(ctx, S_W1, (size_t)npad * q, &Wm));
        MRBF_TRY(get_buf(ctx, S_G, (size_t)q * q, &G));
        MRBF_TRY(get_buf(ctx, S_T1, (size_t)q * k, &T1));
        MRBF_TRY(get_buf(ctx, S_MISC, (size_t)8, &scal));
        if (side) {
            MRBF_HIP(ctx, hipEventRecord(ctx->evx[0], main_stream));
            MRBF_HIP(ctx, hipStreamWaitEvent(ctx->panel_stream, ctx->evx[0], 0));
            ctx->stream = ctx->panel_stream;
        }
        struct RestoreStream {
            mrbf_ctx *c;
            hipStream_t s;
            ~RestoreStream() { c->stream = s; }
        } restore{ctx, main_stream};
        if (tailq) {
            double *scratch;
            MRBF_TRY(get_buf(ctx, S_PI, tail_basis_scratch_doubles(), &scratch));
            MRBF_TRY(get_buf(ctx, S_QR_INV, (size_t)128 * 128, &LxInv));
            MRBF_TRY(launch_tail_basis(ctx, M, Y, scratch, LxInv, T1, Q1, B, builtin ? Phi : nullptr, ld, xt, dinfo));
        } else if (q > 1) {
            dq = round_up(d, 128);
            lt = dq + npad;
            MRBF_TRY(get_buf(ctx, S_PI, (size_t)lt * dq, &Tall));
            MRBF_HIP(ctx, hipMemsetAsync(Tall, 0, (size_t)lt * dq * sizeof(double), ctx->stream));
            hipLaunchKernelGGL(xc_to_tall_kernel, dim3(nblk(n * d)), dim3(256), 0, ctx->stream, M->Xc, n, d, M->dpad, Tall, lt, dq);
            MRBF_TRY(tsmm_tn(ctx, n, d, d, 1.0, Tall + dq, lt, Tall + dq, lt, 0.0, Tall, lt));
            MRBF_TRY(launch_pad_identity(ctx, Tall, d, dq, lt));
            if (dq == 128) MRBF_TRY(get_buf(ctx, S_QR_INV, (size_t)128 * 128, &LxInv));
            MRBF_TRY(potrf_blocked_tall(ctx, dq, lt, Tall, lt, dinfo + 1, LxInv, popt));
        }
        if (!tailq) hipLaunchKernelGGL(build_q1_kernel, dim3(nblk(npad * q)), dim3(256), 0, ctx->stream, Tall, lt, dq, n, npad, q, Q1);
        if (!fused) MRBF_HIP(ctx, hipMemsetAsync(Wm, 0, (size_t)npad * q * sizeof(double), ctx->stream));
        if (!tailq) {
            MRBF_TRY(tsmm_tn(ctx, n, q, k, 1.0, Q1, npad, B, npad, 0.0, T1, q));
            hipLaunchKernelGGL(sub_qt_kernel, dim3((unsigned)((n + 63) / 64)), dim3(256), 0, ctx->stream, B, npad, Q1, npad, T1, n, q, k);
            if (builtin) hipLaunchKernelGGL(set_rhs_rows_kernel, dim3(nblk(npad * xt)), dim3(256), 0, ctx->stream, Phi, ld, npad, xt, B, k);
        }
        if (side) MRBF_HIP(ctx, hipEventRecord(ctx->evx[1], ctx->stream));
    }
    ctx->stream = main_stream;
    MRBF_HIP(ctx, hipEventRecord(ctx->ev[0], ctx->stream));
    double *Wpart = nullptr, *rspart = nullptr;
    int nseg = 0;
    if (fused)
        MRBF_TRY(launch_gram_w(ctx, M, Phi, ld, &Wpart, &rspart, &nseg));
    else
        MRBF_TRY(launch_gram(ctx, ctx->gram_mode, M->C, M->Xc, M->sq, n, M->npad, M->d, M->dpad, M->kp, Phi, ld));
    MRBF_HIP(ctx, hipEventRecord(ctx->ev[1], ctx->stream));
    if (side) MRBF_HIP(ctx, hipStreamWaitEvent(ctx->stream, ctx->evx[1], 0));
    if (fused) {
        const int skip = (q > 1 && round_up(2 * (q - 1), 16) < round_up(2 * q, 16)) ? 1 : 0;
        const int K2 = (int)round_up(2 * (q - skip), 16);
        double *PA, *PB, *v0 = nullptr;
        MRBF_TRY(get_buf(ctx, S_STAGE_C, (size_t)npad * K2, &PA));
        MRBF_TRY(get_buf(ctx, S_STAGE_D, (size_t)npad * K2, &PB));
        if (skip) MRBF_TRY(get_buf(ctx, S_V0, (size_t)npad, &v0));
        MRBF_TRY(launch_projection_small(ctx, M, Wpart, rspart, nseg, LxInv, Q1, Wm, G, scal, dinfo, K2, skip, PA, PB, v0));
        MRBF_TRY(launch_update_lower(ctx, PA, npad, PB, npad, Phi, ld, npad / 128, K2, v0, 1.0 / std::sqrt((double)n), n));
    } else if (q > 0) {
        MRBF_TRY(symm_panel(ctx, n, npad, q, Phi, ld, Q1, npad, Wm, npad, true, 1.0 / std::sqrt((double)n)));
        MRBF_TRY(tsmm_tn(ctx, n, q, q, 1.0, Q1, npad, Wm, npad, 0.0, G, q));
        hipLaunchKernelGGL(trace_kernel, dim3(1), dim3(256), 0, ctx->stream, G, q, scal);
        MRBF_BLAS(ctx, rocblas_dgemm(ctx->blas, rocblas_operation_none, rocblas_operation_none, (int)n, q, q, &mhalf, Q1, (int)npad,
                                     G, q, &one, Wm, (int)npad));
        hipLaunchKernelGGL(shift_from_trace_kernel, dim3(1), dim3(1), 0, ctx->stream, scal, (double)n * M->kp.phi0,
                           (double)std::max<int64_t>(n - q, 1), dinfo);
        const int skip = (q > 1 && round_up(2 * (q - 1), 16) < round_up(2 * q, 16)) ? 1 : 0;
        const int K2 = (int)round_up(2 * (q - skip), 16);
        double *PA, *PB, *v0 = nullptr;
        MRBF_TRY(get_buf(ctx, S_STAGE_C, (size_t)npad * K2, &PA));
        MRBF_TRY(get_buf(ctx, S_STAGE_D, (size_t)npad * K2, &PB));
        if (skip) MRBF_TRY(get_buf(ctx, S_V0, (size_t)npad, &v0));
        hipLaunchKernelGGL(build_panels_kernel, dim3(nblk(npad * K2)), dim3(256), 0, ctx->stream, Q1, Wm, scal, n, npad, q, K2, skip, PA, PB, v0);
        MRBF_TRY(launch_update_lower(ctx, PA, npad, PB, npad, Phi, ld, npad / 128, K2, v0, 1.0 / std::sqrt((double)n), n));
    }
    MRBF_HIP(ctx, hipEventRecord(ctx->ev[2], ctx->stream));
    int hinfo = 0;
    double *linv_all = nullptr;
    if (builtin) {
        MRBF_TRY(get_buf(ctx, S_CHOL_WS, (size_t)npad * 128, &linv_all));
        MRBF_TRY(launch_pad_identity(ctx, Phi, n, npad, ld));
        if (q == 0) hipLaunchKernelGGL(set_rhs_rows_kernel, dim3(nblk(npad * xt)), dim3(256), 0, ctx->stream, Phi, ld, npad, xt, B, k);
        popt.xreal = k;
        popt.info_clean = true;
        MRBF_TRY(potrf_blocked_tall(ctx, npad, npad + xt, Phi, ld, dinfo, linv_all, popt));
        MRBF_HIP(ctx, hipEventRecord(ctx->ev[3], ctx->stream));
    } else {
        int *dpot;
        MRBF_TRY(get_buf(ctx, S_IPIV, (size_t)4, &dpot));
        MRBF_BLAS(ctx, rocsolver_dpotrf(ctx->blas, rocblas_fill_lower, (int)n, Phi, (int)ld, dpot));
        MRBF_HIP(ctx, hipMemcpyAsync(dinfo, dpot, sizeof(int), hipMemcpyDeviceToDevice, ctx->stream));
        MRBF_HIP(ctx, hipEventRecord(ctx->ev[3], ctx->stream));
    }
    double *T1w = nullptr;
    if (q > 0) MRBF_TRY(get_buf(ctx, S_T1W, (size_t)q * k, &T1w));
    auto solve_tail = [&](bool persistent) -> int {
        if (builtin) {
            hipLaunchKernelGGL(get_rhs_rows_kernel, dim3(nblk(npad * k)), dim3(256), 0, ctx->stream, Phi, ld, npad, B, k);
            if (persistent)
                MRBF_TRY(backsolve_persistent(ctx, npad, Phi, ld, linv_all, B, npad, k, dinfo + 3));
            else
                MRBF_TRY(backsolve_blocked(ctx, npad, Phi, ld, linv_all, B, npad, k));
        } else {
            MRBF_BLAS(ctx, rocsolver_dpotrs(ctx->blas, rocblas_fill_lower, (int)n, k, Phi, (int)ld, B, (int)npad));
        }
        static const int tail3 = mrbf_env("MRBF_TAIL3") ? atoi(mrbf_env("MRBF_TAIL3")) : 1;
        if (tail3 && q > 0 && q <= 129 && k <= 16 && (q == 1 || LxInv)) {
            const int nch = (int)(npad / 64);
            double *T2, *part;
            MRBF_TRY(get_buf(ctx, S_T2, (size_t)q * k, &T2));
            MRBF_TRY(get_buf(ctx, S_TAIL_PART, (size_t)nch * 2 * k * q, &part));
            hipLaunchKernelGGL(tail_dots_kernel, dim3((unsigned)nch), dim3(256), 0, ctx->stream, B, npad, Q1, Wm, npad, n, q, k, part);
            hipLaunchKernelGGL(tail_coeff_kernel, dim3(1), dim3(1024), 0, ctx->stream, part, nch, q, k, q > 1 ? d : 0, T1, G, fused ? 1.0 : 0.5, LxInv,
                               std::sqrt((double)n), M->mean, T2, T1w);
            hipLaunchKernelGGL(tail_apply_kernel, dim3((unsigned)nch), dim3(256), 0, ctx->stream, B, npad, Q1, npad, T2, T1w, n, M->npad, q, k, M->W,
                               M->Wc, M->lam);
            MRBF_HIP(ctx, hipGetLastError());
            return 0;
        }
        if (q > 0) {
            double *T2;
            MRBF_TRY(get_buf(ctx, S_T2, (size_t)q * k, &T2));
            MRBF_HIP(ctx, hipMemcpyAsync(T1w, T1, (size_t)q * k * sizeof(double), hipMemcpyDeviceToDevice, ctx->stream));
            MRBF_TRY(tsmm_tn(ctx, n, q, k, 1.0, Q1, npad, B, npad, 0.0, T2, q));
            hipLaunchKernelGGL(sub_qt_kernel, dim3((unsigned)((n + 63) / 64)), dim3(256), 0, ctx->stream, B, npad, Q1, npad, T2, n, q, k);
            MRBF_TRY(tsmm_tn(ctx, n, q, k, -1.0, Wm, npad, B, npad, 1.0, T1w, q));
            if (q > 1) {
                if (LxInv)
                    hipLaunchKernelGGL(apply_linv_t_kernel, dim3(1), dim3(256), 0, ctx->stream, LxInv, d, T1w + 1, (int64_t)q, k);
                else if (d <= 256)
                    hipLaunchKernelGGL(trsm_lt_small_kernel, dim3(1), dim3(256), 0, ctx->stream, Tall, lt, d, T1w + 1, (int64_t)q, k);
                else
                    MRBF_BLAS(ctx, rocblas_dtrsm(ctx->blas, rocblas_side_left, rocblas_fill_lower, rocblas_operation_transpose,
                                                 rocblas_diagonal_non_unit, d, k, &one, Tall, (int)lt, T1w + 1, q));
            }
            hipLaunchKernelGGL(finish_lambda_kernel, dim3((unsigned)k), dim3(64), 0, ctx->stream, T1w, q, k, std::sqrt((double)n), M->mean);
        }
        hipLaunchKernelGGL(scatter_solution_kernel, dim3(nblk(M->npad * k + (int64_t)q * k)), dim3(256), 0, ctx->stream, B, npad, n,
                           M->npad, k, q, (int64_t)0, M->W, M->Wc, M->lam, T1w ? T1w : B, (int64_t)q);
        MRBF_HIP(ctx, hipGetLastError());
        return 0;
    };
    MRBF_TRY(solve_tail(true));
    MRBF_HIP(ctx, hipEventRecord(ctx->ev[4], ctx->stream));
    {
        int hflags_local[4] = {0, 0, 0, 0};
        double hscal_local[2] = {0.0, 0.0};
        int *hflags = ctx->hpin ? reinterpret_cast<int *>(ctx->hpin + HPIN_FIT_FLAGS) : hflags_local;
        double *hscal = ctx->hpin ? reinterpret_cast<double *>(ctx->hpin + HPIN_FIT_SCAL) : hscal_local;
        hscal[0] = hscal[1] = 0.0;
        static const int publish = mrbf_env("MRBF_FIT_PUBLISH") ? atoi(mrbf_env("MRBF_FIT_PUBLISH")) : 1;
        if (ctx->hpin && publish) {
            unsigned long long *hstat = nullptr;
            const unsigned long long *dstat = nullptr;
            if (ctx->mega_stat_pending && ctx->mega_stat_dev) {
                ctx->hpin[HPIN_MEGA_STAT] = ~0ull;
                hstat = &ctx->hpin[HPIN_MEGA_STAT];
                dstat = ctx->mega_stat_dev;
                ctx->mega_stat_pending = 2;
            }
            hipLaunchKernelGGL(fit_publish_kernel, dim3(1), dim3(64), 0, ctx->stream, (const int *)dinfo, q > 0 ? (const double *)scal : nullptr, dstat,
                               hflags, hscal, hstat);
        } else {
        MRBF_HIP(ctx, hipMemcpyAsync(hflags, dinfo, 4 * sizeof(int), hipMemcpyDeviceToHost, ctx->stream));
        if (q > 0) MRBF_HIP(ctx, hipMemcpyAsync(hscal, scal, 2 * sizeof(double), hipMemcpyDeviceToHost, ctx->stream));
        MRBF_TRY(mega_stat_enqueue(ctx));
        }
        MRBF_HIP(ctx, hipStreamSynchronize(ctx->stream));
        MRBF_TRY(mega_stat_finish(ctx));
        info->ms_factor_device = ctx->last_device_ms;
        hinfo = hflags[0];
        if (hinfo < 0) {
            *gave_up = 1;
            info->giveup_code = -hinfo;
            return 0;
        }
        info->factor_info = hinfo;
        if (q > 0) info->mu = hscal[1];
        if (hflags[1] < 0) {
            *gave_up = 1;
            info->giveup_code = -hflags[1];
            return 0;
        }
        if (hflags[1] != 0) {
            *not_pd = 1;
            info->factor_info = -2;
            return 0;
        }
        if (hflags[2] != 0) {
            *not_pd = 1;
            info->factor_info = -1;
            return 0;
        }
        if (hinfo != 0) {
            *not_pd = 1;
            return 0;
        }
        if (hflags[3] != 0) {
            info->fallbacks |= MRBF_FB_BACKSOLVE_BLOCKED;
            info->giveup_code = hflags[3];
            MRBF_TRY(solve_tail(false));
            MRBF_HIP(ctx, hipEventRecord(ctx->ev[4], ctx->stream));
        }
    }
    MRBF_HIP(ctx, hipEventSynchronize(ctx->ev[4]));
    MRBF_HIP(ctx, hipEventElapsedTime(&info->ms_gram, ctx->ev[0], ctx->ev[1]));
    MRBF_HIP(ctx, hipEventElapsedTime(&info->ms_project, ctx->ev[1], ctx->ev[2]));
    MRBF_HIP(ctx, hipEventElapsedTime(&info->ms_factor, ctx->ev[2], ctx->ev[3]));
    MRBF_HIP(ctx, hipEventElapsedTime(&info->ms_solve, ctx->ev[3], ctx->ev[4]));
    info->path = q > 0 ? MRBF_PATH_PROJ_CHOL : MRBF_PATH_CHOL;
    return 0;
}

void fill_small_prob(const mrbf_ctx *ctx, const mrbf_model *M, const double *Y, double *ws, int *flags, double *scal, int *cl, smallfit::Prob *P) {
    P->n = (int)M->n;
    P->d = M->d;
    P->k = M->k;
    P->q = M->q;
    P->deg = M->deg;
    P->n16 = (int)round_up(M->n, 16);
    P->npad = (int)M->npad;
    P->dpad = M->dpad;
    P->q16 = (int)round_up(std::max(M->q, 1), 16);
    P->kp = M->kp;
    P->C = M->C;
    P->Y = Y;
    P->Xc = M->Xc;
    P->sq = M->sq;
    P->mean = M->mean;
    P->W = M->W;
    P->Wc = M->Wc;
    P->lam = M->lam;
    P->ws = ws;
    P->flags = flags;
    P->scal = scal;
    P->stamps = nullptr;
    P->cl = cl;
    P->spin_ticks = (unsigned long long)std::max(1, ctx->spin_ms) * 100000ull;
    P->fault = (ctx->debug_fault & 4) ? 1 : 0;
    {
        static const int d6 = mrbf_env("MRBF_SMALL_DIAG6") ? atoi(mrbf_env("MRBF_SMALL_DIAG6")) : 1;
        P->diag6 = d6;
    }
    P->mean_given = 0;
}
int small_fit_verdict(const mrbf_model *M, const int *hflags, const double *hscal, mrbf_fit_info *info) {
    info->path = M->q > 0 ? MRBF_PATH_PROJ_CHOL : MRBF_PATH_CHOL;
    info->mu = M->q > 0 ? hscal[1] : 0.0;
    info->factor_info = hflags[0];
    if (hflags[1] != 0) {
        info->factor_info = -2;
        return 1;
    }
    if (hflags[2] != 0) {
        info->factor_info = -1;
        return 1;
    }
    return hflags[0] != 0 ? 1 : 0;
}
static int fit_check_enqueue(mrbf_ctx *ctx, mrbf_model *M, const double *Y, double *h, hipEvent_t e0, hipEvent_t e1);
static int fit_check_finish(mrbf_ctx *ctx, const mrbf_model *M, const double *h, mrbf_fit_info *info, hipEvent_t e0, hipEvent_t e1);
static int fit_small(mrbf_ctx *ctx, mrbf_model *M, const double *Y, mrbf_fit_info *info, int *not_pd, int force_nc, int *nc_used,
                     bool *checked = nullptr) {
    *not_pd = 0;
    if (checked) *checked = false;
    smallfit::Prob P;
    const smallfit::Carve cv = smallfit::carve((int)M->npad, (int)round_up(std::max(M->q, 1), 16));
    double *ws, *scal;
    int *flags;
    MRBF_TRY(get_buf(ctx, S_SMALL_WS, cv.total, &ws));
    MRBF_TRY(get_buf(ctx, S_SMALL_FLAGS, (size_t)4, &flags));
    MRBF_TRY(get_buf(ctx, S_MISC, (size_t)8, &scal));
    int *cl;
    MRBF_TRY(get_buf(ctx, S_SMALL_CL, (size_t)smallfit::CL_WORDS, &cl));
    fill_small_prob(ctx, M, Y, ws, flags, scal, cl, &P);
    static const int want_stamps = mrbf_env("MRBF_SMALL_STAMPS") ? atoi(mrbf_env("MRBF_SMALL_STAMPS")) : 0;
    long long *dstamps = nullptr;
    if (want_stamps) {
        MRBF_TRY(get_buf(ctx, S_SMALL_DESC, (size_t)16, &dstamps));
        P.stamps = dstamps;
    }
    int hflags_local[4] = {0, 0, 0, 0};
    double hscal_local[2] = {0.0, 0.0}, hchk_local[3] = {0, 0, 0};
    int *hflags = ctx->hpin ? reinterpret_cast<int *>(ctx->hpin + HPIN_SMALL_FLAGS) : hflags_local;
    double *hscal = ctx->hpin ? reinterpret_cast<double *>(ctx->hpin + HPIN_SMALL_SCAL) : hscal_local;
    double *hchk = ctx->hpin ? reinterpret_cast<double *>(ctx->hpin + HPIN_SMALL_CHK) : hchk_local;
    int nc = force_nc > 0 ? force_nc : small_fit_cluster(ctx, 1);
    for (int attempt = 0; attempt < 2; ++attempt) {
        MRBF_HIP(ctx, hipMemsetAsync(cl, 0, smallfit::CL_WORDS * sizeof(int), ctx->stream));
        MRBF_HIP(ctx, hipEventRecord(ctx->ev[0], ctx->stream));
        MRBF_TRY(launch_small_fit(ctx, &P, 1, nullptr, nc));
        MRBF_HIP(ctx, hipEventRecord(ctx->ev[1], ctx->stream));
        MRBF_HIP(ctx, hipMemcpyAsync(hflags, flags, 4 * sizeof(int), hipMemcpyDeviceToHost, ctx->stream));
        MRBF_HIP(ctx, hipMemcpyAsync(hscal, scal, 2 * sizeof(double), hipMemcpyDeviceToHost, ctx->stream));
        hchk[0] = hchk[1] = hchk[2] = 0.0;
        const bool with_check = checked && ctx->residual;
        if (with_check) MRBF_TRY(fit_check_enqueue(ctx, M, Y, hchk, ctx->ev[2], ctx->ev[3]));
        MRBF_HIP(ctx, hipStreamSynchronize(ctx->stream));
        if (with_check && hflags[3] == 0 && hflags[0] == 0 && hflags[1] == 0 && hflags[2] == 0) {
            MRBF_TRY(fit_check_finish(ctx, M, hchk, info, ctx->ev[2], ctx->ev[3]));
            *checked = true;
        }
        if (nc == 1) break;
        if (hflags[3] == 0) {
            ctx->small_timeouts = 0;
            break;
        }
        if (hflags[3] == 2 || ++ctx->small_timeouts >= 3) ctx->small_nc = 1;
        nc = 1;
    }
    *nc_used = nc;
    MRBF_HIP(ctx, hipEventElapsedTime(&info->ms_factor, ctx->ev[0], ctx->ev[1]));
    if (want_stamps) {
        long long hs[16];
        MRBF_HIP(ctx, hipMemcpy(hs, dstamps, sizeof(hs), hipMemcpyDeviceToHost));
        static const char *names[] = {"centre", "gram", "Q1", "W,G,mu,V", "K update", "rhs", "potrf", "solves", "tail"};
// ... 117 lines not shown
```

Baseline: 176.8.

## Fold small launches into neighbours and retile the lower-triangle update

Several unrelated changes land together. The RHS-row gather now runs inside the backsolve premul kernel, and the mega-Cholesky status kernel is deferred into the fit publish kernel, which removes two tiny launches from the fit path. launch_update_lower becomes a job kernel that splits diagonal tiles into 64-row halves and skips the upper triangle, and the tail-Q kernels raise their wave priority. The cost is more complex status plumbing through a shared ctl pointer and a new K%8 restriction on the update.

```diff
diff --git a/include/mrbf.h b/include/mrbf.h
--- a/include/mrbf.h
+++ b/include/mrbf.h
@@ -196,6 +196,8 @@
 int32_t mrbf_debug_env(const char *name);
 int32_t mrbf_debug_mfma_layout(mrbf_ctx *ctx, double *out16x16_a_times_b, const double *A16x4, const double *B4x16);
 int32_t mrbf_debug_potrf(mrbf_ctx *ctx, int64_t n, double *A_colmajor_inout, int32_t impl, int32_t *info, float *ms);
+int32_t mrbf_debug_update_lower(mrbf_ctx *ctx, int32_t nt, int32_t K, const double *A, const double *B, double *C_inout,
+                                const double *cvec_or_null, double cs, int64_t cn);
 int32_t mrbf_debug_diag(mrbf_ctx *ctx, const double *A128, int32_t reps, float *ms_per_call, double *shader_cycles,
                         double *realtime_us);
 int32_t mrbf_debug_mfma_peak(mrbf_ctx *ctx, int32_t blocks_per_cu, int32_t threads, int32_t iters, float *ms, double *tflops);
diff --git a/morbit.jl_amd/_lib.py b/morbit.jl_amd/_lib.py
--- a/morbit.jl_amd/_lib.py
+++ b/morbit.jl_amd/_lib.py
@@ -200,6 +200,7 @@
     "mrbf_debug_ps_rank": (ctypes.c_int32, [c_vp, ctypes.c_int32, c_vp, c_vp, ctypes.c_uint64, ctypes.c_int32, ctypes.c_int32, c_ip, c_ip]),
     "mrbf_debug_mfma_peak": (ctypes.c_int32, [c_vp, ctypes.c_int32, ctypes.c_int32, ctypes.c_int32, c_fp, c_dp]),
     "mrbf_debug_mfma_asm": (ctypes.c_int32, [c_vp, ctypes.c_int32, ctypes.c_int32, ctypes.c_int32, c_fp, c_dp, c_dp]),
+    "mrbf_debug_update_lower": (ctypes.c_int32, [c_vp, ctypes.c_int32, ctypes.c_int32, c_vp, c_vp, c_vp, c_vp, ctypes.c_double, ctypes.c_int64]),
     "mrbf_debug_dgemm": (ctypes.c_int32, [c_vp, ctypes.c_int32, ctypes.c_int32, ctypes.c_int32, c_fp, c_dp]),
     "mrbf_debug_mega_tables": (ctypes.c_int32, [ctypes.c_int32] * 8 + [c_vp]),
     "mrbf_debug_mega_tables2": (ctypes.c_int32, [ctypes.c_int32] * 8 + [c_vp, c_vp]),
diff --git a/morbit.jl_amd/csrc/backsolve.hip b/morbit.jl_amd/csrc/backsolve.hip
--- a/morbit.jl_amd/csrc/backsolve.hip
+++ b/morbit.jl_amd/csrc/backsolve.hip
@@ -19,9 +19,18 @@
 
 __global__ __launch_bounds__(256) void premul_kernel(const double *__restrict__ L, int64_t lda, const double *__restrict__ linv_all,
                                                      double *__restrict__ Mbuf, int nb, unsigned *__restrict__ flags, int nflags,
-                                                     unsigned long long *__restrict__ xb, int nxb) {
+                                                     unsigned long long *__restrict__ xb, int nxb, const double *__restrict__ rows,
+                                                     double *__restrict__ Y, int64_t ldy, int k) {
     for (int e = blockIdx.x * 256 + threadIdx.x; e < nflags; e += gridDim.x * 256) flags[e] = 0u;
     for (int e = blockIdx.x * 256 + threadIdx.x; e < nxb; e += gridDim.x * 256) xb[e] = ~0ull;
+    if (rows) {
+        const int64_t npad = (int64_t)nb * NB;
+        for (int64_t e = (int64_t)blockIdx.x * 256 + threadIdx.x; e < npad * k; e += (int64_t)gridDim.x * 256) {
+            const int l = (int)(e % k);
+            const int64_t i = e / k;
+            Y[i + (int64_t)l * ldy] = rows[(npad + l) + i * lda];
+        }
+    }
     const int slab = blockIdx.x & 3, t = (blockIdx.x >> 2) & 1, j = blockIdx.x >> 3;
     const int i = j + 1 + t;
     if (i >= nb) return;
@@ -341,15 +350,18 @@
 }
 
 int backsolve_blocked(mrbf_ctx *ctx, int64_t npad, const double *L, int64_t lda, const double *linv_all, double *Y, int64_t ldy, int k);
+int launch_get_rhs_rows(mrbf_ctx *ctx, const double *A, int64_t ld, int64_t npad, double *B, int64_t ldb, int k);
 
 int backsolve_persistent(mrbf_ctx *ctx, int64_t npad, const double *L, int64_t lda, const double *linv_all, double *Y, int64_t ldy, int k,
-                         int *status) {
+                         int *status, bool rhs_rows) {
     using namespace bsolve;
     const int nb = (int)(npad / NB);
     static const int force_old = mrbf_env("MRBF_BACKSOLVE_LAUNCHES") ? atoi(mrbf_env("MRBF_BACKSOLVE_LAUNCHES")) : 0;
     const int ncu = ctx->ncu;
-    if (force_old || nb < 3 || nb > ncu || (lda & 1) || (reinterpret_cast<uintptr_t>(L) & 15))
+    if (force_old || nb < 3 || nb > ncu || (lda & 1) || (reinterpret_cast<uintptr_t>(L) & 15)) {
+        if (rhs_rows) MRBF_TRY(launch_get_rhs_rows(ctx, L, lda, npad, Y, ldy, k));
         return backsolve_blocked(ctx, npad, L, lda, linv_all, Y, ldy, k);
+    }
     unsigned *flags;
     MRBF_TRY(get_buf(ctx, S_BSOLVE_FLAGS, (size_t)(nb + 1) * 32, &flags));
     const unsigned long long spin_ticks = (unsigned long long)std::max(1, ctx->spin_ms) * 100000ull;
@@ -358,7 +370,7 @@
     MRBF_TRY(get_buf(ctx, S_BSOLVE_X, (size_t)2 * nb * 4 * NB, &xb));
     MRBF_TRY(get_buf(ctx, S_BSOLVE_M, (size_t)nb * 2 * NB * NB, &Mbuf));
     hipLaunchKernelGGL(premul_kernel, dim3((unsigned)(8 * (nb - 1))), dim3(256), 0, ctx->stream, L, lda, linv_all, Mbuf, nb, flags, (nb + 1) * 32,
-                       reinterpret_cast<unsigned long long *>(xb), 2 * nb * 4 * NB);
+                       reinterpret_cast<unsigned long long *>(xb), 2 * nb * 4 * NB, rhs_rows ? L : (const double *)nullptr, Y, ldy, k);
     static const bool want_stamps = mrbf_env("MRBF_BSOLVE_STAMPS") && atoi(mrbf_env("MRBF_BSOLVE_STAMPS")) != 0;
     long long *stamps = nullptr;
     if (want_stamps) {
diff --git a/morbit.jl_amd/csrc/chol.hip b/morbit.jl_amd/csrc/chol.hip
--- a/morbit.jl_amd/csrc/chol.hip
+++ b/morbit.jl_amd/csrc/chol.hip
@@ -6,6 +6,8 @@
 
 int debug_diag(mrbf_ctx *ctx, const double *A128_dev, int reps, float *ms_per_call, unsigned long long *stamps_host);
 int launch_pad_identity(mrbf_ctx *ctx, double *A, int64_t n, int64_t npad, int64_t ld);
+int launch_update_lower(mrbf_ctx *ctx, const double *A, int64_t lda, const double *B, int64_t ldb, double *C, int64_t ldc, int64_t nt, int K,
+                        const double *cvec, double cs, int64_t cn);
 
 int potrf_lower(mrbf_ctx *ctx, int impl, int64_t n, double *A, int64_t lda, int *info_host) {
     int *dinfo;
@@ -66,6 +68,32 @@
     return MRBF_OK;
 }
 
+extern "C" int32_t mrbf_debug_update_lower(mrbf_ctx *ctx, int32_t nt, int32_t K, const double *A, const double *B, double *C,
+                                           const double *cvec, double cs, int64_t cn) {
+    if (!ctx) return -1;
+    if (nt <= 0) return -2;
+    if (K <= 0 || K % 16 != 0) return -3;
+    if (!A) return -4;
+    if (!B) return -5;
+    if (!C) return -6;
+    (void)hipSetDevice(ctx->device);
+    const int64_t N = (int64_t)nt * 128;
+    double *dA, *dB, *dC, *dv = nullptr;
+    MRBF_TRY(get_buf(ctx, S_STAGE_C, (size_t)N * K, &dA));
+    MRBF_TRY(get_buf(ctx, S_STAGE_D, (size_t)N * K, &dB));
+    MRBF_TRY(get_buf(ctx, S_PHI, (size_t)N * N, &dC));
+    if (cvec) MRBF_TRY(get_buf(ctx, S_V0, (size_t)N, &dv));
+    MRBF_HIP(ctx, hipStreamSynchronize(ctx->stream));
+    MRBF_HIP(ctx, hipMemcpy(dA, A, (size_t)N * K * sizeof(double), hipMemcpyHostToDevice));
+    MRBF_HIP(ctx, hipMemcpy(dB, B, (size_t)N * K * sizeof(double), hipMemcpyHostToDevice));
+    MRBF_HIP(ctx, hipMemcpy(dC, C, (size_t)N * N * sizeof(double), hipMemcpyHostToDevice));
+    if (cvec) MRBF_HIP(ctx, hipMemcpy(dv, cvec, (size_t)N * sizeof(double), hipMemcpyHostToDevice));
+    MRBF_TRY(launch_update_lower(ctx, dA, N, dB, N, dC, N, nt, K, dv, cs, cn));
+    MRBF_HIP(ctx, hipStreamSynchronize(ctx->stream));
+    MRBF_HIP(ctx, hipMemcpy(C, dC, (size_t)N * N * sizeof(double), hipMemcpyDeviceToHost));
+    return MRBF_OK;
+}
+
 extern "C" int32_t mrbf_debug_diag(mrbf_ctx *ctx, const double *A128, int32_t reps, float *ms_per_call, double *shader_cycles,
                                    double *realtime_us) {
     if (!ctx) return -1;
diff --git a/morbit.jl_amd/csrc/chol_blocked.hip b/morbit.jl_amd/csrc/chol_blocked.hip
--- a/morbit.jl_amd/csrc/chol_blocked.hip
+++ b/morbit.jl_amd/csrc/chol_blocked.hip
@@ -116,6 +116,80 @@
         }
     }
     if (bid + (int)gridDim.x < tile_end) __syncthreads();
+    }
+}
+
+template <int TM>
+__device__ __forceinline__ void update_lower_job(const double *__restrict__ A, int64_t lda, const double *__restrict__ B, int64_t ldb,
+                                                 double *__restrict__ C, int64_t ldc, int K, int64_t I0, int64_t J0,
+                                                 const double *__restrict__ cvec, double cs, int64_t cn, double *smem) {
+    constexpr int NJ = TM / 32;
+    constexpr bool DIAG = TM == 64;
+    const int tid = threadIdx.x, lane = tid & 63, wave = tid >> 6;
+    const int l15 = lane & 15, l4 = lane >> 4;
+    const int ioff = (TM == 128) ? (wave >> 1) * 64 : 0;
+    const int joff = (TM == 128) ? (wave & 1) * 64 : wave * 32;
+    v4d acc[NJ][4];
+#pragma unroll
+    for (int j = 0; j < NJ; ++j)
+#pragma unroll
+        for (int r = 0; r < 4; ++r) {
+            const int64_t gj = J0 + joff + j * 16 + l4 + 4 * r;
+#pragma unroll
+            for (int i = 0; i < 4; ++i) {
+                const int64_t gi = I0 + ioff + i * 16 + l15;
+                acc[j][i][r] = (!DIAG || gi >= gj) ? -C[gi + gj * ldc] : 0.0;
+            }
+        }
+    mega::gemm_acc<TM>(A + I0, lda, B + J0, ldb, K, acc, smem);
+    double cvi[4] = {0.0, 0.0, 0.0, 0.0}, cei[4] = {0.0, 0.0, 0.0, 0.0};
+    if (cvec) {
+#pragma unroll
+        for (int i = 0; i < 4; ++i) {
+            const int64_t gi = I0 + ioff + i * 16 + l15;
+            cvi[i] = cs * cvec[gi];
+            cei[i] = gi < cn ? cs : 0.0;
+        }
+    }
+#pragma unroll
+    for (int j = 0; j < NJ; ++j) {
+        double cvj[4] = {0.0, 0.0, 0.0, 0.0}, cej[4] = {0.0, 0.0, 0.0, 0.0};
+        if (cvec) {
+#pragma unroll
+            for (int r = 0; r < 4; ++r) {
+                const int64_t gj = J0 + joff + j * 16 + l4 + 4 * r;
+                cvj[r] = cvec[gj];
+                cej[r] = gj < cn ? 1.0 : 0.0;
+            }
+        }
+#pragma unroll
+        for (int r = 0; r < 4; ++r) {
+            const int64_t gj = J0 + joff + j * 16 + l4 + 4 * r;
+#pragma unroll
+            for (int i = 0; i < 4; ++i) {
+                const int64_t gi = I0 + ioff + i * 16 + l15;
+                double x = -acc[j][i][r];
+                if (cvec) x -= fma(cei[i], cvj[r], cvi[i] * cej[r]);
+                if (!DIAG || gi >= gj) C[gi + gj * ldc] = x;
+            }
+        }
+    }
+}
+
+__global__ __launch_bounds__(256, 2) void update_lower_jobs_kernel(const double *__restrict__ A, int64_t lda, const double *__restrict__ B,
+                                                                   int64_t ldb, double *__restrict__ C, int64_t ldc, int K, int nt,
+                                                                   const double *__restrict__ cvec, double cs, int64_t cn) {
+    __shared__ __attribute__((aligned(16))) double smem[mega::NSTG * mega::STG];
+    const int job = blockIdx.x, noff = nt * (nt - 1) / 2;
+    if (job < noff) {
+        int t = (int)((sqrt(8.0 * (double)job + 1.0) - 1.0) * 0.5);
+        while ((t + 1) * (t + 2) / 2 <= job) ++t;
+        while (t * (t + 1) / 2 > job) --t;
+        const int ti = t + 1, tj = job - t * (t + 1) / 2;
+        update_lower_job<128>(A, lda, B, ldb, C, ldc, K, (int64_t)ti * 128, (int64_t)tj * 128, cvec, cs, cn, smem);
+    } else {
+        const int h = job - noff, ti = h >> 1;
+        update_lower_job<64>(A, lda, B, ldb, C, ldc, K, (int64_t)ti * 128 + 64 * (h & 1), (int64_t)ti * 128, cvec, cs, cn, smem);
     }
 }
 
@@ -399,8 +473,9 @@
 int launch_update_lower(mrbf_ctx *ctx, const double *A, int64_t lda, const double *B, int64_t ldb, double *C, int64_t ldc, int64_t nt,
                         int K, const double *cvec, double cs, int64_t cn) {
     if (nt <= 0 || K <= 0) return 0;
-    hipLaunchKernelGGL((chol_update_kernel<128, UPD_LOWER_SUB>), dim3((unsigned)(nt * (nt + 1) / 2)), dim3(256), 0, ctx->stream, A,
-                       lda, B, ldb, C, ldc, K, (const int *)nullptr, (int)nt, 0, cvec, cs, cn);
+    if (nt > 32767 || K % 8 != 0) return fail(ctx, MRBF_EHIP, "launch_update_lower: nt=%lld K=%d out of range", (long long)nt, K);
+    const int64_t njobs = nt * (nt - 1) / 2 + 2 * nt;
+    hipLaunchKernelGGL(update_lower_jobs_kernel, dim3((unsigned)njobs), dim3(256), 0, ctx->stream, A, lda, B, ldb, C, ldc, K, (int)nt, cvec, cs, cn);
     MRBF_HIP(ctx, hipGetLastError());
     return 0;
 }
diff --git a/morbit.jl_amd/csrc/chol_mega.hip b/morbit.jl_amd/csrc/chol_mega.hip
--- a/morbit.jl_amd/csrc/chol_mega.hip
+++ b/morbit.jl_amd/csrc/chol_mega.hip
@@ -1275,7 +1275,11 @@
     }
     unsigned long long *dstat;
     MRBF_TRY(get_buf(ctx, S_MEGA_STAT, (size_t)2, &dstat));
-    hipLaunchKernelGGL(mega_status_kernel, dim3(1), dim3(1), 0, ctx->stream, (const unsigned *)fl, dinfo, dstat);
+    static_assert(CTL_TIMEOUT == CTL_TIMEOUT_WORD && CTL_TS == CTL_TS_WORD, "common.hpp names these two words for the fit's publish kernel");
+    if (opt.status_later)
+        ctx->mega_ctl_dev = fl;
+    else
+        hipLaunchKernelGGL(mega_status_kernel, dim3(1), dim3(1), 0, ctx->stream, (const unsigned *)fl, dinfo, dstat);
     ctx->mega_stat_dev = dstat;
     ctx->mega_stat_shape = (long)NT * 100000 + MT;
     ctx->mega_stat_pending = 1;
@@ -1298,6 +1302,14 @@
             fprintf(stderr, "  (NT %d MT %d pcols %u qpanel %u/%d qchain %u/%d)\n", NT, MT, h[CTL_PCOLS], h[CTL_QP], a.npanel, h[CTL_QC], a.nchainjobs);
         }
     }
+    MRBF_HIP(ctx, hipGetLastError());
+    return 0;
+}
+
+int mega_status_late(mrbf_ctx *ctx, int *dinfo) {
+    if (!ctx->mega_ctl_dev) return 0;
+    hipLaunchKernelGGL(mega::mega_status_kernel, dim3(1), dim3(1), 0, ctx->stream, ctx->mega_ctl_dev, dinfo, ctx->mega_stat_dev);
+    ctx->mega_ctl_dev = nullptr;
     MRBF_HIP(ctx, hipGetLastError());
     return 0;
 }
diff --git a/morbit.jl_amd/csrc/common.hpp b/morbit.jl_amd/csrc/common.hpp
--- a/morbit.jl_amd/csrc/common.hpp
+++ b/morbit.jl_amd/csrc/common.hpp
@@ -77,7 +77,11 @@
     bool any_size = false;
     int xreal = 0;
     bool info_clean = false;
-};
+    bool status_later = false;
+};
+namespace mega {
+constexpr int CTL_TIMEOUT_WORD = 64, CTL_TS_WORD = 144;
+}
 struct EvalHints {
     bool population = false;
     bool check_call = false;
@@ -106,6 +110,7 @@
     unsigned long long *mega_stat_dev = nullptr;
     long mega_stat_shape = 0;
     int mega_stat_pending = 0;
+    const unsigned *mega_ctl_dev = nullptr;
     char *pin_base = nullptr;
     size_t pin_off = 0;
     bool pin_armed = false;
@@ -244,5 +249,6 @@
 int mega_collect_stat(mrbf_ctx *ctx);
 int mega_stat_enqueue(mrbf_ctx *ctx);
 int mega_stat_finish(mrbf_ctx *ctx);
-
-}
+int mega_status_late(mrbf_ctx *ctx, int *dinfo);
+
+}
diff --git a/morbit.jl_amd/csrc/small.hip b/morbit.jl_amd/csrc/small.hip
--- a/morbit.jl_amd/csrc/small.hip
+++ b/morbit.jl_amd/csrc/small.hip
@@ -726,11 +726,15 @@
     double rsn;
 };
 constexpr int TQ_PS = 4096 + 1024 + 16;
+#ifndef MRBF_TAILQ_PRIO
+#define MRBF_TAILQ_PRIO 3
+#endif
 
 __global__ __launch_bounds__(256) void tailq_gram_kernel(TailQ t) {
     __shared__ double red[4];
     __shared__ double part4[4][64];
     const int tid = threadIdx.x, p = blockIdx.x;
+    __builtin_amdgcn_s_setprio(MRBF_TAILQ_PRIO);
     const int n16 = (t.n + 15) & ~15, d16 = (t.d + 15) & ~15;
     const int r0 = p * t.rows, r1 = min(r0 + t.rows, n16), K = max(r1 - r0, 0);
     double *out = t.part + (size_t)p * TQ_PS;
@@ -839,6 +843,7 @@
     __shared__ double part4[4][64];
     const int tid = threadIdx.x, d = t.d, d16 = (t.d + 15) & ~15;
     const int R0 = 64 * blockIdx.x;
+    __builtin_amdgcn_s_setprio(MRBF_TAILQ_PRIO);
     for (int e = tid; e < 64 * 65; e += 256) Qs[e] = 0.0;
     __syncthreads();
     wg_gemm<true, true, false>(64, d16, d16, t.Xc + (int64_t)R0 * t.dpad, t.dpad, t.LinvX, 128, NoPre(), [&](int i, int a, double v, double) {
diff --git a/morbit.jl_amd/csrc/solve.hip b/morbit.jl_amd/csrc/solve.hip
--- a/morbit.jl_amd/csrc/solve.hip
+++ b/morbit.jl_amd/csrc/solve.hip
@@ -4,11 +4,23 @@
 namespace mrbf {
 
 __global__ void fit_publish_kernel(const int *__restrict__ dinfo, const double *__restrict__ scal, const unsigned long long *__restrict__ dstat,
-                                   int *__restrict__ hflags, double *__restrict__ hscal, unsigned long long *__restrict__ hstat) {
+                                   const unsigned *__restrict__ ctl, int *__restrict__ hflags, double *__restrict__ hscal,
+                                   unsigned long long *__restrict__ hstat) {
     const int t = threadIdx.x;
-    if (t < 4) hflags[t] = dinfo[t];
+    if (t < 4) {
+        int v = dinfo[t];
+        if (t == 0 && ctl && ctl[mega::CTL_TIMEOUT_WORD] != 0 && v == 0) v = -(int)ctl[mega::CTL_TIMEOUT_WORD];
+        hflags[t] = v;
+    }
     if (t >= 4 && t < 6 && scal) hscal[t - 4] = scal[t - 4];
-    if (t == 6 && dstat && hstat) hstat[0] = dstat[0];
+    if (t == 6 && hstat) {
+        if (ctl) {
+            const unsigned long long *ts = (const unsigned long long *)(ctl + mega::CTL_TS_WORD);
+            hstat[0] = (ts[0] != 0 && ts[1] != 0) ? ts[1] - ~ts[0] : 0ull;
+        } else if (dstat) {
+            hstat[0] = dstat[0];
+        }
+    }
 }
 
 __global__ void fill_saddle_kernel(const double *__restrict__ Pi, int64_t n, int q, double *__restrict__ S, int64_t N) {
@@ -304,7 +316,7 @@
 
 int backsolve_blocked(mrbf_ctx *ctx, int64_t npad, const double *L, int64_t lda, const double *linv_all, double *Y, int64_t ldy, int k);
 int backsolve_persistent(mrbf_ctx *ctx, int64_t npad, const double *L, int64_t lda, const double *linv_all, double *Y, int64_t ldy, int k,
-                         int *status);
+                         int *status, bool rhs_rows);
 int launch_update_lower(mrbf_ctx *ctx, const double *A, int64_t lda, const double *B, int64_t ldb, double *C, int64_t ldc, int64_t nt, int K,
                         const double *cvec, double cs, int64_t cn);
 int launch_pad_identity(mrbf_ctx *ctx, double *A, int64_t n, int64_t npad, int64_t ld);
@@ -320,12 +332,17 @@
     const int64_t i = idx / xt;
     A[(npad + l) + i * ld] = (l < k) ? B[i + (int64_t)l * npad] : 0.0;
 }
-__global__ void get_rhs_rows_kernel(const double *__restrict__ A, int64_t ld, int64_t npad, double *__restrict__ B, int k) {
+__global__ void get_rhs_rows_kernel(const double *__restrict__ A, int64_t ld, int64_t npad, double *__restrict__ B, int64_t ldb, int k) {
     const int64_t idx = (int64_t)blockIdx.x * blockDim.x + threadIdx.x;
     if (idx >= npad * k) return;
     const int l = (int)(idx % k);
     const int64_t i = idx / k;
-    B[i + (int64_t)l * npad] = A[(npad + l) + i * ld];
+    B[i + (int64_t)l * ldb] = A[(npad + l) + i * ld];
+}
+int launch_get_rhs_rows(mrbf_ctx *ctx, const double *A, int64_t ld, int64_t npad, double *B, int64_t ldb, int k) {
+    hipLaunchKernelGGL(get_rhs_rows_kernel, dim3(nblk(npad * k)), dim3(256), 0, ctx->stream, A, ld, npad, B, ldb, k);
+    MRBF_HIP(ctx, hipGetLastError());
+    return 0;
 }
 __global__ void xc_to_tall_kernel(const double *__restrict__ Xc, int64_t n, int d, int dpad, double *__restrict__ Tall, int64_t lt,
                                   int64_t dq) {
@@ -697,6 +714,8 @@
         if (q == 0) hipLaunchKernelGGL(set_rhs_rows_kernel, dim3(nblk(npad * xt)), dim3(256), 0, ctx->stream, Phi, ld, npad, xt, B, k);
         popt.xreal = k;
         popt.info_clean = true;
+        popt.status_later = true;
+        ctx->mega_ctl_dev = nullptr;
         MRBF_TRY(potrf_blocked_tall(ctx, npad, npad + xt, Phi, ld, dinfo, linv_all, popt));
         MRBF_HIP(ctx, hipEventRecord(ctx->ev[3], ctx->stream));
     } else {
@@ -710,11 +729,12 @@
     if (q > 0) MRBF_TRY(get_buf(ctx, S_T1W, (size_t)q * k, &T1w));
     auto solve_tail = [&](bool persistent) -> int {
         if (builtin) {
-            hipLaunchKernelGGL(get_rhs_rows_kernel, dim3(nblk(npad * k)), dim3(256), 0, ctx->stream, Phi, ld, npad, B, k);
-            if (persistent)
-                MRBF_TRY(backsolve_persistent(ctx, npad, Phi, ld, linv_all, B, npad, k, dinfo + 3));
-            else
+            if (persistent) {
+                MRBF_TRY(backsolve_persistent(ctx, npad, Phi, ld, linv_all, B, npad, k, dinfo + 3, true));
+            } else {
+                MRBF_TRY(launch_get_rhs_rows(ctx, Phi, ld, npad, B, npad, k));
                 MRBF_TRY(backsolve_blocked(ctx, npad, Phi, ld, linv_all, B, npad, k));
+            }
         } else {
             MRBF_BLAS(ctx, rocsolver_dpotrs(ctx->blas, rocblas_fill_lower, (int)n, k, Phi, (int)ld, B, (int)npad));
         }
@@ -774,8 +794,10 @@
                 ctx->mega_stat_pending = 2;
             }
             hipLaunchKernelGGL(fit_publish_kernel, dim3(1), dim3(64), 0, ctx->stream, (const int *)dinfo, q > 0 ? (const double *)scal : nullptr, dstat,
-                               hflags, hscal, hstat);
+                               ctx->mega_ctl_dev, hflags, hscal, hstat);
+            ctx->mega_ctl_dev = nullptr;
         } else {
+        MRBF_TRY(mega_status_late(ctx, dinfo));
         MRBF_HIP(ctx, hipMemcpyAsync(hflags, dinfo, 4 * sizeof(int), hipMemcpyDeviceToHost, ctx->stream));
         if (q > 0) MRBF_HIP(ctx, hipMemcpyAsync(hscal, scal, 2 * sizeof(double), hipMemcpyDeviceToHost, ctx->stream));
         MRBF_TRY(mega_stat_enqueue(ctx));
```

Result: no change. 178.3 (median of 6 runs) (+0.9%).
